# rubendhz/houdini-gsplat-renderer

Hardware: AMD Instinct MI355X
Metric: frames/sec at 1920x1080 + achieved HBM GB/s (blend kernel) (higher is better)
Workload: dtype f32

## Files before the change

### houdini-gsplat-renderer_amd/csrc/gsr_api.hip

```cpp
#include <hip/hip_runtime.h>

#include <cmath>
#include <cstddef>
#include <cstdio>
#include <cstring>
#include <chrono>
#include <algorithm>
#include <new>
#include <vector>

#include "../../include/gsplat_hip.h"
#include "gsr_device.h"
#include "k_binning.h"
#include "k_blend.h"
#include "k_cluster.h"
#include "k_colour.h"
#include "k_preprocess.h"
#ifdef GSR_HOST_TIMING
static double g_t_verdict = 0, g_acc_py = 0, g_acc_pre = 0, g_acc_launch = 0; static long g_acc_n = 0;
static double now_us() { return std::chrono::duration<double, std::micro>(std::chrono::steady_clock::now().time_since_epoch()).count(); }
#endif
#include "k_sort.h"
#include "k_wire.h"
#include "gsr_frame_plan.h"
// ... 21 lines not shown
    bool same(const SortKey& o) const
    {
        return gen == o.gen && shard_index == o.shard_index && shard_count == o.shard_count && shard_layout == o.shard_layout && flags == o.flags &&
               band_first == o.band_first && band_tile_rows == o.band_tile_rows &&
               std::memcmp(&cam, &o.cam, sizeof(gsr_camera)) == 0;
    }
};

struct FrameArgs {
    gsr_camera cam{};
    const float* depth = nullptr;
    bool depth_is_device = false;
    float* out = nullptr;
    bool out_is_device = false;
    int aov = 0;
    float* aov_out = nullptr;
    gsr_background bg{};
};

struct FrameJob {
    FrameArgs args;
    bool open = false;
    GsrFrame f{};
    uint32_t n = 0;
    int local_tiles = 0, band_rows = 0, n_super = 0;
    size_t out_px = 0;
    float* target = nullptr;
    int format = 0;
    const float* d_depth = nullptr;
    bool timing = false, timing_all = false, use_map = false;
    bool speculative = false;
    int bn_items = 4;
    uint32_t bn_grid = 0;
    uint32_t k1_grid = 0;
    bool local_sort = false;
    bool sort_failed = false;
    bool redo = false;
    bool ranges_folded = false;
    bool deferred = false;
    bool lazy = false;
    bool cull = false;
    bool direct = false;
    uint32_t ticket = 0;
    int phase = 0;
    bool dcull = false;
    int dpar = 0;
    bool sort_fresh = false;
    bool dblind = false;
    bool dstat = false;
    bool blend_guess_plain = false;
    float2* aov_target = nullptr;
    GsrBgArgs bg{};
};

struct FrameSlot {
    hipStream_t own = nullptr;
    hipStream_t stream = nullptr;
    hipEvent_t ev_done = nullptr;
    hipEvent_t ev_user = nullptr;
    hipEvent_t ev_band[GSR_HOST_BANDS_MAX] = {nullptr, nullptr, nullptr, nullptr, nullptr, nullptr, nullptr, nullptr};
    int bands = 0;
    int band_row[GSR_HOST_BANDS_MAX + 1] = {0, 0, 0, 0, 0, 0, 0, 0, 0};
    hipEvent_t ev_pairs = nullptr;
    GsrRecord* rec = nullptr;
    uint32_t *keyA = nullptr, *keyB = nullptr;
    uint32_t* blk_cnt = nullptr;
    uint2 *valA = nullptr, *valB = nullptr;
    uint32_t* d_n = nullptr;
    float* zwin = nullptr;
    StageBuf depth_stage;
    float* dpyr = nullptr;
    size_t dpyr_cap = 0;
    uint32_t* dactive = nullptr;
    int dpar = 0;
    bool dpyr_built = false;
    bool sorted_dculled = false;
    uint32_t* hist = nullptr;
    size_t hist_cap = 0;
    uint32_t* totals = nullptr;
    uint2* pvA = nullptr;
    size_t pair_cap = 0;
    int32_t *sstart = nullptr, *send = nullptr;
    uint4* tile_work = nullptr;
    size_t tile_cap = 0;
    uint4* tile_work_a = nullptr;
    float* tbuf = nullptr;
    size_t tbuf_cap = 0;
    float* hpyr2 = nullptr;
    uint32_t* slab = nullptr;
    bool slab_dirty = false;
    int32_t* redo = nullptr;
    int32_t* order = nullptr;
    size_t order_cap = 0;
    bool order_valid = false;
    int order_age = 0;
    int order_sig[6] = {0, 0, 0, 0, 0, 0}, order_per_xcd = 0;
    uint32_t* st_scan = nullptr;
    GsrTilePartial* partial = nullptr;
    uint32_t* sup_work = nullptr;
    int sup_par = 0;
    float* hpyr = nullptr;
    float* hpyr_next = nullptr;
    float* hraw = nullptr;
    float* hstat = nullptr;
    bool hstat_valid = false;
    uint32_t* dbg_viol = nullptr;
    int hpyr_re = 0;
    uint32_t* cseg = nullptr;
    uint32_t* ccnt = nullptr;
    uint32_t* d_counts = nullptr;
    uint32_t* bkt_key = nullptr;
    uint2* bkt_val = nullptr;
    uint32_t* bkt_cnt = nullptr;
    GsrSlotHints hints;
    GsrLocalSortPolicy local_pol;
    unsigned long long* h_end = nullptr;
    unsigned long long* h_rows = nullptr;
    unsigned long long* h_rows_dev = nullptr;
    uint32_t rows_ticket = 0;
    int rows_tiles_y = 0;
    unsigned long long* h_end_dev = nullptr;
    bool horizon_valid = false;
    int horizon_sig[7] = {0, 0, 0, 0, 0, 0, 0};
    gsr_camera horizon_cam{};
    bool sorted_culled = false;
    unsigned long long* lazy_ctr = nullptr;
    uint32_t* colour_evals = nullptr;
    bool last_lazy = false;
    StageBuf fb;
    StageBuf aovb;
    float* fb32 = nullptr;
    size_t fb32_cap = 0;
    StageBuf bgb;
    unsigned long long* counters = nullptr;
    unsigned long long* h_total = nullptr;
    unsigned long long* h_total_dev = nullptr;
    uint32_t ticket = 0;
    unsigned long long* h_counters = nullptr;
    unsigned long long* d_frame = nullptr;
    bool sort_valid = false;
    SortKey sort_key{};
    uint32_t key_min = 0;
    FrameJob job;
    int last_tiles_x = 0, last_local_ty = 0, last_supers = 0;
    uint32_t last_cc_groups = 0, last_cc_per = 0;
    uint32_t last_pairs = 0;
    int super_tile = 0, stiles_x = 0, stiles_y = 0;
    uint64_t frame_id = 0;
    hipEvent_t ev[GSR_STAGE_EVENTS];
    bool ev_pending = false;
    bool ev_all = false;
    bool ev_ok = false;
};

struct gsr_context {
    int device = 0;
    hipStream_t own_stream = nullptr;
    hipStream_t stream = nullptr;

    uint32_t n = 0, cap = 0;
    bool has_sh = false;
    float origin[3] = {0, 0, 0};
    uint64_t geo_gen = 0;
    bool has_geometry = false;
    float4* geoA = nullptr;
    uint4* geoB = nullptr;
    uint4* col = nullptr;
    uint4* colrow = nullptr;
    int col_chunks = 0;
    float4* geoA2 = nullptr;
    uint4 *geoB2 = nullptr, *col2 = nullptr, *colrow2 = nullptr;
    float4 *clusA2 = nullptr, *clusB2 = nullptr;
    uint32_t* perm = nullptr;
    std::vector<int32_t> h_perm;
    float4 *clusA = nullptr, *clusB = nullptr;
    uint32_t nclus = 0;
    uint32_t* prefix = nullptr;
    uint32_t* prefix_all = nullptr;
    uint32_t* prefix_none = nullptr;
    bool prefix_valid = false;
    bool uploading = false;
    uint32_t up_total = 0, up_filled = 0;
    bool bbox_ok = false;
    double bb_lo[3] = {0, 0, 0}, bb_hi[3] = {0, 0, 0};

    FrameSlot slot[GSR_MAX_SLOTS];
    uint32_t* pos_order = nullptr;
    size_t pos_cap = 0;
    bool pos_valid = false;
    uint64_t pos_gen = 0;
    float pos_cam[3] = {0, 0, 0}, last_cam[3] = {0, 0, 0};
    uint32_t pos_kmin = 0, pos_kmax = 0;
    bool last_cam_set = false;
    uint32_t* blk_pre = nullptr;
    size_t blk_pre_cap = 0;
    int opt_order_keep = 32;
    int opt_fuse_order = 1;
    int opt_mid_sort = 1;
    int opt_host_bands = 4;
// ... 68 lines not shown
    hipDeviceSynchronize();
    return hipMemcpyFromSymbol(out128, HIP_SYMBOL(g_kprof), sizeof(g_kprof)) == hipSuccess ? 0 : -1;
}
#endif
#ifdef SW_PROFILE
extern "C" int gsr_debug_sw_profile(unsigned long long* out8) {
    hipDeviceSynchronize();
    hipMemcpyFromSymbol(out8, HIP_SYMBOL(g_sw_prof), 64);
    return 0;
}
#endif
#ifdef GSR_DEBUG_XCC
extern "C" int gsr_debug_xcc(unsigned* out4, int reset) {
    hipDeviceSynchronize();
    if (out4) hipMemcpyFromSymbol(out4, HIP_SYMBOL(g_dbg_xcc), 16);
    if (reset) { void* p = nullptr; hipGetSymbolAddress(&p, HIP_SYMBOL(g_dbg_xcc)); hipMemset(p, 0, 16); }
    return 0;
}
#endif
#ifdef BL_PROFILE
extern "C" int gsr_debug_blend_profile(unsigned long long* out, int reset) {
    hipDeviceSynchronize();
    if (out) hipMemcpyFromSymbol(out, HIP_SYMBOL(g_blend_prof), sizeof(unsigned long long) * BLP_MAX_WG * 4 * 16);
    if (reset) { void* p = nullptr; hipGetSymbolAddress(&p, HIP_SYMBOL(g_blend_prof)); hipMemset(p, 0, sizeof(unsigned long long) * BLP_MAX_WG * 4 * 16); }
    return 0;
}
#endif
__attribute__((visibility("hidden"))) int gsr_internal_set_error(int code, const char* text) { return set_err(code, "%s", text); }
void gsr_internal_comm_release(gsr_context* c);
bool gsr_internal_comm_set_user_stream(gsr_context* c, void* stream, void* own);
int gsr_internal_comm_sync(gsr_context* c);

extern "C" int gsr_device_count(void)
{
    int n = 0;
    if (hipGetDeviceCount(&n) != hipSuccess) return 0;
    return n;
}

extern "C" const char* gsr_last_error(void) { return g_err; }
extern "C" const char* gsr_version(void) { return GSR_VERSION_STR; }

static int finish_open_frames(gsr_context* c);

static int sync_all(gsr_context* c)
{
    int frc = finish_open_frames(c);
    if (frc) return frc;
    for (int k = 0; k < GSR_MAX_SLOTS; ++k)
        if (c->slot[k].own) HIP_TRY(hipStreamSynchronize(c->slot[k].own));
    if (c->stream) HIP_TRY(hipStreamSynchronize(c->stream));
    return GSR_OK;
}

static bool slot_init(FrameSlot& sl)
{
    bool ok = hipStreamCreateWithFlags(&sl.own, hipStreamNonBlocking) == hipSuccess;
    sl.stream = sl.own;
    ok = ok && hipEventCreateWithFlags(&sl.ev_done, hipEventDisableTiming) == hipSuccess;
    ok = ok && hipEventCreateWithFlags(&sl.ev_user, hipEventDisableTiming) == hipSuccess;
    ok = ok && hipEventCreateWithFlags(&sl.ev_pairs, hipEventDisableTiming) == hipSuccess;
    ok = ok && hipMalloc(reinterpret_cast<void**>(&sl.counters), 8 * sizeof(unsigned long long)) == hipSuccess;
    ok = ok && hipMalloc(reinterpret_cast<void**>(&sl.d_n), sizeof(uint32_t)) == hipSuccess;
    ok = ok && hipMemset(sl.d_n, 0, sizeof(uint32_t)) == hipSuccess;
    ok = ok && hipMalloc(reinterpret_cast<void**>(&sl.totals), 512 * sizeof(uint32_t)) == hipSuccess;
    ok = ok && hipMalloc(reinterpret_cast<void**>(&sl.lazy_ctr), 2 * sizeof(unsigned long long)) == hipSuccess;
    ok = ok && hipMemset(sl.lazy_ctr, 0, 2 * sizeof(unsigned long long)) == hipSuccess;
    ok = ok && hipMalloc(reinterpret_cast<void**>(&sl.colour_evals), 256 * sizeof(uint32_t)) == hipSuccess;
    ok = ok && hipMemset(sl.colour_evals, 0, 256 * sizeof(uint32_t)) == hipSuccess;
    ok = ok && hipMalloc(reinterpret_cast<void**>(&sl.hpyr), GSR_PYR_FLOATS * sizeof(float)) == hipSuccess;
    ok = ok && hipMalloc(reinterpret_cast<void**>(&sl.hpyr_next), GSR_PYR_FLOATS * sizeof(float)) == hipSuccess;
    ok = ok && hipMalloc(reinterpret_cast<void**>(&sl.hraw), (size_t)GSR_MAX_TILES_SIDE * GSR_MAX_TILES_SIDE * sizeof(float)) == hipSuccess;
    ok = ok && hipMalloc(reinterpret_cast<void**>(&sl.hstat), (size_t)GSR_MAX_TILES_SIDE * GSR_MAX_TILES_SIDE * sizeof(float)) == hipSuccess;
    ok = ok && hipMalloc(reinterpret_cast<void**>(&sl.hpyr2), GSR_PYR_FLOATS * sizeof(float)) == hipSuccess;
    ok = ok && hipMalloc(reinterpret_cast<void**>(&sl.slab), (GSR_SLAB_BINS + 8) * sizeof(uint32_t)) == hipSuccess;
    ok = ok && hipMemset(sl.slab, 0, (GSR_SLAB_BINS + 8) * sizeof(uint32_t)) == hipSuccess;
    ok = ok && hipMalloc(reinterpret_cast<void**>(&sl.ccnt), CC_MAX_GROUPS * sizeof(uint32_t)) == hipSuccess;
    ok = ok && hipMalloc(reinterpret_cast<void**>(&sl.bkt_key), (size_t)BK_BUCKETS * BK_CAP * sizeof(uint32_t)) == hipSuccess;
    ok = ok && hipMalloc(reinterpret_cast<void**>(&sl.bkt_val), (size_t)BK_BUCKETS * BK_CAP * sizeof(uint2)) == hipSuccess;
    ok = ok && hipMalloc(reinterpret_cast<void**>(&sl.bkt_cnt), (size_t)BK_BUCKETS * BK_STRIDE * sizeof(uint32_t)) == hipSuccess;
    ok = ok && hipMemset(sl.bkt_cnt, 0, (size_t)BK_BUCKETS * BK_STRIDE * sizeof(uint32_t)) == hipSuccess;
    ok = ok && hipMalloc(reinterpret_cast<void**>(&sl.d_counts), 4 * sizeof(uint32_t)) == hipSuccess;
    ok = ok && hipMemset(sl.d_counts, 0, 4 * sizeof(uint32_t)) == hipSuccess;
    ok = ok && hipHostMalloc(reinterpret_cast<void**>(&sl.h_end), sizeof(unsigned long long), hipHostMallocMapped | hipHostMallocCoherent) == hipSuccess;
    if (ok) sl.h_end[0] = 0ull;
    ok = ok && hipHostGetDevicePointer(reinterpret_cast<void**>(&sl.h_end_dev), sl.h_end, 0) == hipSuccess;
    ok = ok && hipMalloc(reinterpret_cast<void**>(&sl.st_scan), 512 * sizeof(uint32_t)) == hipSuccess;
    ok = ok && hipMemset(sl.st_scan, 0, 512 * sizeof(uint32_t)) == hipSuccess;
    ok = ok && hipMalloc(reinterpret_cast<void**>(&sl.partial), (size_t)(GSR_MAX_TILES_SIDE / 8) * (GSR_MAX_TILES_SIDE / 8) * sizeof(GsrTilePartial)) == hipSuccess;
    ok = ok && hipMalloc(reinterpret_cast<void**>(&sl.sup_work), 512 * sizeof(uint32_t)) == hipSuccess;
    ok = ok && hipMemset(sl.sup_work, 0, 512 * sizeof(uint32_t)) == hipSuccess;
    ok = ok && hipHostMalloc(reinterpret_cast<void**>(&sl.h_total), 4 * sizeof(unsigned long long), hipHostMallocMapped | hipHostMallocCoherent) == hipSuccess;
    if (ok) { sl.h_total[0] = 0ull; sl.h_total[1] = 0ull; sl.h_total[2] = 0ull; sl.h_total[3] = 0ull; }
    ok = ok && hipHostGetDevicePointer(reinterpret_cast<void**>(&sl.h_total_dev), sl.h_total, 0) == hipSuccess;
    ok = ok && hipHostMalloc(reinterpret_cast<void**>(&sl.h_counters), 8 * sizeof(unsigned long long), 0) == hipSuccess;
    if (ok) for (int j = 0; j < 8; ++j) sl.h_counters[j] = 0;
    ok = ok && hipMalloc(reinterpret_cast<void**>(&sl.d_frame), 8 * sizeof(unsigned long long)) == hipSuccess;
    ok = ok && hipMemset(sl.d_frame, 0, 8 * sizeof(unsigned long long)) == hipSuccess;
    ok = ok && hipMemset(sl.counters, 0, 8 * sizeof(unsigned long long)) == hipSuccess;
    if (ok) {
        for (int k = 0; k < GSR_STAGE_EVENTS; ++k) sl.ev[k] = nullptr;
        sl.ev_ok = true;
        for (int k = 0; k < GSR_STAGE_EVENTS && ok; ++k) ok = hipEventCreate(&sl.ev[k]) == hipSuccess;
    }
    return ok;
}

static void slot_free_splat_arrays(FrameSlot& sl)
{
    dev_free(sl.rec); dev_free(sl.keyA); dev_free(sl.keyB); dev_free(sl.valA); dev_free(sl.valB); dev_free(sl.blk_cnt);
    dev_free(sl.zwin); dev_free(sl.cseg);
    sl.sort_valid = false;
}

struct SlotSplatArrays {
    GsrRecord* rec = nullptr;
    uint32_t *keyA = nullptr, *keyB = nullptr, *blk_cnt = nullptr, *cseg = nullptr;
    uint2 *valA = nullptr, *valB = nullptr;
    float* zwin = nullptr;
    void release() { dev_free(rec); dev_free(keyA); dev_free(keyB); dev_free(valA); dev_free(valB); dev_free(blk_cnt); dev_free(zwin); dev_free(cseg); }
};
static int alloc_splat_arrays(SlotSplatArrays& a, size_t cap)
{
    int rc = GSR_OK;
    if ((rc = dev_alloc(&a.rec, cap)) || (rc = dev_alloc(&a.keyA, cap + 256)) || (rc = dev_alloc(&a.keyB, cap + 256)) ||
        (rc = dev_alloc(&a.valA, cap + 256)) || (rc = dev_alloc(&a.valB, cap + 256)) ||
        (rc = dev_alloc(&a.zwin, cap)) || (rc = dev_alloc(&a.blk_cnt, cap / 256 + 16)) ||
        (rc = dev_alloc(&a.cseg, cap / GSR_CLUSTER + (size_t)CC_THREADS * 64 + 16)))
        a.release();
    return rc;
}
static void slot_take_splat_arrays(FrameSlot& sl, SlotSplatArrays& a)
{
    slot_free_splat_arrays(sl);
    sl.rec = a.rec; sl.keyA = a.keyA; sl.keyB = a.keyB; sl.valA = a.valA; sl.valB = a.valB; sl.blk_cnt = a.blk_cnt; sl.zwin = a.zwin; sl.cseg = a.cseg;
    a = SlotSplatArrays{};
}

static void slot_destroy(FrameSlot& sl)
{
    slot_free_splat_arrays(sl);
    dev_free(sl.hist); dev_free(sl.totals);
    dev_free(sl.pvA);
    dev_free(sl.sstart); dev_free(sl.send); dev_free(sl.tile_work); dev_free(sl.order); dev_free(sl.sup_work); sl.fb.release(); dev_free(sl.fb32); sl.aovb.release(); sl.bgb.release();
    dev_free(sl.hpyr); dev_free(sl.hpyr_next); dev_free(sl.hraw); dev_free(sl.hstat); dev_free(sl.hpyr2); dev_free(sl.slab); dev_free(sl.tile_work_a); dev_free(sl.tbuf); dev_free(sl.ccnt); dev_free(sl.bkt_key); dev_free(sl.bkt_val); dev_free(sl.bkt_cnt); dev_free(sl.d_counts); dev_free(sl.st_scan); dev_free(sl.partial);
    if (sl.h_end) (void)hipHostFree(sl.h_end); if (sl.h_rows) (void)hipHostFree(sl.h_rows); sl.depth_stage.release(); dev_free(sl.dpyr); dev_free(sl.dactive);
    dev_free(sl.redo); dev_free(sl.lazy_ctr); dev_free(sl.colour_evals);
    dev_free(sl.counters); dev_free(sl.d_n);
    if (sl.h_total) (void)hipHostFree(sl.h_total);
    if (sl.h_counters) (void)hipHostFree(sl.h_counters);
    dev_free(sl.d_frame);
    if (sl.ev_ok)
        for (int k = 0; k < GSR_STAGE_EVENTS; ++k)
            if (sl.ev[k]) (void)hipEventDestroy(sl.ev[k]);
    if (sl.ev_done) (void)hipEventDestroy(sl.ev_done);
    if (sl.ev_user) (void)hipEventDestroy(sl.ev_user);
    for (int k = 0; k < GSR_HOST_BANDS_MAX; ++k) if (sl.ev_band[k]) (void)hipEventDestroy(sl.ev_band[k]);
    if (sl.ev_pairs) (void)hipEventDestroy(sl.ev_pairs);
    if (sl.own) (void)hipStreamDestroy(sl.own);
}

extern "C" int gsr_create(int device, gsr_context** out)
{
    if (!out) return set_err(GSR_E_INVALID, "gsr_create: out is NULL");
    *out = nullptr;
    int ndev = gsr_device_count();
    if (ndev <= 0) return set_err(GSR_E_NO_DEVICE, "gsr_create: no HIP device visible");
    if (device < 0 || device >= ndev) return set_err(GSR_E_NO_DEVICE, "gsr_create: device %d out of range (0..%d)", device, ndev - 1);
    HIP_TRY(hipSetDevice(device));
    gsr_context* c = new (std::nothrow) gsr_context();
    if (!c) return set_err(GSR_E_OOM, "gsr_create: host allocation failed");
    c->device = device;
    if (const char* e = std::getenv("GSR_ORDER_KEEP")) c->opt_order_keep = std::atoi(e);
    if (const char* e = std::getenv("GSR_SCATTER_DIRECT")) c->opt_scatter_direct = std::atoi(e);
    if (const char* e = std::getenv("GSR_K1_SCATTER")) c->opt_k1_scatter = std::atoi(e);
    if (const char* e = std::getenv("GSR_HOST_BANDS")) c->opt_host_bands = std::min(std::max(std::atoi(e), 1), GSR_HOST_BANDS_MAX);
    if (const char* e = std::getenv("GSR_MID_SORT")) c->opt_mid_sort = std::atoi(e);
    if (const char* e = std::getenv("GSR_FUSE_ORDER")) c->opt_fuse_order = std::atoi(e);
    if (const char* e = std::getenv("GSR_SLAB_FRAC")) { const int v = std::atoi(e); if (v >= 1 && v <= 255) c->slab_frac = v; }
    if (const char* e = std::getenv("GSR_SLAB_MIN")) { const int v = std::atoi(e); if (v >= 1) c->slab_min = v; }
    if (const char* e = std::getenv("GSR_SLAB_MAX")) { const int v = std::atoi(e); if (v >= 1) c->slab_max = v; }
    if (const char* e = std::getenv("GSR_BN_ITEMS")) { const int v = std::atoi(e); if (v == 1 || v == 2 || v == 4) c->opt_bn_items = v; }
    hipError_t e = hipStreamCreateWithFlags(&c->own_stream, hipStreamNonBlocking);
    if (e != hipSuccess) { delete c; return set_err(GSR_E_HIP, "hipStreamCreate failed: %s", hipGetErrorString(e)); }
    c->stream = c->own_stream;
    bool ok = true;
    for (int k = 0; k < GSR_MAX_SLOTS && ok; ++k) ok = slot_init(c->slot[k]);
    if (!ok) {
        gsr_destroy(c);
        return set_err(GSR_E_HIP, "gsr_create: allocating frame slots (streams/events/mailboxes) failed");
    }
    if (hipMalloc(reinterpret_cast<void**>(&c->prefix), 256 * 4) != hipSuccess ||
        hipMalloc(reinterpret_cast<void**>(&c->prefix_all), 256 * 4) != hipSuccess ||
        hipMalloc(reinterpret_cast<void**>(&c->prefix_none), 256 * 4) != hipSuccess ||
        hipMemset(c->prefix, 0xff, 256 * 4) != hipSuccess || hipMemset(c->prefix_all, 0xff, 256 * 4) != hipSuccess ||
        hipMemset(c->prefix_none, 0, 256 * 4) != hipSuccess ||
        hipMalloc(reinterpret_cast<void**>(&c->lazy_hint), 4) != hipSuccess || hipMemset(c->lazy_hint, 0, 4) != hipSuccess) {
        gsr_destroy(c);
        return set_err(GSR_E_HIP, "gsr_create: allocating the colour-prefix tables failed");
    }
    c->st.record_bytes = (int32_t)sizeof(GsrRecord);
    c->st.pair_bytes = 8;
    *out = c;
    return GSR_OK;
}

static void vis_drop_mask(gsr_context* c)
{
    dev_free(c->vis_mask);
    if (c->vis.n_volumes == 0) { c->vis_on = false; c->vis_hidden = 0; }
}

static void free_geometry(gsr_context* c)
{
    dev_free(c->geoA); dev_free(c->geoB); dev_free(c->col); dev_free(c->colrow);
    dev_free(c->perm); dev_free(c->clusA); dev_free(c->clusB); c->nclus = 0; c->h_perm.clear();
    dev_free(c->geoA2); dev_free(c->geoB2); dev_free(c->col2); dev_free(c->colrow2); dev_free(c->clusA2); dev_free(c->clusB2);
    dev_free(c->alpha0);
    dev_free(c->alpha0_2);
    vis_drop_mask(c);
    for (int k = 0; k < GSR_MAX_SLOTS; ++k) slot_free_splat_arrays(c->slot[k]);
    c->cap = 0; c->n = 0;
}

extern "C" void gsr_destroy(gsr_context* c)
{
    if (!c) return;
// ... 1256 lines not shown
}

static inline int mark(FrameSlot& sl, int k)
{
    const FrameJob& j = sl.job;
    if (j.timing && (j.timing_all || k >= 5)) HIP_TRY(hipEventRecord(sl.ev[k], sl.stream));
    return GSR_OK;
}

static GsrRangeArgs range_args(gsr_context* c, FrameSlot& sl)
{
    const FrameJob& j = sl.job;
    GsrRangeArgs a;
    a.totals = sl.totals; a.n_super = j.n_super; a.sstart = sl.sstart; a.send = sl.send; a.host_total = sl.h_total_dev;
    a.ticket = j.ticket; a.max_pairs = (unsigned long long)GSR_MAX_PAIRS; a.redo_count = reinterpret_cast<uint32_t*>(sl.lazy_ctr);
    a.lazy_hint = c->lazy_hint; a.n_sorted = sl.d_n; a.k1_counts = sl.d_counts; a.sorted_keys = sl.keyA;
    a.depth_active = j.dcull ? sl.dactive + j.dpar : (const uint32_t*)nullptr;
    return a;
}

static inline void tile_sig(const GsrFrame& f, int* sig )
{
    const int now[6] = {f.width, f.height, f.shard_rpb > 0 ? f.shard_first : f.shard_index, f.shard_count, f.shard_rpb, f.super_shift};
    std::memcpy(sig, now, sizeof now);
}

static inline int32_t list_cap(const FrameSlot& sl) { return (int32_t)std::min<size_t>(sl.pair_cap, (size_t)0x7fffffff); }

static GsrSumArgs sum_args(const FrameJob& j)
{
    GsrSumArgs g;
    g.n_tiles = j.local_tiles; g.tiles_x = j.f.tiles_x; g.tiles_y = j.f.tiles_y; g.shard = gsr_frame_shard(j.f, 0);
    g.super_shift = j.f.super_shift; g.stiles_x = j.f.stiles_x; g.n_super = j.n_super;
    return g;
}

static GsrHorizonArgs horizon_args(const gsr_context* c, const FrameSlot& sl)
{
    const GsrFrame& f = sl.job.f;
    GsrHorizonArgs hz{};
    hz.list_cap = list_cap(sl); hz.lists = sl.pvA; hz.geoA = c->geoA; hz.idx_mask = f.idx_mask;
    for (int l = 0; l < GSR_PYR_LEVELS; ++l) hz.pyr_off[l] = f.pyr_off[l];
    hz.cam[0] = f.cam[0]; hz.cam[1] = f.cam[1]; hz.cam[2] = f.cam[2];
    return hz;
}

static int queue_blend(gsr_context* c, FrameSlot& sl, bool with_depth, bool guarded)
{
    const FrameJob& j = sl.job;
    const GsrFrame& f = j.f;
    hipStream_t s = sl.stream;
    if (j.local_tiles <= 0) return GSR_OK;
    if (!j.direct) HIP_TRY(hipStreamWaitEvent(s, sl.ev_user, 0));
    GsrBlendArgs a;
    a.guard = guarded ? sl.dactive + j.dpar : (const uint32_t*)nullptr; a.guard_want = 0u;
    {
        const bool persp = f.pr[8] == 0.0f && f.pr[9] == 0.0f && f.pr[12] == 0.0f && f.pr[13] == 0.0f && f.pr[14] == -1.0f && f.pr[15] == 0.0f;
        a.near_alpha = persp ? 0.5f * (1.0f - f.pr[10]) : 0.0f;
        a.near_scale = persp ? 1.12f : 0.0f;
    }
    a.tile_cov = (with_depth && j.dcull && !j.dblind) ? sl.dpyr + 4 * sl.dpyr_cap : (const float*)nullptr;
    a.idx_mask = f.idx_mask; a.zq0 = f.zq0; a.zqs = f.zqs;
    a.tile_dmax = (with_depth && j.dcull && !j.dblind && f.idx_mask != 0xffffffffu) ? sl.dpyr + (size_t)(2 * j.dpar) * sl.dpyr_cap + f.pyr_off[0] : (const float*)nullptr;
    a.width = f.width; a.height = f.height; a.tiles_x = f.tiles_x; a.local_tiles = j.local_tiles;
    a.shard = gsr_frame_shard(f, 0); a.band_rows = j.band_rows;
    a.super_shift = f.super_shift; a.rect_shift = f.rect_shift; a.stiles_x = f.stiles_x; a.use_map = j.use_map ? 1 : 0; a.flags = f.flags;
    a.list_cap = list_cap(sl);
    a.sup_work = (a.use_map && c->opt_swizzle >= 2 && sl.sup_work) ? sl.sup_work + 256 * sl.sup_par : nullptr;
    a.slab = j.phase; a.tbuf = sl.tbuf; a.tile_work_a = sl.tile_work_a;
    uint4* const tw = j.phase == 1 ? sl.tile_work_a : sl.tile_work;
    int sig[6];
    tile_sig(f, sig);
    const bool ordered = a.use_map && c->opt_swizzle >= 2 && sl.order_valid && std::memcmp(sig, sl.order_sig, sizeof sig) == 0;
    const int32_t* tmap = ordered ? sl.order : c->tile_map;
    const unsigned grid = ordered ? (unsigned)(8 * sl.order_per_xcd) : a.use_map ? (unsigned)c->map_grid : (unsigned)j.local_tiles;
    GsrLazyArgs lz;
    lz.f = f; lz.colrow = c->colrow;
    lz.redo = j.lazy ? sl.redo : nullptr;
    lz.redo_count = reinterpret_cast<uint32_t*>(sl.lazy_ctr);
    const bool over = j.bg.kind != 0;
    a.out_format = j.format; a.out_packed = (j.format != GSR_TARGET_RGBA32F || over) ? (void*)j.target : nullptr;
    float4* tgt = reinterpret_cast<float4*>((j.format != GSR_TARGET_RGBA32F || over) ? sl.fb32 : j.target);
    auto launch = [&](auto kernel, unsigned g, const int32_t* map, uint4* work, auto... tail) {
        hipLaunchKernelGGL(kernel, dim3(g), dim3(256), 0, s, a, map, sl.pvA, sl.sstart, sl.send, sl.rec, tgt, work, sl.zwin, j.d_depth, lz, tail...);
    };
    auto launch_verb = [&](auto plain, auto aov, auto bg, unsigned g, const int32_t* map, uint4* work) {
        if (j.aov_target) launch(aov, g, map, work, j.aov_target);
        else if (over) launch(bg, g, map, work, j.bg);
        else launch(plain, g, map, work);
    };
    int nb = 1;
    if (!j.args.out_is_device && j.phase != 1 && c->opt_host_bands > 1 && c->shard_count == 1 && c->band_tile_rows < 0 && f.local_tiles_y >= 4 * c->opt_host_bands) nb = c->opt_host_bands;
    if (nb > 1 && !c->copy_stream && hipStreamCreateWithFlags(&c->copy_stream, hipStreamNonBlocking) != hipSuccess) { c->copy_stream = nullptr; nb = 1; (void)hipGetLastError(); }
    for (int b = 0; b < nb && nb > 1; ++b)
        if (!sl.ev_band[b] && hipEventCreateWithFlags(&sl.ev_band[b], hipEventDisableTiming) != hipSuccess) { sl.ev_band[b] = nullptr; nb = 1; (void)hipGetLastError(); }
    sl.bands = nb;
    for (int b = 0; b < nb; ++b) {
        a.row_lo = nb > 1 ? (int)((int64_t)f.local_tiles_y * b / nb) : 0;
        a.row_hi = nb > 1 ? (int)((int64_t)f.local_tiles_y * (b + 1) / nb) : 0x7fffffff;
        sl.band_row[b] = a.row_lo; sl.band_row[b + 1] = nb > 1 ? a.row_hi : f.local_tiles_y;
        if (with_depth) launch_verb(k_blend<true>, k_blend_aov<true>, k_blend_over<true>, grid, tmap, tw);
        else launch_verb(k_blend<false>, k_blend_aov<false>, k_blend_over<false>, grid, tmap, tw);
        if (j.lazy && with_depth) launch_verb(k_blend_lazy<true>, k_blend_aov_lazy<true>, k_blend_over_lazy<true>, (unsigned)j.local_tiles, c->tile_map, sl.tile_work);
        else if (j.lazy) launch_verb(k_blend_lazy<false>, k_blend_aov_lazy<false>, k_blend_over_lazy<false>, (unsigned)j.local_tiles, c->tile_map, sl.tile_work);
        if (nb > 1) HIP_TRY(hipEventRecord(sl.ev_band[b], s));
    }
    HIP_TRY(hipGetLastError());
    return GSR_OK;
}

static int queue_back_end(gsr_context* c, FrameSlot& sl)
{
    const FrameJob& j = sl.job;
    const GsrFrame& f = j.f;
    hipStream_t s = sl.stream;
    int rc;
    if ((rc = mark(sl, 3))) return rc;
    if (j.n > 0) {
        const uint32_t nblk = div_up(j.n, (uint32_t)BN_THREADS * (uint32_t)j.bn_items);
        const size_t lds = (size_t)4 * j.bn_items * j.n_super * (8 + 4);
        const GsrShard shd = gsr_frame_shard(f, f.rect_shift);
        const GsrRangeArgs ra = j.ranges_folded ? range_args(c, sl) : GsrRangeArgs{};
        const uint32_t bn_extra = (uint32_t)BN_SPLIT_TILES * (uint32_t)std::max(f.stiles_y - 1, 0);
        const uint32_t grid = std::min(nblk, j.bn_grid) + bn_extra + (j.ranges_folded ? 1u : 0u);
#define GSR_PLACE(I) hipLaunchKernelGGL((f.idx_mask != 0xffffffffu ? k_bin_place<I, true> : k_bin_place<I, false>), dim3(grid), dim3(BN_THREADS), lds, s, sl.valA, sl.d_n,          \
                                        f.super_shift - f.rect_shift, shd, f.stiles_x, j.n_super, sl.hist, sl.sstart, nblk, (uint32_t)sl.pair_cap, sl.pvA, ra,   \
                                        f.idx_mask != 0xffffffffu ? sl.zwin : (const float*)nullptr, f.zq0, f.zqs)
        if (j.bn_items == 1) GSR_PLACE(1); else if (j.bn_items == 2) GSR_PLACE(2); else GSR_PLACE(4);
#undef GSR_PLACE
        HIP_TRY(hipGetLastError());
    }
    if ((rc = mark(sl, 4))) return rc;
    if (j.lazy && j.n > 0) {
        const bool predict = c->prefix_valid && !(f.flags & GSR_FLAG_LAZY_NO_PREFIX);
        hipLaunchKernelGGL(k_colour_prefix, dim3((unsigned)(j.n_super * CL_BLOCKS_PER_LIST)), dim3(CL_THREADS), 0, s, f, sl.pvA,
                           sl.sstart, sl.send, (f.flags & GSR_FLAG_LAZY_NO_PREFIX) ? c->prefix_none : (predict ? c->prefix : c->prefix_all),
                           (int)list_cap(sl), c->colrow, sl.rec, sl.colour_evals);
        HIP_TRY(hipGetLastError());
    }
    if ((rc = mark(sl, 5))) return rc;
    sl.job.blend_guess_plain = j.d_depth != nullptr && j.dcull && !c->depth_active && !j.deferred && j.f.idx_mask == 0xffffffffu && !j.aov_target && j.bg.kind == 0;
    if ((rc = queue_blend(c, sl, j.d_depth != nullptr && !sl.job.blend_guess_plain, sl.job.blend_guess_plain))) return rc;
    return mark(sl, 6);
}

static int queue_frame_end(gsr_context* c, FrameSlot& sl)
{
    const FrameJob& j = sl.job;
    hipStream_t s = sl.stream;
    const GsrSumArgs g = sum_args(j);
    GsrHorizonArgs hz{};
    hz.list_cap = list_cap(sl);
    if (c->opt_cull && c->opt_cull != 3 && j.n > 0 && !j.deferred && (c->opt_cull >= 2 || j.cull || j.phase == 2 || (c->cull_pol.vis_unculled >= 300000u && c->cull_pol.holdoff <= 2))) {
        hz = horizon_args(c, sl);
        hz.raw = sl.hraw; hz.pyr_in = sl.hpyr; hz.pyr_out = sl.hpyr_next; hz.dilate = j.f.cull_dilate; hz.culled = j.cull ? 1 : 0;
        hz.host_end = j.cull ? sl.h_end_dev : nullptr; hz.ticket = j.ticket;
        hz.stat = sl.hstat;
        hz.stat_in_use = (j.cull && j.dcull && j.dstat) ? 1 : 0;
        hz.depth_culled = (j.dcull && !j.dblind) ? 1 : 0;
        static const bool dbgv = std::getenv("GSR_DEBUG_VIOL") != nullptr;
        if (dbgv) {
            if (!sl.dbg_viol && hipMalloc(reinterpret_cast<void**>(&sl.dbg_viol), 80 * 4) != hipSuccess) sl.dbg_viol = nullptr;
            if (sl.dbg_viol) (void)hipMemsetAsync(sl.dbg_viol, 0, 80 * 4, s);
            hz.dbg = sl.dbg_viol;
        }
    }
    if (j.phase == 2) { hz.slab = 2; hz.tile_work_a = sl.tile_work_a; }
    const int nblocks8 = ((j.f.tiles_x + 7) >> 3) * ((j.f.tiles_y + 7) >> 3);
    hipLaunchKernelGGL(k_tile_pass, dim3((unsigned)nblocks8), dim3(64), 0, s, sl.tile_work, g, sl.sstart, sl.send, hz, sl.partial, sl.st_scan);
    uint32_t* const prefix_arg = (j.f.sh_order > 0 && c->opt_lazy) ? c->prefix : (uint32_t*)nullptr;
    const uint32_t* const redo_arg = j.lazy ? reinterpret_cast<const uint32_t*>(sl.lazy_ctr) : (const uint32_t*)nullptr;
    uint32_t* const work_next = sl.sup_work ? sl.sup_work + 256 * (sl.sup_par ^ 1) : (uint32_t*)nullptr;
    sl.horizon_valid = hz.raw != nullptr;
    sl.hstat_valid = hz.raw != nullptr;
    int osig[6];
    tile_sig(j.f, osig);
    const bool order_due = c->opt_swizzle >= 3 || (c->opt_swizzle == 2 && c->order_pays);
    const bool order_kept = !order_due && c->opt_swizzle == 2 && c->opt_order_keep > 0 && sl.order_valid && sl.order_age < c->opt_order_keep &&
                            std::memcmp(osig, sl.order_sig, sizeof osig) == 0;
    const bool order_refresh = !order_due && !order_kept && c->opt_swizzle == 2 && c->opt_order_keep > 0 && c->n >= 1000000u;
    if (order_kept) sl.order_age += 1; else sl.order_valid = false;
    const bool order_now = j.use_map && (order_due || order_refresh) && j.local_tiles > 0 && j.n_super <= 256 && sl.sup_work;
    const int per_xcd = 2 * ((j.n_super + 15) / 16) << (2 * j.f.super_shift);
    if (order_now && (size_t)8 * per_xcd > sl.order_cap) {
        const int rc = regrow(s, sl.order, sl.order_cap, (size_t)8 * per_xcd, (size_t)8 * per_xcd);
        if (rc) return rc;
    }
    const bool fused_order = order_now && c->opt_fuse_order != 0;
    if (sl.horizon_valid) sl.hpyr_re = std::min(c->cull_pol.dilate, GSR_DILATE_EXACT_MAX);
    if (fused_order) {
        const GsrOrderArgs oa{sl.tile_work, j.f.tiles_y, sl.sup_work + 256 * sl.sup_par, per_xcd, sl.order};
        const int ndil = sl.horizon_valid ? nblocks8 : 0;
        hipLaunchKernelGGL(k_frame_end_order, dim3(9u + (unsigned)((ndil + TO_THREADS / 64 - 1) / (TO_THREADS / 64))), dim3(TO_THREADS), 0, s, sl.partial, nblocks8, ndil, g, sl.counters, sl.d_n, sl.d_frame,
                           prefix_arg, redo_arg, sl.colour_evals, sl.lazy_ctr + 1, sl.sstart, sl.send, c->lazy_hint, work_next, hz, sl.st_scan, sl.hpyr_re, oa);
        HIP_TRY(hipGetLastError());
    } else if (sl.horizon_valid) {
        hipLaunchKernelGGL(k_frame_end, dim3((unsigned)nblocks8 + 1u), dim3(SW_THREADS), 0, s, sl.partial, nblocks8, g, sl.counters, sl.d_n, sl.d_frame,
                           prefix_arg, redo_arg, sl.colour_evals, sl.lazy_ctr + 1, sl.sstart, sl.send, c->lazy_hint, work_next, hz, sl.st_scan, sl.hpyr_re);
        HIP_TRY(hipGetLastError());
    } else {
        hipLaunchKernelGGL(k_sum_work, dim3(1), dim3(SW_THREADS), 0, s, sl.partial, nblocks8, g, sl.counters, sl.d_n, sl.d_frame,
                           prefix_arg, redo_arg, sl.colour_evals, sl.lazy_ctr + 1, sl.sstart, sl.send, c->lazy_hint, work_next, hz, sl.st_scan);
        HIP_TRY(hipGetLastError());
    }
    if (sl.horizon_valid) {
        std::swap(sl.hpyr, sl.hpyr_next);
        tile_sig(j.f, sl.horizon_sig);
        sl.horizon_sig[6] = (int)c->geo_gen;
        sl.horizon_cam = j.args.cam;
    }
    if (order_now) {
        if (!fused_order) {
            hipLaunchKernelGGL(k_tile_order, dim3(8), dim3(TO_THREADS), 0, s, sl.tile_work, g, j.f.tiles_y, sl.sup_work + 256 * sl.sup_par,
                               per_xcd, sl.order);
            HIP_TRY(hipGetLastError());
        }
        std::memcpy(sl.order_sig, osig, sizeof osig);
        sl.order_per_xcd = per_xcd;
        sl.order_valid = true;
        sl.order_age = 0;
    }
    if (c->opt_row_work && sl.h_rows_dev) {
        hipLaunchKernelGGL(k_row_work, dim3((unsigned)((j.f.tiles_y + RW_THREADS / 64 - 1) / (RW_THREADS / 64))), dim3(RW_THREADS), 0, s, sl.tile_work,
                           j.phase == 2 ? sl.tile_work_a : (const uint4*)nullptr, g, sl.h_rows_dev, j.ticket);
        HIP_TRY(hipGetLastError());
        sl.rows_ticket = j.ticket; sl.rows_tiles_y = j.f.tiles_y;
    }
    sl.sup_par ^= 1;
    if (j.f.sh_order > 0 && c->opt_lazy) c->prefix_valid = j.phase == 0;
    sl.last_lazy = j.lazy;
    if (j.timing) { sl.ev_pending = true; sl.ev_all = j.timing_all; }
    if (!j.args.out_is_device) {
        const size_t bpp = (size_t)gsr_format_pixel_bytes(j.format);
        if (sl.bands > 1 && c->copy_stream) {
            for (int b = 0; b < sl.bands; ++b) {
                const size_t r0 = std::min<size_t>((size_t)sl.band_row[b] * GSR_TILE, (size_t)j.band_rows), r1 = std::min<size_t>((size_t)sl.band_row[b + 1] * GSR_TILE, (size_t)j.band_rows);
                if (r1 <= r0) continue;
                const size_t off = r0 * (size_t)j.f.width * bpp;
                HIP_TRY(hipStreamWaitEvent(c->copy_stream, sl.ev_band[b], 0));
                HIP_TRY(hipMemcpyAsync(reinterpret_cast<char*>(j.args.out) + off, static_cast<const char*>(sl.fb.p) + off, (r1 - r0) * (size_t)j.f.width * bpp, hipMemcpyDeviceToHost, c->copy_stream));
            }
            HIP_TRY(hipStreamSynchronize(c->copy_stream));
        } else {
            HIP_TRY(hipMemcpyAsync(j.args.out, sl.fb.p, j.out_px * bpp, hipMemcpyDeviceToHost, s));
        }
        if (j.aov_target) HIP_TRY(hipMemcpyAsync(j.args.aov_out, sl.aovb.p, j.out_px * 8, hipMemcpyDeviceToHost, s));
        HIP_TRY(hipStreamSynchronize(s));
    }
    if (!j.direct) {
        HIP_TRY(hipEventRecord(sl.ev_done, s));
        HIP_TRY(hipStreamWaitEvent(c->stream, sl.ev_done, 0));
    }
// ... 107 lines not shown
    }
    GsrOutcomeIn in;
    in.has_splats = j.n > 0; in.phase = j.phase; in.cull = j.cull; in.local_sort = j.local_sort; in.dcull = j.dcull; in.dblind = j.dblind;
    in.speculative = j.speculative; in.deferred = j.deferred; in.blend_guess_plain = j.blend_guess_plain; in.key_min = j.f.key_min;
    in.pair_cap = sl.pair_cap; in.has_list_buffer = sl.pvA != nullptr; in.max_pairs = (uint64_t)GSR_MAX_PAIRS;
    in.mb_pairs = mb.pairs; in.mb_hints = mb.hints; in.mb_kept = mb.kept; in.mb_clusters = mb.clusters; in.mb_key_lo = mb.key_lo; in.mb_key_hi = mb.key_hi;
    const GsrFrameOutcome o = gsr_frame_outcome(in, sl.hints);
    const uint32_t D = mb.pairs;
    if (o.local_result >= 0) sl.local_pol.on_sort_result(o.local_result != 0);
    if (o.end == GSR_FE_SORT_GAVE_UP) {
        j.sort_failed = true;
        sl.last_pairs = 0;
        return abandon_attempt(sl, false);
    }
    if (o.end == GSR_FE_DEPTH_APPEARED) {
        c->depth_active = true;
        c->st.frames_requeued += 1;
        return abandon_attempt(sl, true);
    }
    if (o.depth_active >= 0) {
        c->depth_active = o.depth_active != 0;
        if (j.sort_fresh) sl.sorted_dculled = c->depth_active;
    }
    if (o.verdicts) {
        c->lazy_pays = mb.has(GSR_HINT_LAZY_PAYS);
        c->cull_pol.on_kernel_verdict(mb.has(GSR_HINT_CULL_PAYS));
        c->prefix_cheaper = mb.has(GSR_HINT_PREFIX_CHEAPER);
        c->order_pays = mb.has(GSR_HINT_ORDER_PAYS);
    }
    if (o.kept_counts) c->cull_pol.on_kept(j.cull, mb.kept, c->opt_cull);
    if (o.slab_done) c->slab_pol.on_frame_done(sl.hints.kept_hint, c->cull_pol.vis_unculled);
    if (j.n > 0 && j.phase != 0) {
        static const bool dbg = std::getenv("GSR_SLAB_DEBUG") != nullptr;
        if (dbg) fprintf(stderr, "[slab] phase %d: clusters through K1 %u, splats kept %u, pairs %u\n", j.phase, mb.clusters, mb.kept, D);
    }
    if (o.end == GSR_FE_TOO_MANY_PAIRS)
        return frame_abort(sl, set_err(GSR_E_TOO_MANY_PAIRS, "gsr_render: the frame's super-tile pairs exceed the limit of %lld", GSR_MAX_PAIRS));
    if (o.grow) {
        const size_t floor_ = sl.pvA ? 0 : std::min<size_t>((size_t)2 * j.n + 4096, (size_t)1 << 22);
        const size_t want = std::max<size_t>((size_t)D + D / 4 + 4096, std::max(floor_, c->pair_want));
        const int rc = regrow(sl.stream, sl.pvA, sl.pair_cap, want + 4, want);
        if (rc) return frame_abort(sl, rc);
        c->pair_want = std::max(c->pair_want, want);
    }
    if (o.end == GSR_FE_SLAB_OVERRUN) {
        c->st.frames_requeued += 1;
        return abandon_attempt(sl, true);
    }
    if (o.back_end == GSR_BE_TRUNCATED) c->st.frames_truncated += 1;
    if (o.back_end == GSR_BE_REQUEUED) {
        c->st.frames_requeued += 1;
        if (sl.sup_work) (void)hipMemsetAsync(sl.sup_work + 256 * sl.sup_par, 0, 256 * sizeof(uint32_t), sl.stream);
    }
    if (o.back_end == GSR_BE_QUEUED || o.back_end == GSR_BE_REQUEUED) {
        const int rc = queue_back_end(c, sl);
        if (rc) return frame_abort(sl, rc);
    }
    sl.last_pairs = D;
    if (o.guard_miss) {
        j.blend_guess_plain = false;
        const int rc = queue_blend(c, sl, true, false);
        if (rc) return frame_abort(sl, rc);
    }
    if (o.end == GSR_FE_PHASE_2) {
        const int rc = queue_slab_mid(c, sl);
        if (rc) return frame_abort(sl, rc);
        if (j.timing) { sl.ev_pending = true; sl.ev_all = false; }
        j.open = false;
        const FrameArgs a = j.args;
        return render_again(c, a, 2, nullptr);
    }
    if (!j.deferred) {
        const int rc = queue_frame_end(c, sl);
        if (rc) return frame_abort(sl, rc);
    }
    j.open = false;
    return GSR_OK;
}

static int frame_verdict(gsr_context* c, FrameSlot& sl, bool* broke)
{
    (void)c;
    const FrameJob& j = sl.job;
    volatile unsigned long long* box = sl.h_end;
    unsigned long long v = 0;
    const int wrc = wait_mailbox(sl, box, j.ticket, "culling verdict", &v);
    if (wrc) return wrc;
    *broke = (v & GSR_END_HORIZON_BROKE) != 0ull;
    return GSR_OK;
}

static int finish_open_frames(gsr_context* c)
{
    int rc = GSR_OK;
    for (int k = 0; k < GSR_MAX_SLOTS; ++k) {
        const int r = frame_finish(c, c->slot[k]);
        if (r && !rc) rc = r;
    }
    return rc;
}

static int build_pos_order(gsr_context* c, FrameSlot& sl, const GsrFrame& f, int key_bits)
{
    const uint32_t n = c->n;
    int rc;
    uint32_t *kA = nullptr, *kB = nullptr, *vA = nullptr, *vB = nullptr;
    auto drop = [&]() { dev_free(kA); dev_free(kB); dev_free(vA); dev_free(vB); };
    if ((rc = dev_alloc(&kA, (size_t)n + 256)) || (rc = dev_alloc(&kB, (size_t)n + 256)) || (rc = dev_alloc(&vA, (size_t)n + 256)) ||
        (rc = dev_alloc(&vB, (size_t)n + 256))) { drop(); return rc; }
    hipStream_t s = sl.stream;
    hipLaunchKernelGGL(k_pos_keys, dim3(div_up(n, 256)), dim3(256), 0, s, c->geoA, n, f.cam[0], f.cam[1], f.cam[2], f.key_min, f.key_max, kA, vA);
    rc = radix_sort(sl, kA, vA, kB, vB, n, key_bits, true, (uint32_t*)nullptr, RS_XCD_DEPTH != 0);
    if (!rc && hipStreamSynchronize(s) != hipSuccess) rc = set_err(GSR_E_HIP, "position-keyed order: sort failed");
    if (rc) { drop(); return rc; }
    dev_free(c->pos_order);
    c->pos_order = vA; vA = nullptr;
    drop();
    c->pos_valid = true;
    c->pos_gen = c->geo_gen;
    std::memcpy(c->pos_cam, f.cam, sizeof c->pos_cam);
    c->pos_kmin = f.key_min; c->pos_kmax = f.key_max;
    return GSR_OK;
}

struct FrontEnd {
    GsrFramePlan p;
    bool pos_match = false;
    SortKey key_now;
    int rounds = 0; uint32_t ngroups = 0;
    int hist_shift = 0;
    GsrDepthPyrArgs dp{};
    uint32_t n_dp = 0;
    GsrDepthCull dc_clus{nullptr, nullptr, nullptr}, dc_k1{nullptr, nullptr, nullptr};
    GsrK1Scatter scat{};
};

static int frame_open(gsr_context* c, const FrameArgs& a, FrameSlot*& slot)
{
    const gsr_camera* cam = &a.cam;
    if (c->uploading) return set_err(GSR_E_INVALID, "gsr_render: upload in progress");
    if (cam->width <= 0 || cam->height <= 0 || cam->width > GSR_MAX_DIM || cam->height > GSR_MAX_DIM)
        return set_err(GSR_E_INVALID, "gsr_render: bad framebuffer size %dx%d (max %d)", cam->width, cam->height, GSR_MAX_DIM);
    if (!c->has_geometry) return set_err(GSR_E_NO_GEOMETRY, "gsr_render: nothing uploaded");
    HIP_TRY(hipSetDevice(c->device));

    FrameSlot& sl = c->slot[c->frame_no % (uint64_t)c->nslots];
    slot = &sl;
    int rc = frame_finish(c, sl);
    if (rc) return rc;
    hipStream_t want = (c->nslots == 1) ? c->stream : sl.own;
    if (want != sl.stream) {
        HIP_TRY(hipStreamSynchronize(sl.stream));
        sl.stream = want;
    }
    if (sl.pair_cap > 0 && sl.pair_cap < c->pair_want && (rc = regrow(sl.stream, sl.pvA, sl.pair_cap, c->pair_want + 4, c->pair_want))) return rc;

    FrameJob& j = sl.job;
    j = FrameJob();
    j.args = a;
    build_frame(c, cam, &j.f);
    j.n = c->n;
    j.local_tiles = j.f.tiles_x * j.f.local_tiles_y;
    j.band_rows = ctx_band_rows(c, cam->height);
    j.out_px = (size_t)j.band_rows * cam->width;
    j.n_super = j.f.stiles_x * j.f.stiles_y;
    j.use_map = c->opt_swizzle != 0;
    return GSR_OK;
}

static void plan_frame(gsr_context* c, FrameSlot& sl, FrontEnd& fe, bool allow_cull, int phase_in)
{
    FrameJob& j = sl.job;
    const FrameArgs& a = j.args;
    const gsr_camera* cam = &a.cam;
    const GsrFrame& f = j.f;
    fe.key_now = SortKey{c->geo_gen, c->shard_index, c->shard_count, c->shard_layout, c->opt_flags, c->band_first, c->band_tile_rows, *cam};
    int sig[7] = {0, 0, 0, 0, 0, 0, (int)c->geo_gen};
    tile_sig(f, sig);
    GsrPlanIn in;
    in.phase_in = phase_in; in.allow_cull = allow_cull; in.out_is_device = a.out_is_device; in.has_depth = a.depth != nullptr;
    in.n = j.n; in.nclus = c->nclus; in.sh_order = f.sh_order; in.key_min = f.key_min; in.key_max = f.key_max;
    in.opt_deferred = c->opt_deferred; in.opt_lazy = c->opt_lazy; in.opt_cull = c->opt_cull; in.opt_slab = c->opt_slab; in.opt_cluster = c->opt_cluster;
    in.opt_sort_cache = c->opt_sort_cache; in.opt_local_sort = c->opt_local_sort; in.opt_k1_scatter = c->opt_k1_scatter;
    in.opt_scatter_direct = c->opt_scatter_direct; in.opt_mid_sort = c->opt_mid_sort; in.opt_bn_items = c->opt_bn_items;
    in.full_keys = (c->opt_flags & GSR_FLAG_FULL_KEYS) != 0; in.shard_count = c->shard_count;
    in.timing = c->opt_timing != 0 && (c->opt_timing >= 2 || c->frame_no % (uint64_t)c->opt_timing_every == 0);
    in.timing_all = c->opt_timing >= 2;
    in.opt_timing = c->opt_timing;
    in.lazy_pays = c->lazy_pays; in.prefix_cheaper = c->prefix_cheaper; in.prefix_valid = c->prefix_valid; in.bbox_ok = c->bbox_ok;
    in.horizon_match = sl.horizon_valid && std::memcmp(sig, sl.horizon_sig, sizeof sig) == 0;
    in.hpyr_re = sl.hpyr_re;
    in.sort_match = sl.sort_valid && sl.sort_key.same(fe.key_now);
    in.sorted_culled = sl.sorted_culled; in.sorted_dculled = sl.sorted_dculled;
    in.pos_match = c->pos_valid && c->pos_gen == c->geo_gen && std::memcmp(c->pos_cam, cam->cam_pos, sizeof c->pos_cam) == 0 &&
                   c->pos_kmin == f.key_min && c->pos_kmax == f.key_max;
    in.same_pos = c->last_cam_set && std::memcmp(c->last_cam, cam->cam_pos, sizeof c->last_cam) == 0;
    in.hints = sl.hints;
    fe.pos_match = in.pos_match;
    fe.p = gsr_plan_frame(in, c->cull_pol, c->slab_pol, sl.local_pol, c->classic_once, [&] { return camera_jumped(c, sl.horizon_cam, *cam); });
    const GsrFramePlan& p = fe.p;
    j.deferred = p.deferred; j.lazy = p.lazy; j.cull = p.cull; j.phase = p.phase; j.timing = p.timing; j.timing_all = p.timing_all;
    j.dcull = p.dcull; j.local_sort = p.local || p.local_phase; j.bn_items = p.bn_items; j.bn_grid = p.bn_grid; j.k1_grid = p.k1_grid;
    j.f.cull_dilate = p.cull_dilate;
    j.f.phase = p.phase;
    c->st.frames_jumped += p.jumped;
    c->st.frames_culled += p.cull;
    c->st.frames_slab += p.phase == 1;
    c->st.frames_lazy += p.lazy && j.n > 0 && phase_in == 0;
    j.ticket = ++sl.ticket ? sl.ticket : ++sl.ticket;
    if (j.timing) harvest_slot(c, sl);
}

static int stage_frame_buffers(gsr_context* c, FrameSlot& sl)
{
    FrameJob& j = sl.job;
    const FrameArgs& a = j.args;
    const gsr_camera* cam = &a.cam;
    const GsrFrame& f = j.f;
    hipStream_t s = sl.stream;
    int rc;
    j.direct = sl.stream == c->stream;
    if (!j.direct) HIP_TRY(hipEventRecord(sl.ev_user, c->stream));

    if ((size_t)j.local_tiles + 1 > sl.tile_cap || !sl.sstart) {
        HIP_TRY(hipStreamSynchronize(s));
        dev_free(sl.tile_work); dev_free(sl.tile_work_a); dev_free(sl.sstart); dev_free(sl.send); dev_free(sl.redo);
        sl.tile_cap = 0;
        if ((rc = dev_alloc(&sl.tile_work, (size_t)j.local_tiles + 1)) || (rc = dev_alloc(&sl.tile_work_a, (size_t)j.local_tiles + 1)) || (rc = dev_alloc(&sl.sstart, (size_t)65536 + 1)) ||
            (rc = dev_alloc(&sl.send, (size_t)65536 + 1)) || (rc = dev_alloc(&sl.redo, (size_t)j.local_tiles + 1))) return rc;
        sl.tile_cap = (size_t)j.local_tiles + 1;
    }
    if (j.phase == 1 && j.out_px > sl.tbuf_cap && (rc = regrow(s, sl.tbuf, sl.tbuf_cap, j.out_px, j.out_px))) return rc;
    if (j.use_map && (rc = build_tile_map(c, f))) return rc;
    j.d_depth = a.depth;
    if (a.depth && !a.depth_is_device) {
        if ((rc = sl.depth_stage.upload(s, a.depth, (size_t)cam->width * cam->height * sizeof(float)))) return rc;
        j.d_depth = static_cast<const float*>(sl.depth_stage.p);
    }
    if (a.bg.kind != 0) {
        j.bg.kind = a.bg.kind; j.bg.format = a.bg.format;
        std::memcpy(j.bg.rgba, a.bg.rgba, sizeof j.bg.rgba);
        j.bg.image = a.bg.kind == GSR_BG_IMAGE ? a.bg.image : nullptr;
        if (a.bg.kind == GSR_BG_IMAGE && !a.bg.image_is_device) {
            if ((rc = sl.bgb.upload(s, a.bg.image, (size_t)cam->width * cam->height * (size_t)gsr_format_pixel_bytes(a.bg.format)))) return rc;
            j.bg.image = sl.bgb.p;
        }
    }
    if (j.dcull) {
        frame_depth_codes(c, cam, &j.f);
        const size_t need = (size_t)f.pyr_off[GSR_PYR_LEVELS - 1] + (size_t)gsr_pyr_dim(f.tiles_x, GSR_PYR_LEVELS - 1) * gsr_pyr_dim(f.tiles_y, GSR_PYR_LEVELS - 1) + 16;
        if (need > sl.dpyr_cap || !sl.dactive) {
            if ((rc = regrow(s, sl.dpyr, sl.dpyr_cap, 5 * need, need))) return rc;
            HIP_TRY(hipMemsetAsync(sl.dpyr, 0, 5 * need * sizeof(float), s));
            if (!sl.dactive) {
                if ((rc = dev_alloc(&sl.dactive, 2))) return rc;
                HIP_TRY(hipMemsetAsync(sl.dactive, 0, 2 * sizeof(uint32_t), s));
            }
        }
        if (j.phase != 2) sl.dpar ^= 1;
        j.dpar = sl.dpar;
    }
    j.target = a.out;
    j.format = c->target_format;
    const size_t bpp = (size_t)gsr_format_pixel_bytes(j.format);
    if ((j.format != GSR_TARGET_RGBA32F || a.bg.kind != 0) && j.phase == 1 && j.out_px * 4 > sl.fb32_cap && (rc = regrow(s, sl.fb32, sl.fb32_cap, j.out_px * 4, j.out_px * 4))) return rc;
    int band[6];
    tile_sig(f, band);
    if (!a.out_is_device) {
        band[5] = j.format;
        if ((rc = sl.fb.ensure(s, j.out_px * bpp)) || (rc = sl.fb.clear_if_reshaped(s, band, j.out_px * bpp))) return rc;
        j.target = static_cast<float*>(sl.fb.p);
    }
    if (a.aov != 0 && a.aov_out != nullptr) {
        j.aov_target = reinterpret_cast<float2*>(a.aov_out);
        if (!a.out_is_device) {
            band[5] = 0;
            if ((rc = sl.aovb.ensure(s, j.out_px * sizeof(float2))) || (rc = sl.aovb.clear_if_reshaped(s, band, j.out_px * sizeof(float2)))) return rc;
            j.aov_target = static_cast<float2*>(sl.aovb.p);
        }
    }
    return GSR_OK;
}

static int queue_pos_order(gsr_context* c, FrameSlot& sl, FrontEnd& fe)
{
    if (fe.p.want_pos && !fe.pos_match) {
        c->pos_valid = false;
        if (const int rc = fe.p.ordered ? build_pos_order(c, sl, sl.job.f, fe.p.key_bits) : GSR_OK) return rc;
    }
    std::memcpy(c->last_cam, sl.job.args.cam.cam_pos, sizeof c->last_cam);
    c->last_cam_set = true;
    return GSR_OK;
}

static int queue_cull(gsr_context* c, FrameSlot& sl, FrontEnd& fe)
{
    FrameJob& j = sl.job;
    const GsrFrame& f = j.f;
    const GsrFramePlan& p = fe.p;
    hipStream_t s = sl.stream;
    if (j.n == 0) return GSR_OK;
    cluster_grid(c->nclus, &fe.rounds, &fe.ngroups);
    if ((c->opt_flags & GSR_FLAG_CULL_ROUNDS) && c->nclus > 0) {
        fe.rounds = std::max(fe.rounds, 3);
        fe.ngroups = div_up(c->nclus, (uint32_t)CC_THREADS * (uint32_t)fe.rounds);
    }
    fe.hist_shift = p.key_bits > 10 ? p.key_bits - 10 : 0;
    const float* pyr = j.phase == 2 ? sl.hpyr2 : ((j.cull && !p.ordered) ? sl.hpyr : (const float*)nullptr);
    const GsrSlabPick pk{(uint32_t)c->slab_min, (uint32_t)c->slab_max, (uint32_t)c->slab_frac, f.key_max - f.key_min};
    GsrDepthPyrArgs& dp = fe.dp;
    if (j.dcull) {
        float* const dp0 = sl.dpyr + (size_t)(2 * j.dpar) * sl.dpyr_cap;
// ... 432 lines not shown
    if (rc) return rc;
    hipStream_t s = c->slot[0].own;
    GsrFrame f;
    build_frame(c, cam, &f);
    const size_t npix = (size_t)cam->width * cam->height;
    if (npix > c->wire_cap) {
        dev_free(c->wire_zbuf); dev_free(c->wire_out);
        c->wire_cap = 0;
        if ((rc = dev_alloc(&c->wire_zbuf, npix)) || (rc = dev_alloc(&c->wire_out, npix * 4))) {
            dev_free(c->wire_zbuf); dev_free(c->wire_out);
            return rc;
        }
        c->wire_cap = npix;
    }
    if ((rc = ensure_inverse_perm(c))) return rc;
    const uint32_t* const inv = (c->perm && c->n > 0) ? c->wire_inv : (const uint32_t*)nullptr;
    unsigned long long* zbuf = c->wire_zbuf;
    float* target = out_is_device ? rgba_out : c->wire_out;
    hipError_t e = hipMemsetAsync(zbuf, 0xff, npix * 8, s);
    if (e == hipSuccess && over && !out_is_device) e = hipMemcpyAsync(c->wire_out, rgba_out, npix * bpp, hipMemcpyHostToDevice, s);
    if (e == hipSuccess && c->n > 0)
        hipLaunchKernelGGL(k_wire_splats, dim3(div_up(c->n, 256)), dim3(256), 0, s, c->n, f, c->geoA, c->geoB, zbuf, inv ? c->perm : (const uint32_t*)nullptr);
    if (e == hipSuccess)
        hipLaunchKernelGGL(k_wire_resolve, dim3((unsigned)((npix + 255) / 256)), dim3(256), 0, s, zbuf, npix, c->col,
                           target, c->target_format, inv, over);
    if (e == hipSuccess) e = hipGetLastError();
    if (e == hipSuccess && !out_is_device) e = hipMemcpyAsync(rgba_out, c->wire_out, npix * bpp, hipMemcpyDeviceToHost, s);
    if (e == hipSuccess) e = hipStreamSynchronize(s);
    if (e != hipSuccess) return set_err(GSR_E_HIP, "gsr_render_wire: %s", hipGetErrorString(e));
    return GSR_OK;
}

extern "C" int gsr_debug_policy(int32_t* state16, int event, long long a, long long b)
{
    if (!state16) return set_err(GSR_E_INVALID, "gsr_debug_policy: NULL state");
    gsr_policy_apply(state16, event, a, b);
    return state16[11] < 0 ? set_err(GSR_E_INVALID, "gsr_debug_policy: unknown event %d", event) : GSR_OK;
}
extern "C" int gsr_debug_frame_plan(int which, const int32_t* in, int32_t* policy16, int32_t* out)
{
    if (!in || !out || (which == 0 && !policy16)) return set_err(GSR_E_INVALID, "gsr_debug_frame_plan: NULL argument");
    return gsr_frame_plan_apply(which, in, policy16, out) ? set_err(GSR_E_INVALID, "gsr_debug_frame_plan: unknown selector %d", which) : GSR_OK;
}
extern "C" int gsr_debug_policy_state(gsr_context* c, int32_t* state16)
{
    if (!c || !state16) return set_err(GSR_E_INVALID, "gsr_debug_policy_state: NULL argument");
    const GsrCullPolicy& p = c->cull_pol;
    const int32_t v[GSR_POLICY_STATE_INTS] = {p.pays, p.weak, (int32_t)p.vis_unculled, p.holdoff, p.backoff, p.streak, p.dilate, p.opt_dilate,
                                              c->slab_pol.holdoff, c->slot[0].local_pol.fails, c->slot[0].local_pol.holdoff, 0, 0, 0, 0, 0};
    std::memcpy(state16, v, sizeof v);
    return GSR_OK;
}

extern "C" int gsr_synchronize(gsr_context* c)
{
    if (!c) return set_err(GSR_E_INVALID, "gsr_synchronize: ctx is NULL");
    HIP_TRY(hipSetDevice(c->device));
    int rc = sync_all(c);
    return rc ? rc : gsr_internal_comm_sync(c);
}

static void fetch_counters(gsr_context* c)
{
    for (int k = 0; k < GSR_MAX_SLOTS; ++k)
        if (c->slot[k].d_frame && c->slot[k].h_counters)
            (void)hipMemcpy(c->slot[k].h_counters, c->slot[k].d_frame, 8 * sizeof(unsigned long long), hipMemcpyDeviceToHost);
}

static FrameSlot* latest_slot(gsr_context* c)
{
    FrameSlot* best = nullptr;
    for (int k = 0; k < GSR_MAX_SLOTS; ++k)
        if (c->slot[k].frame_id && (!best || c->slot[k].frame_id > best->frame_id)) best = &c->slot[k];
    return best;
}

extern "C" int gsr_get_stats(gsr_context* c, gsr_stats* out)
{
    if (!c || !out) return set_err(GSR_E_INVALID, "gsr_get_stats: NULL argument");
    HIP_TRY(hipSetDevice(c->device));
    int rc = sync_all(c);
    if (rc) return rc;
    fetch_counters(c);
    FrameSlot* last = latest_slot(c);
    for (int k = 0; k < GSR_MAX_SLOTS; ++k)
        if (&c->slot[k] != last) harvest_slot(c, c->slot[k]);
    if (last) {
        harvest_slot(c, *last);
        FrameSlot& sl = *last;
        c->st.n_visible = (int64_t)(sl.h_counters[6] & 0xffffffffull);
        c->st.lazy_redo_tiles = sl.last_lazy ? (int64_t)(sl.h_counters[7] & 0xffffffffull) : 0;
        c->st.pairs_consumed = (int64_t)sl.h_counters[1];
        c->st.entries_scanned = (int64_t)sl.h_counters[3];
        c->st.pairs_total = sl.last_pairs;
        c->st.clusters_total = c->nclus;
        c->st.clusters_kept = sl.hints.surv_hint;
        c->st.policy_bits = (c->lazy_pays ? 1 : 0) | (c->order_pays ? 2 : 0) | (c->cull_pol.pays ? 4 : 0) | (c->cull_pol.weak ? 8 : 0) | (c->prefix_cheaper ? 16 : 0) | (c->depth_active ? 32 : 0);
        c->st.cull_dilate = c->cull_pol.dilate;
        c->st.cull_holdoff = c->cull_pol.holdoff;
        c->st.tiles_x = sl.last_tiles_x;
        c->st.tiles_y = sl.last_local_ty;
        c->st.super_tile = sl.super_tile;
        c->st.stiles_x = sl.stiles_x;
        c->st.stiles_y = sl.stiles_y;
        int64_t rec_tot = 0, ent_tot = 0, ev_tot = 0;
        for (int k = 0; k < GSR_MAX_SLOTS; ++k) {
            if (!c->slot[k].frame_id) continue;
            rec_tot += (int64_t)c->slot[k].h_counters[2];
            ent_tot += (int64_t)c->slot[k].h_counters[4];
            ev_tot += (int64_t)c->slot[k].h_counters[5];
        }
        c->st.blend_pairs_consumed_total = rec_tot;
        c->st.blend_entries_scanned_total = ent_tot;
        c->st.blend_wave_evals_total = ev_tot;
        {
            unsigned long long tot = 0, v = 0;
            for (int k = 0; k < GSR_MAX_SLOTS; ++k)
                if (c->slot[k].lazy_ctr && hipMemcpy(&v, c->slot[k].lazy_ctr + 1, 8, hipMemcpyDeviceToHost) == hipSuccess) tot += v;
            c->st.lazy_colours_total = (int64_t)tot - c->lazy_base;
        }
    }
    *out = c->st;
    return GSR_OK;
}

static int peek_row_work(gsr_context* c, uint32_t* out, int n_rows, int64_t* frame_out)
{
    int order[GSR_MAX_SLOTS];
    for (int k = 0; k < GSR_MAX_SLOTS; ++k) order[k] = k;
    std::sort(order, order + GSR_MAX_SLOTS, [&](int a, int b) { return c->slot[a].frame_id > c->slot[b].frame_id; });
    for (int k = 0; k < GSR_MAX_SLOTS; ++k) {
        const FrameSlot& sl = c->slot[order[k]];
        if (!sl.h_rows || !sl.frame_id || !sl.rows_ticket || sl.rows_ticket != sl.ticket || sl.rows_tiles_y != n_rows) continue;
        const volatile unsigned long long* box = sl.h_rows;
        bool whole = true;
        for (int r = 0; r < n_rows && whole; ++r) {
            const unsigned long long v = box[r];
            whole = (uint32_t)(v >> 32) == sl.rows_ticket;
            out[r] = (uint32_t)v;
        }
        if (!whole) continue;
        if (frame_out) *frame_out = (int64_t)sl.frame_id;
        return 0;
    }
    return 1;
}
__attribute__((visibility("hidden"))) int gsr_internal_peek_row_work(gsr_context* c, uint32_t* out, int n_rows, int64_t* frame_out)
{
    if (!c || !out || !c->opt_row_work || n_rows < 1 || n_rows > GSR_MAX_TILES_SIDE) return 1;
    return peek_row_work(c, out, n_rows, frame_out);
}

extern "C" int gsr_read_row_work(gsr_context* c, uint32_t* out, int n_rows, int64_t* frame_out)
{
    if (!c || !out) return set_err(GSR_E_INVALID, "gsr_read_row_work: NULL argument");
    if (!c->opt_row_work) return set_err(GSR_E_INVALID, "gsr_read_row_work: GSR_OPT_ROW_WORK is off");
    HIP_TRY(hipSetDevice(c->device));
    int rc = sync_all(c);
    if (rc) return rc;
    FrameSlot* sl = latest_slot(c);
    if (!sl || !sl->rows_ticket) return set_err(GSR_E_INVALID, "gsr_read_row_work: no frame has run with GSR_OPT_ROW_WORK on");
    if (n_rows != sl->rows_tiles_y) return set_err(GSR_E_INVALID, "gsr_read_row_work: expected %d tile rows", sl->rows_tiles_y);
    if (peek_row_work(c, out, n_rows, frame_out)) return set_err(GSR_E_HIP, "gsr_read_row_work: the frame finished without delivering its row sums");
    return GSR_OK;
}

// ... 97 lines not shown
            gsr_debug_record& o = out[i];
            const GsrRecord& q = hr[slot];
            o.visible = 1;
            o.cx = q.cx; o.cy = q.cy; o.a1x = q.a1x; o.a1y = q.a1y; o.b1x = q.b1x; o.b1y = q.b1y;
            o.hx = q.hx; o.hy = q.hy; o.r = q.r; o.g = q.g; o.b = q.b; o.la = q.la;
            const uint32_t kb = hk[r] + sl->key_min;
            std::memcpy(&o.key, &kb, 4);
        }
    }
    delete[] hr; delete[] hk; delete[] hv;
    return rc;
}

extern "C" int gsr_debug_read_cull(gsr_context* c, uint32_t* rect, int64_t n, uint32_t* clusters, int64_t cap, int64_t* n_clusters)
{
    if (!c || !rect || n < 0 || (uint64_t)n > c->n || cap < 0 || (cap > 0 && !clusters) || !n_clusters) return set_err(GSR_E_INVALID, "gsr_debug_read_cull: bad argument");
    HIP_TRY(hipSetDevice(c->device));
    int rc = sync_all(c);
    if (rc) return rc;
    FrameSlot* sl = latest_slot(c);
    if (!sl) return set_err(GSR_E_INVALID, "gsr_debug_read_cull: no frame rendered yet");
    if (!sl->last_cc_groups) return set_err(GSR_E_INVALID, "gsr_debug_read_cull: the last frame ran no cluster pass over clusters");
    if ((rc = host_perm(c))) return rc;
    const uint32_t ns = sorted_count(sl);
    std::vector<uint2> hv(ns ? ns : 1);
    if (ns) HIP_TRY(hipMemcpy(hv.data(), sl->valA, (size_t)ns * 8, hipMemcpyDeviceToHost));
    for (int64_t i = 0; i < n; ++i) rect[i] = 0xffffffffu;
    for (uint32_t r = 0; r < ns; ++r) {
        const uint32_t slot = hv[r].x;
        if ((uint64_t)slot >= c->n) continue;
        const uint32_t i = to_upload_index(c, slot);
        if ((int64_t)i < n) rect[i] = hv[r].y;
    }
    const uint32_t ng = sl->last_cc_groups, per = sl->last_cc_per;
    std::vector<uint32_t> cnt(ng), seg((size_t)ng * per);
    HIP_TRY(hipMemcpy(cnt.data(), sl->ccnt, (size_t)ng * 4, hipMemcpyDeviceToHost));
    HIP_TRY(hipMemcpy(seg.data(), sl->cseg, (size_t)ng * per * 4, hipMemcpyDeviceToHost));
    int64_t m = 0;
    for (uint32_t g = 0; g < ng; ++g)
        for (uint32_t k = 0; k < cnt[g] && k < per; ++k, ++m)
            if (m < cap) clusters[m] = seg[(size_t)g * per + k];
    *n_clusters = m;
    return GSR_OK;
}

extern "C" int gsr_debug_read_depth_order(gsr_context* c, int32_t* perm, int64_t cap, int64_t* n_sorted)
{
    if (!c || !perm || !n_sorted || cap < 0) return set_err(GSR_E_INVALID, "gsr_debug_read_depth_order: bad argument");
    HIP_TRY(hipSetDevice(c->device));
    int rc = sync_all(c);
    if (rc) return rc;
    FrameSlot* sl = latest_slot(c);
    if (!sl) return set_err(GSR_E_INVALID, "gsr_debug_read_depth_order: no frame rendered yet");
    const uint32_t ns = sorted_count(sl);
    *n_sorted = ns;
    const int64_t m = (int64_t)ns < cap ? (int64_t)ns : cap;
    if (m) HIP_TRY(hipMemcpy2D(perm, 4, sl->valA, 8, 4, (size_t)m, hipMemcpyDeviceToHost));
    if ((rc = host_perm(c))) return rc;
    for (int64_t r = 0; r < m; ++r) perm[r] = (int32_t)to_upload_index(c, (uint32_t)perm[r]);
    return GSR_OK;
}

extern "C" int gsr_debug_read_tile_lists(gsr_context* c, int32_t* list_start, int32_t* list_end, int64_t n_lists,
                                         int32_t* pair_splat, int64_t n_pairs)
{
    if (!c || !list_start || !list_end) return set_err(GSR_E_INVALID, "gsr_debug_read_tile_lists: bad argument");
    HIP_TRY(hipSetDevice(c->device));
    int rc = sync_all(c);
    if (rc) return rc;
    FrameSlot* sl = latest_slot(c);
    if (!sl) return set_err(GSR_E_INVALID, "gsr_debug_read_tile_lists: no frame rendered yet");
    if (n_lists != (int64_t)sl->last_supers || n_pairs != (int64_t)sl->last_pairs || (n_pairs > 0 && !pair_splat))
        return set_err(GSR_E_INVALID, "gsr_debug_read_tile_lists: expected %d lists / %u pairs", sl->last_supers, sl->last_pairs);
    if (n_lists) {
        HIP_TRY(hipMemcpy(list_start, sl->sstart, (size_t)n_lists * 4, hipMemcpyDeviceToHost));
        HIP_TRY(hipMemcpy(list_end, sl->send, (size_t)n_lists * 4, hipMemcpyDeviceToHost));
    }
    if (n_pairs) HIP_TRY(hipMemcpy2D(pair_splat, 4, sl->pvA, 8, 4, (size_t)n_pairs, hipMemcpyDeviceToHost));
    if ((rc = host_perm(c))) return rc;
    for (int64_t r = 0; r < n_pairs; ++r) pair_splat[r] = (int32_t)to_upload_index(c, (uint32_t)pair_splat[r] & sl->job.f.idx_mask);
    return GSR_OK;
}

extern "C" int gsr_debug_read_tile_work(gsr_context* c, uint32_t* work4, int64_t n_tiles)
{
    if (!c || !work4) return set_err(GSR_E_INVALID, "gsr_debug_read_tile_work: bad argument");
    HIP_TRY(hipSetDevice(c->device));
    int rc = sync_all(c);
    if (rc) return rc;
    FrameSlot* sl = latest_slot(c);
    if (!sl || n_tiles != (int64_t)sl->last_tiles_x * sl->last_local_ty)
        return set_err(GSR_E_INVALID, "gsr_debug_read_tile_work: expected %d tiles", sl ? sl->last_tiles_x * sl->last_local_ty : 0);
    if (n_tiles) HIP_TRY(hipMemcpy(work4, sl->tile_work, (size_t)n_tiles * 16, hipMemcpyDeviceToHost));
    return GSR_OK;
}

extern "C" int gsr_debug_read_horizons(gsr_context* c, float* out4, int64_t n_tiles)
{
    if (!c || !out4) return set_err(GSR_E_INVALID, "gsr_debug_read_horizons: bad argument");
    HIP_TRY(hipSetDevice(c->device));
    int rc = sync_all(c);
    if (rc) return rc;
    FrameSlot* sl = latest_slot(c);
    if (!sl || n_tiles <= 0) return set_err(GSR_E_INVALID, "gsr_debug_read_horizons: no frame");
    std::vector<float> zero((size_t)n_tiles, 0.0f);
    HIP_TRY(hipMemcpy(out4, sl->hpyr, (size_t)n_tiles * 4, hipMemcpyDeviceToHost));
    HIP_TRY(hipMemcpy(out4 + n_tiles, sl->hraw, (size_t)n_tiles * 4, hipMemcpyDeviceToHost));
    HIP_TRY(hipMemcpy(out4 + 2 * n_tiles, sl->hstat, (size_t)n_tiles * 4, hipMemcpyDeviceToHost));
    if (sl->dpyr && sl->dpyr_cap >= (size_t)n_tiles) HIP_TRY(hipMemcpy(out4 + 3 * n_tiles, sl->dpyr + (size_t)(2 * sl->dpar + 1) * sl->dpyr_cap, (size_t)n_tiles * 4, hipMemcpyDeviceToHost));
    else std::memcpy(out4 + 3 * n_tiles, zero.data(), (size_t)n_tiles * 4);
    return GSR_OK;
}

static int debug_sort_pairs(gsr_context* c, uint32_t* keys, uint32_t* vals, int64_t n64, int key_bits, bool local);
extern "C" int gsr_debug_sort_pairs(gsr_context* c, uint32_t* keys, uint32_t* vals, int64_t n64, int key_bits)
{
    return debug_sort_pairs(c, keys, vals, n64, key_bits, false);
}
static thread_local uint32_t dbg_lo = 0;
static thread_local int dbg_shift = 0;
extern "C" int gsr_debug_sort_pairs_local(gsr_context* c, uint32_t* keys, uint32_t* vals, int64_t n64, int key_bits, uint32_t bucket_lo, int bucket_shift)
{
    if (bucket_shift < 0 || bucket_shift > 31) return set_err(GSR_E_INVALID, "gsr_debug_sort_pairs_local: bad bucket shift");
    dbg_lo = bucket_lo; dbg_shift = bucket_shift;
    return debug_sort_pairs(c, keys, vals, n64, key_bits, true);
}
static int debug_sort_pairs(gsr_context* c, uint32_t* keys, uint32_t* vals, int64_t n64, int key_bits, bool local)
{
    if (!c || n64 < 0 || n64 > 0x7fffffffll || key_bits < 1 || key_bits > 32 || (n64 > 0 && (!keys || !vals)))
        return set_err(GSR_E_INVALID, "gsr_debug_sort_pairs: bad argument");
    if (n64 == 0) return GSR_OK;
    HIP_TRY(hipSetDevice(c->device));
    int rc = sync_all(c);
    if (rc) return rc;
    FrameSlot& sl = c->slot[0];
    const uint32_t n = (uint32_t)n64;
    uint32_t *kA = nullptr, *kB = nullptr, *vA = nullptr, *vB = nullptr;
    if ((rc = dev_alloc(&kA, n)) || (rc = dev_alloc(&kB, n)) || (rc = dev_alloc(&vA, n)) || (rc = dev_alloc(&vB, n))) {
        dev_free(kA); dev_free(kB); dev_free(vA); dev_free(vB);
        return rc;
    }
    hipError_t e = hipMemcpyAsync(kA, keys, (size_t)n * 4, hipMemcpyHostToDevice, sl.stream);
    if (e == hipSuccess) e = hipMemcpyAsync(vA, vals, (size_t)n * 4, hipMemcpyHostToDevice, sl.stream);
    if (e == hipSuccess) {
        if (local) {
            const uint32_t nblk = div_up(n, RS_TILE);
            hipError_t e2 = hipMemsetAsync(sl.bkt_cnt, 0, (size_t)BK_BUCKETS * BK_STRIDE * sizeof(uint32_t), sl.stream);
            if (e2 == hipSuccess) e2 = hipMemsetAsync(sl.d_counts + 2, 0, 4, sl.stream);
            hipLaunchKernelGGL(HIP_KERNEL_NAME(k_bucket_scatter<uint32_t, false>), dim3(nblk), dim3(RS_THREADS), 0, sl.stream, kA, vA, n, (const uint32_t*)nullptr,
                               dbg_shift, dbg_lo, (const uint32_t*)nullptr, sl.bkt_cnt, sl.bkt_key, reinterpret_cast<uint32_t*>(sl.bkt_val), (uint32_t*)nullptr, sl.d_counts + 2);
            hipLaunchKernelGGL(HIP_KERNEL_NAME(k_radix_local<uint32_t>), dim3(BK_BUCKETS), dim3(RL_THREADS), 0, sl.stream, sl.bkt_cnt, dbg_shift, key_bits, dbg_lo,
                               sl.bkt_key, reinterpret_cast<uint32_t*>(sl.bkt_val), kA, vA, (uint32_t*)nullptr, (uint32_t*)nullptr);
            uint32_t over = 0;
            if (e2 == hipSuccess) e2 = hipMemcpyAsync(&over, sl.d_counts + 2, 4, hipMemcpyDeviceToHost, sl.stream);
            if (e2 == hipSuccess) e2 = hipStreamSynchronize(sl.stream);
            if (e2 != hipSuccess) rc = set_err(GSR_E_HIP, "gsr_debug_sort_pairs_local: %s", hipGetErrorString(e2));
            else if (over) rc = set_err(GSR_E_INVALID, "gsr_debug_sort_pairs_local: a bucket overflowed its region of %d keys (the pipeline would fall back to the global sort)", BK_CAP);
        } else {
            rc = radix_sort(sl, kA, vA, kB, vB, n, key_bits, true, (uint32_t*)nullptr, RS_XCD_DEPTH != 0);
        }
        if (!rc) {
            e = hipMemcpyAsync(keys, kA, (size_t)n * 4, hipMemcpyDeviceToHost, sl.stream);
            if (e == hipSuccess) e = hipMemcpyAsync(vals, vA, (size_t)n * 4, hipMemcpyDeviceToHost, sl.stream);
            if (e == hipSuccess) e = hipStreamSynchronize(sl.stream);
        }
    }
// ... 563 lines not shown
```

### houdini-gsplat-renderer_amd/csrc/gsr_mailbox.h

```cpp
#pragma once
#include <stdint.h>

static constexpr uint32_t GSR_HINT_LAZY_PAYS = 1u;
static constexpr uint32_t GSR_HINT_ORDER_PAYS = 2u;
static constexpr uint32_t GSR_HINT_CULL_PAYS = 4u;
static constexpr uint32_t GSR_HINT_PREFIX_CHEAPER = 8u;
static constexpr uint32_t GSR_HINT_VERDICTS = 31u;
static constexpr uint32_t GSR_HINT_SORT_GAVE_UP = 32u;
static constexpr uint32_t GSR_HINT_DEPTH_COVERED = 64u;
static constexpr uint32_t GSR_MB_TOO_MANY_PAIRS = 0xffffffffu;
static constexpr uint32_t GSR_END_HORIZON_BROKE = 1u;

struct GsrMailbox {
    uint32_t pairs = 0, hints = 0, kept = 0, clusters = 0, key_lo = 0, key_hi = 0;
    static GsrMailbox read(const volatile unsigned long long* box)
    {
        GsrMailbox m;
        const unsigned long long w1 = box[1], w3 = box[3];
        m.pairs = (uint32_t)box[0];
        m.hints = (uint32_t)w1; m.kept = (uint32_t)(w1 >> 32);
        m.clusters = (uint32_t)box[2];
        m.key_lo = (uint32_t)w3; m.key_hi = (uint32_t)(w3 >> 32);
        return m;
    }
    bool has(uint32_t hint) const { return (hints & hint) != 0u; }
};
```

### houdini-gsplat-renderer_amd/csrc/k_blend.h

```cpp
#pragma once
#include <type_traits>
#include "gsr_device.h"
#include "k_preprocess.h"
#include "k_cluster.h"

#ifndef BL_ROUND
#define BL_ROUND 64
#endif
#ifndef BL_WAVES_PER_EU
#define BL_WAVES_PER_EU 6
#endif
#ifndef BL_CHECK
#define BL_CHECK 4
#endif
#ifndef BL_BATCH
#define BL_BATCH 256
#endif
#ifndef BL_CHECK_AOVD
#define BL_CHECK_AOVD 2
#endif
#define BL_QCAP 2048
#define BL_PAIR_F4_MAX 6
#define GSR_T_MIN 6.103515625e-05f

#ifdef BL_PROFILE
#define BLP_MAX_WG 65536
__device__ unsigned long long g_blend_prof[BLP_MAX_WG][4][16];
#define BLP(i) { const long long now_ = clock64(); prof[i] += (unsigned long long)(now_ - tlast); tlast = now_; }
#else
#define BLP(i)
#endif

__device__ __forceinline__ uint32_t gsr_tile_weight(const uint4& w) { return w.z * 32u + w.y * 8u + (w.x >> 1); }

#ifdef GSR_DEBUG_XCC
__device__ uint32_t g_dbg_xcc[4];
#endif
struct GsrBlendArgs {
    int32_t width, height;
    int32_t tiles_x;
    int32_t local_tiles;
    GsrShard shard;
    int32_t band_rows;
    int32_t super_shift;
    int32_t rect_shift;
    int32_t stiles_x;
    int32_t use_map;
    int32_t flags;
    int32_t list_cap;
    uint32_t* sup_work;
    int32_t slab;
    float* tbuf;
    const uint4* tile_work_a;
    const uint32_t* guard;
    uint32_t guard_want;
    float near_alpha, near_scale;
    const float* tile_cov;
    uint32_t idx_mask;
    float zq0, zqs;
    const float* tile_dmax;
    int32_t row_lo, row_hi;
    int32_t out_format;
    void* out_packed;
};

#if BL_WAVES_PER_EU > 0
#define BL_OCC __attribute__((amdgpu_waves_per_eu(BL_WAVES_PER_EU)))
#else
#define BL_OCC
#endif
struct GsrLazyArgs {
    GsrFrame f;
    const uint4* colrow;
    int32_t* redo;
    uint32_t* redo_count;
};
struct GsrBgArgs {
    int32_t kind;
    int32_t format;
    float rgba[4];
    const void* image;
};
template <bool HAS_DEPTH, bool LAZY, bool AOV = false, bool OVER = false>
__device__ __forceinline__ void
gsr_blend_tile(const GsrBlendArgs& a, const int32_t* __restrict__ tile_map, const uint2* __restrict__ svals,
               const int32_t* __restrict__ sstart, const int32_t* __restrict__ send,
               const GsrRecord* __restrict__ recs, float4* __restrict__ out, uint4* __restrict__ tile_work,
               const float* __restrict__ zwin, const float* __restrict__ depth, const GsrLazyArgs& lz, float2* __restrict__ aov = nullptr,
               const GsrBgArgs* __restrict__ bg = nullptr)
{
    constexpr bool ZSTAGE = HAS_DEPTH || AOV;
    constexpr int PF4 = 5;
    __shared__ float4 slist[4][(BL_ROUND / 2) * PF4];
    __shared__ float2 szl[ZSTAGE ? 4 : 1][ZSTAGE ? BL_ROUND / 2 : 1];
    __shared__ uint32_t q[BL_QCAP];
    __shared__ __attribute__((aligned(16))) uint32_t scnt[2][4];
    __shared__ uint32_t sdone[2][4];
    __shared__ float swmax[2][4];
    __shared__ uint32_t sevals, sredo, sdmet;
    __shared__ uint32_t slastu[4];
    __shared__ uint32_t stail[32];
    __shared__ uint32_t slast[4];

    int tile;
    if (LAZY) {
        if (blockIdx.x >= *lz.redo_count) return;
        tile = lz.redo[blockIdx.x];
    } else {
        tile = a.use_map ? tile_map[blockIdx.x] : (int)blockIdx.x;
    }
#ifdef GSR_DEBUG_XCC
    if (threadIdx.x == 0) {
        uint32_t xcc;
        asm volatile("s_getreg_b32 %0, hwreg(HW_REG_XCC_ID)" : "=s"(xcc));
        xcc &= 0xfu;
        atomicAdd(&g_dbg_xcc[(xcc == (blockIdx.x & 7u)) ? 0 : 1], 1u);
        if (blockIdx.x == 0) g_dbg_xcc[2] = xcc;
    }
#endif
    if (tile < 0 || tile >= a.local_tiles) return;
    if (a.row_hi != 0x7fffffff) { const int row = tile / a.tiles_x; if (row < a.row_lo || row >= a.row_hi) return; }
    const uint32_t guard_now = (!HAS_DEPTH && a.guard) ? *a.guard : 0u;
    const int tid = threadIdx.x, lane = tid & 63, wave = tid >> 6;
#ifdef BL_PROFILE
    unsigned long long prof[10] = {0, 0, 0, 0, 0, 0, 0, 0, 0, 0};
    unsigned long long occ_lanes = 0, occ_evals = 0, occ_half = 0, occ_none = 0;
    long long tlast = clock64();
    const unsigned long long wall0 = wall_clock64();
#endif
    const int tx = tile % a.tiles_x, lty = tile / a.tiles_x;
    const int gty = gsr_shard_global_row(a.shard, lty);
    const int px = tx * GSR_TILE_PX + (wave & 1) * 8 + (lane & 7);
    const int py = gty * GSR_TILE_PX + (wave >> 1) * 8 + (lane >> 3);
    const bool pix_ok = (px < a.width) && (py < a.height);
    const gsr_v2f lx = (gsr_v2f)((float)((wave & 1) * 8 + (lane & 7))), ly = (gsr_v2f)((float)((wave >> 1) * 8 + (lane >> 3)));
    const float tcx0 = (float)(tx * GSR_TILE_PX) + 0.5f, tcy0 = (float)(gty * GSR_TILE_PX) + 0.5f;
    const float qcx = tcx0 + 3.5f + 8.0f * (float)(wave & 1), qcy = tcy0 + 3.5f + 8.0f * (float)(wave >> 1);
    if (tid == 0) { sevals = 0; sredo = 0; sdmet = 0; }
    if (tid < 4) slast[tid] = 0u;
    uint32_t my_evals = 0;
    uint32_t my_last = 0;
    const bool tile_plain = HAS_DEPTH && a.tile_cov != nullptr && !(a.flags & GSR_FLAG_NO_DEPTH_CLASS) && a.tile_cov[gty * a.tiles_x + tx] < 0.0f;
    const float dpx = (HAS_DEPTH && pix_ok && !tile_plain) ? depth[(size_t)py * a.width + px] : __builtin_inff();
    bool d_met = false;
    bool d_triv = true, d_init = !HAS_DEPTH;
    float d_wmin = __builtin_inff();

    const int st = (gty >> a.super_shift) * a.stiles_x + (tx >> a.super_shift);
    const int s = sstart[st];
    const int e_ = send[st] < a.list_cap ? send[st] : a.list_cap;
    const int n = e_ > s ? e_ - s : 0;
    if (!HAS_DEPTH && a.guard && (guard_now != 0u) != (a.guard_want != 0u)) return;

    gsr_v2f C01 = {0.0f, 0.0f};
    float C2 = 0.0f, T = 1.0f;
    float Z = 0.0f;
    bool wave_done = false;
    if (a.slab == 2) {
        const uint4 wa = a.tile_work_a[tile];
        if (wa.w & 1u) {
            if (tid == 0) tile_work[tile] = make_uint4(0u, 0u, 0u, 1u | 0x8000u | (0xffffu << 16));
            return;
        }
        if (pix_ok) {
            const size_t at = (size_t)(lty * GSR_TILE_PX + (wave >> 1) * 8 + (lane >> 3)) * a.width + (size_t)(tx * GSR_TILE_PX + (wave & 1) * 8 + (lane & 7));
            const float4 c = out[at];
            C01 = (gsr_v2f){c.x, c.y}; C2 = c.z; T = a.tbuf[at];
            if constexpr (AOV) Z = aov[at].x;
        }
        wave_done = __all(!pix_ok || T < GSR_T_MIN);
    }
    bool u_done = false;
    uint32_t my_last_u = 0;
    uint32_t es_u = 0xffu;
    bool u_all = false;
    uint32_t fetched = 0;


    int scan_pos = 0;
    uint32_t q_head = 0, q_tail = 0;
    int spar = 0;
    uint32_t zlim = 0xffffffffu;
    const bool zfilter = HAS_DEPTH && a.tile_dmax != nullptr && a.idx_mask != 0xffffffffu && !tile_plain && !(a.flags & GSR_FLAG_NO_DEPTH_CLASS);
    if (zfilter) zlim = (gsr_zq(a.tile_dmax[gty * a.tiles_x + tx], a.zq0, a.zqs) << GSR_ZQ_SHIFT) | a.idx_mask;
    uint32_t imask = HAS_DEPTH ? a.idx_mask : 0xffffffffu;
    if (HAS_DEPTH) asm volatile("" : "+s"(imask));
    const uint32_t sub_mask = (1u << a.super_shift) - 1u;
    const uint32_t tile_bits = (1u << ((tx & sub_mask) >> a.rect_shift)) | (0x10000u << ((gty & sub_mask) >> a.rect_shift));
    typedef uint32_t gsr_u4 __attribute__((ext_vector_type(4), aligned(8)));
    gsr_u4 preA = {0u, 0u, 0u, 0u}, preB = {0u, 0u, 0u, 0u};
    auto prefetch = [&]() __attribute__((always_inline)) {
        const int i = scan_pos + 4 * tid;
        if (i < n) {
            const gsr_u4* src = reinterpret_cast<const gsr_u4*>(svals + s + i);
            preA = src[0]; preB = src[1];
        }
    };
    prefetch();
    int round = 0;
    int first_hit_step = -1;
    bool saturated = false;

    auto ext_steps_of = [&](uint32_t c) __attribute__((always_inline)) -> uint32_t {
        const int cur = (scan_pos >> 10) - 1;
        if (c == 0u) return 0u;
        if (cur < 0) return 0xffu;
        const int ln = (int)__builtin_amdgcn_mbcnt_hi(~0u, __builtin_amdgcn_mbcnt_lo(~0u, 0u));
        const bool reached = ln < 32 && cur - ln >= 0 && stail[(cur - ln) & 31] >= c;
        const unsigned long long m = __ballot(reached);
        const int k = __builtin_ctzll(~m | (1ull << 63));
        const int e = cur - (k - 1) + 1;
        return (m & 1ull) == 0ull || e <= 0 || e > 0xfe ? 0xffu : (uint32_t)e;
    };
    auto init_depth = [&]() __attribute__((always_inline)) {
        d_init = true;
        u_done = __all(!pix_ok || T < GSR_T_MIN || dpx < 1.0f);
        d_triv = __all(dpx >= 1.0f) && !(a.flags & GSR_FLAG_NO_DEPTH_CLASS);
        if (a.flags & GSR_FLAG_NO_DEPTH_CLASS) {
            d_wmin = -__builtin_inff();
        } else if (!d_triv) {
            const float ninf = -__builtin_inff();
            float vmin = pix_ok ? (dpx == dpx ? dpx : ninf) : __builtin_inff();
#pragma unroll
            for (int d = 32; d > 0; d >>= 1) vmin = __builtin_fminf(vmin, __shfl_xor(vmin, d, 64));
            d_wmin = __builtin_bit_cast(float, __builtin_amdgcn_readfirstlane(__builtin_bit_cast(int, vmin)));
        }
    };
    BLP(0)
    for (;;) {
        bool scanned_any = false;
        constexpr int batch = BL_BATCH;
        while ((int)(q_tail - q_head) < batch && scan_pos < n) {
            const int rem = n - (scan_pos + 4 * tid);
            bool h0 = rem > 0 && (preA.y & tile_bits) == tile_bits, h1 = rem > 1 && (preA.w & tile_bits) == tile_bits;
            bool h2 = rem > 2 && (preB.y & tile_bits) == tile_bits, h3 = rem > 3 && (preB.w & tile_bits) == tile_bits;
            if (HAS_DEPTH) { h0 = h0 && preA.x <= zlim; h1 = h1 && preA.z <= zlim; h2 = h2 && preB.x <= zlim; h3 = h3 && preB.z <= zlim; }
            const unsigned long long b0 = __ballot(h0), b1 = __ballot(h1), b2 = __ballot(h2), b3 = __ballot(h3);
            uint32_t pos = 0;
            pos = __builtin_amdgcn_mbcnt_hi((uint32_t)(b0 >> 32), __builtin_amdgcn_mbcnt_lo((uint32_t)b0, pos));
            pos = __builtin_amdgcn_mbcnt_hi((uint32_t)(b1 >> 32), __builtin_amdgcn_mbcnt_lo((uint32_t)b1, pos));
            pos = __builtin_amdgcn_mbcnt_hi((uint32_t)(b2 >> 32), __builtin_amdgcn_mbcnt_lo((uint32_t)b2, pos));
            pos = __builtin_amdgcn_mbcnt_hi((uint32_t)(b3 >> 32), __builtin_amdgcn_mbcnt_lo((uint32_t)b3, pos));
            const uint32_t wtot = (uint32_t)(__builtin_popcountll(b0) + __builtin_popcountll(b1) + __builtin_popcountll(b2) +
                                             __builtin_popcountll(b3));
            if (lane == 0) scnt[spar][wave] = wtot;
            __syncthreads();
            const uint4 wt = *reinterpret_cast<const uint4*>(scnt[spar]);
            pos += q_tail + (wave > 0 ? wt.x : 0u) + (wave > 1 ? wt.y : 0u) + (wave > 2 ? wt.z : 0u);
            if (h0) { q[pos & (BL_QCAP - 1)] = preA.x; ++pos; }
            if (h1) { q[pos & (BL_QCAP - 1)] = preA.z; ++pos; }
            if (h2) { q[pos & (BL_QCAP - 1)] = preB.x; ++pos; }
            if (h3) { q[pos & (BL_QCAP - 1)] = preB.z; }
            q_tail += wt.x + wt.y + wt.z + wt.w;
            if (tid == 0) stail[(scan_pos >> 10) & 31] = q_tail;
            if (first_hit_step < 0 && q_tail != 0u) first_hit_step = scan_pos >> 10;
            scan_pos += 1024;
            spar ^= 1;
            scanned_any = true;
            prefetch();
        }
        if (scanned_any) __syncthreads();
        BLP(1)

        const int avail = (int)(q_tail - q_head);
        const int take = avail < batch ? avail : batch;
        if (take == 0) break;
        fetched += (uint32_t)take;
        BLP(2)
        if (HAS_DEPTH && !d_init) init_depth();
        if (!wave_done) {
            for (int sub = 0; sub < take; sub += 64) {
                my_last = q_head + (uint32_t)(sub + 64 < take ? sub + 64 : take);
                const bool have = sub + lane < take;
                float w_max = __builtin_inff(), w_min = -__builtin_inff();
                if (HAS_DEPTH && !d_triv && !(a.flags & GSR_FLAG_NO_DEPTH_CLASS)) {
                    const bool live = pix_ok && T >= GSR_T_MIN;
                    const float dl = dpx == dpx ? dpx : -__builtin_inff();
                    float vmax = live ? dl : -__builtin_inff();
#pragma unroll
                    for (int d = 32; d > 0; d >>= 1) vmax = __builtin_fmaxf(vmax, __shfl_xor(vmax, d, 64));
                    w_max = __builtin_bit_cast(float, __builtin_amdgcn_readfirstlane(__builtin_bit_cast(int, vmax)));
                    w_min = d_wmin;
                }
                float4 r1, r2;
                float rz = 0.0f, c0 = 0.0f, c1 = 0.0f;
                bool hit = false, pending = false, dtest = false, dmet_l = false;
                if (have) {
                    const uint32_t ridx = q[(q_head + (uint32_t)(sub + lane)) & (BL_QCAP - 1)] & imask;
                    const float4* p = reinterpret_cast<const float4*>(recs + ridx);
                    const float4 r0 = p[0];
                    r1 = p[1]; r2 = p[2];
                    rz = (AOV || (HAS_DEPTH && !d_triv)) ? zwin[ridx] : 0.0f;
                    const float rqk = (((a.flags & GSR_FLAG_NO_ALPHA_RADIUS) ? 2.0f : gsr_support_radius_from_la(r2.w)) + 1.0e-3f) * GSR_KAPPA;
                    const float ddx = qcx - r0.x, ddy = qcy - r0.y;
                    const bool box = __builtin_fmaxf(__builtin_fabsf(ddx) - r0.z, __builtin_fabsf(ddy) - r0.w) <= 3.5f;
                    const float lim1 = rqk + 3.5f * (__builtin_fabsf(r1.x) + __builtin_fabsf(r1.y));
                    const float lim2 = rqk + 3.5f * (__builtin_fabsf(r1.z) + __builtin_fabsf(r1.w));
                    const float pu = __builtin_fabsf(ddx * r1.x + ddy * r1.y);
                    const float pv = __builtin_fabsf(ddx * r1.z + ddy * r1.w);
                    hit = box && (((a.flags & GSR_FLAG_NO_SAT) != 0) || (pu <= lim1 && pv <= lim2));
                    if (HAS_DEPTH && !d_triv) {
                        dmet_l = hit && !(rz <= d_wmin && (a.near_alpha - rz) >= a.near_scale * (a.near_alpha - d_wmin));
                        hit = hit && (rz <= w_max);
                        dtest = hit && !(rz <= w_min);
                    }
                    pending = __builtin_bit_cast(uint32_t, r2.x) == GSR_COLOUR_PENDING;
                    if (LAZY) {
                        if (hit && pending) gsr_splat_colour_from_row(lz.f, lz.colrow, ridx, r2.x, r2.y, r2.z);
                    }
                    const float d0x = tcx0 - r0.x, d0y = tcy0 - r0.y;
                    c0 = gsr_fma(d0x, r1.x, d0y * r1.y);
                    c1 = gsr_fma(d0x, r1.z, d0y * r1.w);
                }
                if (!LAZY && __any(pending)) {
                    if (lane == 0) sredo = 1u;
                    wave_done = true;
                    break;
                }
                const unsigned long long bal = __ballot(hit);
                const int cnt = (int)__builtin_popcountll(bal);
                const bool dslow = HAS_DEPTH && __any(dtest);
                if (HAS_DEPTH && __any(dmet_l)) d_met = true;
                if (hit) {
                    const uint32_t pos = __builtin_amdgcn_mbcnt_hi((uint32_t)(bal >> 32), __builtin_amdgcn_mbcnt_lo((uint32_t)bal, 0u));
                    float* blk = reinterpret_cast<float*>(&slist[wave][(pos >> 1) * PF4]);
                    const uint32_t h = pos & 1u;
                    blk[0 + h] = r1.x; blk[2 + h] = r1.y; blk[4 + h] = r1.z; blk[6 + h] = r1.w;
                    blk[8 + h] = c0; blk[10 + h] = c1;
                    reinterpret_cast<float4*>(blk)[3 + h] = r2;
                    if (ZSTAGE) reinterpret_cast<float*>(&szl[wave][pos >> 1])[h] = rz;
                }
                if ((cnt & 1) && lane == 0) {
                    float* blk = reinterpret_cast<float*>(&slist[wave][(cnt >> 1) * PF4]);
                    blk[1] = 0.0f; blk[3] = 0.0f; blk[5] = 0.0f; blk[7] = 0.0f;
                    blk[9] = 0.0f; blk[11] = 0.0f;
                    {
                        typedef volatile __attribute__((address_space(3))) float lds_vfloat;
// ... 98 lines not shown
        q_head += (uint32_t)take;
        const int rpar = round & 1;
        const int wv = __builtin_amdgcn_readfirstlane(wave);
        if (HAS_DEPTH && wave_done && !u_done) { u_done = true; my_last_u = my_last; }
        if (HAS_DEPTH && zfilter) {
            const bool live = pix_ok && T >= GSR_T_MIN && !wave_done;
            float vmax = live ? (dpx == dpx ? dpx : -__builtin_inff()) : -__builtin_inff();
#pragma unroll
            for (int d = 32; d > 0; d >>= 1) vmax = __builtin_fmaxf(vmax, __shfl_xor(vmax, d, 64));
            if (lane == 0) swmax[rpar][wv] = vmax;
        }
        if (lane == 0) { sdone[rpar][wv] = (wave_done ? 1u : 0u) | ((HAS_DEPTH ? u_done : wave_done) ? 2u : 0u); slast[wv] = my_last; if (HAS_DEPTH) slastu[wv] = my_last_u; }
        ++round;
        BLP(5)
        __syncthreads();
        BLP(6)
        if (!LAZY && sredo) {
            int t3 = tile;
            asm volatile("" : "+s"(t3));
            if (tid == 0 && lz.redo) lz.redo[atomicAdd(lz.redo_count, 1u)] = t3;
            return;
        }
        if (HAS_DEPTH && zfilter) {
            const float tm = __builtin_fmaxf(__builtin_fmaxf(swmax[rpar][0], swmax[rpar][1]), __builtin_fmaxf(swmax[rpar][2], swmax[rpar][3]));
            zlim = (gsr_zq(tm, a.zq0, a.zqs) << GSR_ZQ_SHIFT) | a.idx_mask;
        }
        const uint32_t dall = sdone[rpar][0] & sdone[rpar][1] & sdone[rpar][2] & sdone[rpar][3];
        if (HAS_DEPTH && !u_all && (dall & 2u)) {
            u_all = true;
            es_u = ext_steps_of(max(max(slastu[0], slastu[1]), max(slastu[2], slastu[3])));
        }
        if ((dall & 1u) != 0u) { saturated = true; break; }
    }
    if (pix_ok) {
        int t2 = tid;
        asm volatile("" : "+v"(t2));
        const int w2 = t2 >> 6, l2 = t2 & 63;
        const int brow = lty * GSR_TILE_PX + (w2 >> 1) * 8 + (l2 >> 3);
        const int bcol = tx * GSR_TILE_PX + (w2 & 1) * 8 + (l2 & 7);
        const size_t at = (size_t)brow * a.width + bcol;
        if constexpr (OVER) {
            float4 B = make_float4(bg->rgba[0], bg->rgba[1], bg->rgba[2], bg->rgba[3]);
            if (bg->kind == GSR_BGK_IMAGE) {
                const int grow = gsr_shard_global_row(a.shard, lty) * GSR_TILE_PX + (w2 >> 1) * 8 + (l2 >> 3);
                B = gsr_background_pixel(bg->image, bg->format, (size_t)grow * a.width + bcol);
            }
            const float4 S = make_float4(C01.x, C01.y, C2, 1.0f - T);
            if (a.slab == 1) { out[at] = S; a.tbuf[at] = T; }
            const float4 o = gsr_composite_over_pixel(S, B);
            if (a.out_format == GSR_FMT_RGBA32F) reinterpret_cast<float4*>(a.out_packed)[at] = o;
            else gsr_store_packed(a.out_packed, a.out_format, at, o.x, o.y, o.z, o.w);
        } else {
            if (a.out_format == GSR_FMT_RGBA32F || a.slab == 1) out[at] = make_float4(C01.x, C01.y, C2, 1.0f - T);
            if (a.out_format != GSR_FMT_RGBA32F) gsr_store_packed(a.out_packed, a.out_format, at, C01.x, C01.y, C2, 1.0f - T);
            if (a.slab == 1) a.tbuf[at] = T;
        }
        if constexpr (AOV) aov[at] = make_float2(Z, 1.0f - T);
    }
    BLP(8)
#ifdef BL_PROFILE
    if (lane == 0 && blockIdx.x < BLP_MAX_WG) {
        unsigned long long* o = g_blend_prof[blockIdx.x][wave];
#pragma unroll
        for (int i = 0; i < 9; ++i) o[i] = prof[i];
        o[9] = 1ull; o[10] = (unsigned long long)round; o[11] = wall0; o[12] = wall_clock64();
        o[13] = occ_lanes; o[14] = occ_evals; o[15] = occ_half | (occ_none << 32);
    }
#endif
    __syncthreads();
    if (lane == 0) { atomicAdd(&sevals, my_evals); if (HAS_DEPTH && d_met) sdmet = 1u; }
    __syncthreads();
    if (HAS_DEPTH && !d_init) init_depth();
    const uint32_t es_c = ext_steps_of(max(max(slast[0], slast[1]), max(slast[2], slast[3])));
    if (!HAS_DEPTH) { u_all = saturated; es_u = es_c; }
    else if (!u_all) {
        const uint32_t dl = sdone[(round - 1) & 1][0] & sdone[(round - 1) & 1][1] & sdone[(round - 1) & 1][2] & sdone[(round - 1) & 1][3];
        if (round > 0 ? (dl & 2u) != 0u : __syncthreads_and(u_done ? 1 : 0) != 0) { u_all = true; es_u = round > 0 ? ext_steps_of(max(max(slastu[0], slastu[1]), max(slastu[2], slastu[3]))) : 0u; }
    }
    if (tid == 0) {
        const int rd = scan_pos + 1024;
        const uint32_t fs = (uint32_t)(first_hit_step < 0 ? 0 : (first_hit_step > 0x1fff ? 0x1fff : first_hit_step)) | (sdmet ? 0x2000u : 0u);
        const uint4 tw = make_uint4((uint32_t)(rd < n ? rd : n), fetched, sevals, (saturated ? 1u : 0u) | (fs << 1) | (u_all ? 0x8000u : 0u) | (es_c << 16) | (es_u << 24));
        tile_work[tile] = tw;
        if (a.sup_work && gsr_tile_weight(tw)) atomicAdd(&a.sup_work[st], gsr_tile_weight(tw));
    }
}

template <bool HAS_DEPTH>
__global__ void __launch_bounds__(256) BL_OCC
k_blend(GsrBlendArgs a, const int32_t* __restrict__ tile_map, const uint2* __restrict__ svals,
        const int32_t* __restrict__ sstart, const int32_t* __restrict__ send,
        const GsrRecord* __restrict__ recs, float4* __restrict__ out, uint4* __restrict__ tile_work,
        const float* __restrict__ zwin, const float* __restrict__ depth, GsrLazyArgs lz)
{
    gsr_blend_tile<HAS_DEPTH, false>(a, tile_map, svals, sstart, send, recs, out, tile_work, zwin, depth, lz);
}
template <bool HAS_DEPTH>
__global__ void __launch_bounds__(256)
k_blend_lazy(GsrBlendArgs a, const int32_t* __restrict__ tile_map, const uint2* __restrict__ svals,
             const int32_t* __restrict__ sstart, const int32_t* __restrict__ send,
             const GsrRecord* __restrict__ recs, float4* __restrict__ out, uint4* __restrict__ tile_work,
             const float* __restrict__ zwin, const float* __restrict__ depth, GsrLazyArgs lz)
{
    gsr_blend_tile<HAS_DEPTH, true>(a, tile_map, svals, sstart, send, recs, out, tile_work, zwin, depth, lz);
}

template <bool HAS_DEPTH>
__global__ void __launch_bounds__(256) BL_OCC
k_blend_aov(GsrBlendArgs a, const int32_t* __restrict__ tile_map, const uint2* __restrict__ svals,
            const int32_t* __restrict__ sstart, const int32_t* __restrict__ send,
            const GsrRecord* __restrict__ recs, float4* __restrict__ out, uint4* __restrict__ tile_work,
            const float* __restrict__ zwin, const float* __restrict__ depth, GsrLazyArgs lz, float2* __restrict__ aov)
{
    gsr_blend_tile<HAS_DEPTH, false, true>(a, tile_map, svals, sstart, send, recs, out, tile_work, zwin, depth, lz, aov);
}
template <bool HAS_DEPTH>
__global__ void __launch_bounds__(256)
k_blend_aov_lazy(GsrBlendArgs a, const int32_t* __restrict__ tile_map, const uint2* __restrict__ svals,
                 const int32_t* __restrict__ sstart, const int32_t* __restrict__ send,
                 const GsrRecord* __restrict__ recs, float4* __restrict__ out, uint4* __restrict__ tile_work,
                 const float* __restrict__ zwin, const float* __restrict__ depth, GsrLazyArgs lz, float2* __restrict__ aov)
{
    gsr_blend_tile<HAS_DEPTH, true, true>(a, tile_map, svals, sstart, send, recs, out, tile_work, zwin, depth, lz, aov);
}

template <bool HAS_DEPTH>
__global__ void __launch_bounds__(256) BL_OCC
k_blend_over(GsrBlendArgs a, const int32_t* __restrict__ tile_map, const uint2* __restrict__ svals,
             const int32_t* __restrict__ sstart, const int32_t* __restrict__ send,
             const GsrRecord* __restrict__ recs, float4* __restrict__ out, uint4* __restrict__ tile_work,
             const float* __restrict__ zwin, const float* __restrict__ depth, GsrLazyArgs lz, GsrBgArgs bg)
{
    gsr_blend_tile<HAS_DEPTH, false, false, true>(a, tile_map, svals, sstart, send, recs, out, tile_work, zwin, depth, lz, nullptr, &bg);
}
template <bool HAS_DEPTH>
__global__ void __launch_bounds__(256)
k_blend_over_lazy(GsrBlendArgs a, const int32_t* __restrict__ tile_map, const uint2* __restrict__ svals,
                  const int32_t* __restrict__ sstart, const int32_t* __restrict__ send,
                  const GsrRecord* __restrict__ recs, float4* __restrict__ out, uint4* __restrict__ tile_work,
                  const float* __restrict__ zwin, const float* __restrict__ depth, GsrLazyArgs lz, GsrBgArgs bg)
{
    gsr_blend_tile<HAS_DEPTH, true, false, true>(a, tile_map, svals, sstart, send, recs, out, tile_work, zwin, depth, lz, nullptr, &bg);
}

#ifdef SW_PROFILE
__device__ unsigned long long g_sw_prof[8];
#define SWP(i) { if (threadIdx.x == 0) g_sw_prof[i] = clock64(); }
#else
#define SWP(i)
#endif
#define SW_THREADS 256
#ifndef SW_HEADROOM_SHIFT
#define SW_HEADROOM_SHIFT 2
#endif
#ifndef SW_HEADROOM_ADD
#define SW_HEADROOM_ADD 1024u
#endif
struct GsrSumArgs {
    int32_t n_tiles, tiles_x, tiles_y , super_shift, stiles_x, n_super;
    GsrShard shard;
};
struct GsrHorizonArgs {
    float* raw;
    const float* pyr_in;
    float* pyr_out;
    int32_t pyr_off[GSR_PYR_LEVELS];
    int32_t culled;
    int32_t dilate;
    const uint2* lists;
    int32_t list_cap;
    const float4* geoA;
    float cam[3];
    unsigned long long* host_end;
    uint32_t ticket;
    int32_t slab;
    const uint4* tile_work_a;
    float* stat;
    int32_t stat_in_use;
    uint32_t idx_mask;
    int32_t depth_culled;
    uint32_t* dbg;
};
struct __attribute__((aligned(16))) GsrTilePartial {
    unsigned long long scanned, fetched, evals;
    uint32_t wmax, unsat, nused, nfin, viol, pad_;
};
__global__ void __launch_bounds__(64)
k_tile_pass(const uint4* __restrict__ tile_work, GsrSumArgs g, const int32_t* __restrict__ sstart, const int32_t* __restrict__ send,
            GsrHorizonArgs hz, GsrTilePartial* __restrict__ partial ,
            uint32_t* __restrict__ st_scan )
{
    const int lane = threadIdx.x;
    const int lx = (lane & 1) | ((lane >> 1) & 2) | ((lane >> 2) & 4), ly = ((lane >> 1) & 1) | ((lane >> 2) & 2) | ((lane >> 3) & 4);
    const int nbx = (g.tiles_x + 7) >> 3;
    const int b = (int)blockIdx.x, by = b / nbx, bx = b - by * nbx;
    const int tx = bx * 8 + lx, gty = by * 8 + ly;
    const bool inside = tx < g.tiles_x && gty < g.tiles_y;
    if (hz.raw && b == 0) {
        const int n45 = gsr_pyr_dim(g.tiles_x, 4) * gsr_pyr_dim(g.tiles_y, 4) + gsr_pyr_dim(g.tiles_x, 5) * gsr_pyr_dim(g.tiles_y, 5);
        for (int i = lane; i < n45; i += 64) hz.pyr_out[hz.pyr_off[4] + i] = 0.0f;
    }
    bool own = false;
    int ti = 0, st = 0;
    if (inside && gsr_shard_owns(g.shard, gty)) {
        const int lty = gsr_shard_local_row(g.shard, gty);
        const int i = lty * g.tiles_x + tx;
        if (i < g.n_tiles) { own = true; ti = i; st = (gty >> g.super_shift) * g.stiles_x + (tx >> g.super_shift); }
    }
    uint4 w = tile_work[ti];
    uint4 wa = make_uint4(0u, 0u, 0u, 0u);
    if (hz.slab == 2 && own) wa = hz.tile_work_a[ti];
    const bool a_done = (wa.w & 1u) != 0u;
    if (a_done) w = make_uint4(0u, 0u, 0u, 0u);
    const int s0 = sstart[st];
    int e0 = send[st];
    float hold = __builtin_inff();
    if (hz.raw && hz.culled && inside)
        hold = gsr_pyr_max(hz.pyr_in, hz.pyr_off, g.tiles_x, max(tx - hz.dilate, 0), max(gty - hz.dilate, 0),
                           min(tx + hz.dilate, g.tiles_x - 1), min(gty + hz.dilate, g.tiles_y - 1));
    if (!own) { w = make_uint4(0u, 0u, 0u, 0u); hold = __builtin_inff(); }
    e0 = e0 < hz.list_cap ? e0 : hz.list_cap;
    const uint32_t len = (own && e0 > s0) ? (uint32_t)(e0 - s0) : 0u;
    const uint32_t es_all = (w.w >> 16) & 0xffu;
    const uint32_t rd_all = (es_all == 0xffu || (es_all << 10) > w.x) ? w.x : (es_all << 10);
    const bool opaque_all = own && (w.w & 1u) != 0u;
    const bool classic_now = opaque_all && (w.w & 0x4000u) == 0u;
    const bool pred_classic = !(hz.stat && hz.stat_in_use) || !inside || hz.stat[gty * g.tiles_x + tx] != 0.0f;
    const uint32_t es_u = w.w >> 24;
    const uint32_t rd_u = (es_u == 0xffu || (es_u << 10) > w.x) ? w.x : (es_u << 10);
    const uint32_t rdc = pred_classic ? rd_all : rd_u;
    const bool opaque_c = own && (pred_classic ? opaque_all : (classic_now || (w.w & 0x8000u) != 0u));
    const uint32_t rd = classic_now ? rd_all : rd_u;
    const bool opaque = own && (classic_now || (w.w & 0x8000u) != 0u);
    const uint32_t first = ((w.w >> 1) & 0x1fffu) << 10;
    const uint32_t want = rd + ((rd > first ? rd - first : 0u) >> 2) + 1024u;
    {
        const int gs = g.super_shift < 3 ? g.super_shift : 3;
        uint32_t m = opaque_all ? rd_all : 0u, open = (own && !opaque_all && !a_done) ? 1u : 0u, any = own ? 1u : 0u;
        for (int d = 1; d < (1 << (2 * gs)); d <<= 1) {
            const uint32_t om = __shfl_xor(m, d, 64), oo = __shfl_xor(open, d, 64), oa = __shfl_xor(any, d, 64);
            m = om > m ? om : m; open |= oo; any |= oa;
        }
        const int gst = (gty >> g.super_shift) * g.stiles_x + (tx >> g.super_shift);
        if ((lane & ((1 << (2 * gs)) - 1)) == 0 && any && gst < 256 && (tx >> g.super_shift) < g.stiles_x) {
            if (m) atomicMax(&st_scan[gst], m);
            if (open) st_scan[256 + gst] = 1u;
        }
    }
    uint32_t viol = 0u, nused = 0u, nfin = 0u;
    if (hz.raw) {
        const bool ok = opaque && rd > 0u && rd <= len;
        const bool c1 = opaque_c && rdc > 0u && rdc <= len && hold < 3.0e38f, c2 = ok && want < len;
        const uint32_t i1 = hz.lists[c1 ? (uint32_t)s0 + rdc - 1u : 0u].x & hz.idx_mask;
        const bool c3 = ok && !c2 && !(hold < 3.0e38f) && hz.depth_culled != 0;
        const uint32_t i2 = hz.lists[c2 ? (uint32_t)s0 + want : (c3 ? (uint32_t)s0 + len - 1u : 0u)].x & hz.idx_mask;
        const float4 P1 = hz.geoA[c1 ? i1 : 0u], P2 = hz.geoA[c2 ? i2 : 0u];
        float klast, hnew;
        { const float dx = P1.x - hz.cam[0], dy = P1.y - hz.cam[1], dz = P1.z - hz.cam[2]; klast = gsr_fma(dz, dz, gsr_fma(dy, dy, dx * dx)); }
        { const float dx = P2.x - hz.cam[0], dy = P2.y - hz.cam[1], dz = P2.z - hz.cam[2]; hnew = gsr_fma(dz, dz, gsr_fma(dy, dy, dx * dx)); }
        float h = 0.0f;
        if (own) {
            const bool none_c = opaque_c && !pred_classic && rdc == 0u;
            const bool none = opaque && !classic_now && rd == 0u;
            if (hold < 3.0e38f && !none_c && (!opaque_c || !c1 || !(klast <= hold))) viol = 1u;
            if (viol && hz.dbg) {
                const uint32_t k = atomicAdd(hz.dbg, 1u);
                if (k < 8u) {
                    uint32_t* o = hz.dbg + 1 + 8 * k;
                    o[0] = (uint32_t)tx; o[1] = (uint32_t)gty; o[2] = w.w; o[3] = w.x; o[4] = __float_as_uint(hold); o[5] = __float_as_uint(klast);
                    o[6] = (pred_classic ? 1u : 0u) | (opaque_c ? 2u : 0u) | (c1 ? 4u : 0u) | (classic_now ? 8u : 0u); o[7] = (rdc << 8) | (len > 0xffffffu ? 0xffu : 0u); 
                    o[7] = rdc; 
                }
            }
            h = __builtin_inff();
            if (none) h = 0.0f;
            else if (opaque) {
                if (c2) h = hnew;
                else if (hold < 3.0e38f) h = hold * 1.05f;
                else if (c3) h = hnew * 1.05f;
            }
        }
        if (inside && !a_done) hz.raw[gty * g.tiles_x + tx] = (own && !classic_now) ? -h : h;
    }
    if (own && len > 0u) { nused = 1u; if (opaque && rd > 0u && rd <= len && (unsigned long long)want * 10ull <= (unsigned long long)len * 7ull) nfin = 1u; }
    if (a_done) { nused = 1u; nfin = 1u; }
    unsigned long long sc = (unsigned long long)w.x + wa.x, fe = (unsigned long long)w.y + wa.y, ev = (unsigned long long)w.z + wa.z;
    uint32_t wmax = gsr_tile_weight(w) + gsr_tile_weight(wa), unsat = (own && !a_done && !(w.w & 1u) && (w.y || wa.y)) ? 1u : 0u;
#pragma unroll
    for (int d = 32; d > 0; d >>= 1) {
        sc += __shfl_down(sc, d, 64); fe += __shfl_down(fe, d, 64); ev += __shfl_down(ev, d, 64); unsat += __shfl_down(unsat, d, 64);
        nused += __shfl_down(nused, d, 64); nfin += __shfl_down(nfin, d, 64);
        { const uint32_t o = __shfl_down(wmax, d, 64); wmax = o > wmax ? o : wmax; }
    }
    const bool any_viol = __ballot(viol != 0u) != 0ull;
    if (lane == 0) {
        GsrTilePartial p;
        p.scanned = sc; p.fetched = fe; p.evals = ev; p.wmax = wmax; p.unsat = unsat; p.nused = nused; p.nfin = nfin;
        p.viol = any_viol ? 1u : 0u; p.pad_ = 0u;
        partial[b] = p;
    }
}

__global__ void __launch_bounds__(64)
k_slab_mid(const uint4* __restrict__ tile_work_a, GsrSumArgs g, const int32_t* __restrict__ sstart, const int32_t* __restrict__ send,
           GsrHorizonArgs hz ,
           float* __restrict__ pyr2 , const uint32_t* __restrict__ slab, uint32_t key_min)
{
    const int lane = threadIdx.x;
    const int lx = (lane & 1) | ((lane >> 1) & 2) | ((lane >> 2) & 4), ly = ((lane >> 1) & 1) | ((lane >> 2) & 2) | ((lane >> 3) & 4);
    const int nbx = (g.tiles_x + 7) >> 3;
    const int b = (int)blockIdx.x, by = b / nbx, bx = b - by * nbx;
    const int tx = bx * 8 + lx, gty = by * 8 + ly;
    const bool inside = tx < g.tiles_x && gty < g.tiles_y;
    bool own = false;
    int ti = 0, st = 0;
    if (inside && gsr_shard_owns(g.shard, gty)) {
        const int lty = gsr_shard_local_row(g.shard, gty);
        const int i = lty * g.tiles_x + tx;
        if (i < g.n_tiles) { own = true; ti = i; st = (gty >> g.super_shift) * g.stiles_x + (tx >> g.super_shift); }
    }
    const uint4 w = tile_work_a[ti];
    const int s0 = sstart[st];
    int e0 = send[st];
    e0 = e0 < hz.list_cap ? e0 : hz.list_cap;
    const bool opaque = own && (w.w & 1u) != 0u;
    {
        float v = inside ? ((own && !opaque) ? __builtin_inff() : 0.0f) : 0.0f;
        if (inside) pyr2[hz.pyr_off[0] + gty * g.tiles_x + tx] = v;
        v = __builtin_fmaxf(v, __shfl_xor(v, 1, 64)); v = __builtin_fmaxf(v, __shfl_xor(v, 2, 64));
        if ((lane & 3) == 0 && inside) pyr2[hz.pyr_off[1] + (gty >> 1) * gsr_pyr_dim(g.tiles_x, 1) + (tx >> 1)] = v;
        v = __builtin_fmaxf(v, __shfl_xor(v, 4, 64)); v = __builtin_fmaxf(v, __shfl_xor(v, 8, 64));
        if ((lane & 15) == 0 && inside) pyr2[hz.pyr_off[2] + (gty >> 2) * gsr_pyr_dim(g.tiles_x, 2) + (tx >> 2)] = v;
        v = __builtin_fmaxf(v, __shfl_xor(v, 16, 64)); v = __builtin_fmaxf(v, __shfl_xor(v, 32, 64));
        if (lane == 0) {
            pyr2[hz.pyr_off[3] + by * nbx + bx] = v;
            atomicMax(reinterpret_cast<uint32_t*>(pyr2) + hz.pyr_off[4] + (by >> 1) * gsr_pyr_dim(g.tiles_x, 4) + (bx >> 1), __float_as_uint(v));
            atomicMax(reinterpret_cast<uint32_t*>(pyr2) + hz.pyr_off[5] + (by >> 2) * gsr_pyr_dim(g.tiles_x, 5) + (bx >> 2), __float_as_uint(v));
        }
    }
    if (hz.raw) {
        const uint32_t len = (own && e0 > s0) ? (uint32_t)(e0 - s0) : 0u;
        const uint32_t es = (w.w >> 16) & 0xffu;
        const uint32_t rd = (es == 0xffu || (es << 10) > w.x) ? w.x : (es << 10);
        const uint32_t first = ((w.w >> 1) & 0x1fffu) << 10;
        const uint32_t want = rd + ((rd > first ? rd - first : 0u) >> 2) + 1024u;
        const bool c2 = opaque && rd > 0u && rd <= len && want < len;
        const uint32_t i2 = hz.lists[c2 ? (uint32_t)s0 + want : 0u].x & hz.idx_mask;
        const float4 P2 = hz.geoA[c2 ? i2 : 0u];
        const float dx = P2.x - hz.cam[0], dy = P2.y - hz.cam[1], dz = P2.z - hz.cam[2];
        const float hnew = gsr_fma(dz, dz, gsr_fma(dy, dy, dx * dx));
        const uint32_t ka = slab[0];
        const float slab_d2 = ka == 0xffffffffu ? __builtin_inff() : __builtin_bit_cast(float, ka + key_min);
        float h = 0.0f;
        if (own) h = !opaque ? __builtin_inff() : (c2 ? hnew : slab_d2 * 1.05f);
        if (inside) hz.raw[gty * g.tiles_x + tx] = (own && !(opaque && (w.w & 0x4000u) == 0u)) ? -h : h;
    }
}

__device__ __forceinline__ void
gsr_sum_work(const GsrTilePartial* __restrict__ partial, int nblocks, GsrSumArgs g, unsigned long long* __restrict__ counters,
           const uint32_t* __restrict__ n_visible, unsigned long long* __restrict__ summary ,
           uint32_t* __restrict__ prefix ,
           const uint32_t* __restrict__ redo_count ,
           uint32_t* __restrict__ colour_evals ,
           unsigned long long* __restrict__ colour_total ,
           const int32_t* __restrict__ sstart, const int32_t* __restrict__ send,
           uint32_t* __restrict__ lazy_hint ,
           uint32_t* __restrict__ sup_work_next ,
           GsrHorizonArgs hz, uint32_t* __restrict__ st_scan )
{
    SWP(0)
    __shared__ unsigned long long s_sum[3];
    __shared__ uint32_t s_unsat, s_est, s_cev, s_wmax, s_nfin, s_nused, s_viol;
    unsigned long long old2 = 0, old4 = 0, old5 = 0, old_ct = 0;
    uint32_t nvis = 0, nredo = 0, my_cev = 0, my_m = 0;
    int my_s0 = 0, my_e0 = 0;
    if (threadIdx.x == 0) {
        old2 = counters[2]; old4 = counters[4]; old5 = counters[5];
        nvis = *n_visible;
        nredo = redo_count ? *redo_count : 0u;
        if (colour_evals) old_ct = *colour_total;
        s_unsat = 0; s_est = 0; s_cev = 0; s_wmax = 0; s_nfin = 0; s_nused = 0; s_viol = 0;
    }
    if (threadIdx.x < 3) s_sum[threadIdx.x] = 0;
    if (colour_evals) my_cev = colour_evals[threadIdx.x];
    if ((int)threadIdx.x < g.n_super) { my_m = st_scan[threadIdx.x]; my_s0 = sstart[threadIdx.x]; my_e0 = send[threadIdx.x]; }
    unsigned long long sc = 0, fe = 0, ev = 0;
    uint32_t wmax = 0, unsat = 0, nused = 0, nfin = 0, viol = 0;
    for (int i = (int)threadIdx.x; i < nblocks; i += SW_THREADS) {
        const GsrTilePartial p = partial[i];
        sc += p.scanned; fe += p.fetched; ev += p.evals; unsat += p.unsat; nused += p.nused; nfin += p.nfin; viol |= p.viol;
        wmax = p.wmax > wmax ? p.wmax : wmax;
    }
    __syncthreads();
#pragma unroll
    for (int d = 32; d > 0; d >>= 1) {
        sc += __shfl_down(sc, d, 64); fe += __shfl_down(fe, d, 64); ev += __shfl_down(ev, d, 64); unsat += __shfl_down(unsat, d, 64);
        nused += __shfl_down(nused, d, 64); nfin += __shfl_down(nfin, d, 64);
        { const uint32_t o = __shfl_down(wmax, d, 64); wmax = o > wmax ? o : wmax; }
    }
    const bool any_viol = __ballot(viol != 0u) != 0ull;
    if ((threadIdx.x & 63) == 0) {
        atomicAdd(&s_sum[0], sc); atomicAdd(&s_sum[1], fe); atomicAdd(&s_sum[2], ev); atomicAdd(&s_unsat, unsat); atomicMax(&s_wmax, wmax);
        atomicAdd(&s_nused, nused); atomicAdd(&s_nfin, nfin);
        if (any_viol) s_viol = 1u;
    }
    __syncthreads();
    SWP(2)
    if (hz.host_end && threadIdx.x == 0) {
        uint32_t v = s_viol;
        *hz.host_end = ((unsigned long long)hz.ticket << 32) | (unsigned long long)(v ? GSR_END_HORIZON_BROKE : 0u);
        __threadfence_system();
    }
    if (sup_work_next) sup_work_next[threadIdx.x] = 0u;
    {
        const int st = (int)threadIdx.x;
        if (st < g.n_super) {
            st_scan[st] = 0u; st_scan[256 + st] = 0u;
            if (prefix) {
                const uint32_t len = my_e0 > my_s0 ? (uint32_t)(my_e0 - my_s0) : 0u;
                const uint32_t want = my_m + (my_m >> SW_HEADROOM_SHIFT) + SW_HEADROOM_ADD;
                atomicAdd(&s_est, want < len ? want : len);
                prefix[st] = want;
            }
        }
        if (colour_evals) {
            colour_evals[threadIdx.x] = 0u;
            if (my_cev) atomicAdd(&s_cev, my_cev);
        }
    }
    __syncthreads();
    SWP(4)
    if (threadIdx.x == 0) {
        const unsigned long long wsum = s_sum[2] * 32ull + s_sum[1] * 8ull + (s_sum[0] >> 1);
        const uint32_t order_pays = ((unsigned long long)s_wmax * 3072ull > wsum && wsum > 60000000ull) ? GSR_HINT_ORDER_PAYS : 0u;
        if (lazy_hint) *lazy_hint = ((prefix && (unsigned long long)s_est * 10ull < (unsigned long long)nvis * 4ull &&
                                      s_unsat * 64u <= (uint32_t)g.n_tiles) ? GSR_HINT_LAZY_PAYS : 0u) | order_pays |
                                    ((prefix && (unsigned long long)s_est * 3ull < (unsigned long long)nvis * 2ull) ? GSR_HINT_PREFIX_CHEAPER : 0u) |
                                    ((hz.culled || ((unsigned long long)s_nfin * 10ull >= (unsigned long long)s_nused * 3ull && s_nused > 0u)) ? GSR_HINT_CULL_PAYS : 0u);
        const unsigned long long t2 = old2 + s_sum[1], t4 = old4 + s_sum[0], t5 = old5 + s_sum[2];
        counters[1] = s_sum[1]; counters[2] = t2; counters[3] = s_sum[0]; counters[4] = t4; counters[5] = t5;
        if (colour_evals) *colour_total = old_ct + s_cev;
        summary[0] = 0ull; summary[1] = s_sum[1]; summary[2] = t2; summary[3] = s_sum[0]; summary[4] = t4; summary[5] = t5;
        summary[6] = (unsigned long long)nvis;
        summary[7] = (unsigned long long)nredo;
    }
    SWP(5)
}
__global__ void __launch_bounds__(SW_THREADS)
k_sum_work(const GsrTilePartial* __restrict__ partial, int nblocks, GsrSumArgs g, unsigned long long* __restrict__ counters,
           const uint32_t* __restrict__ n_visible, unsigned long long* __restrict__ summary, uint32_t* __restrict__ prefix,
           const uint32_t* __restrict__ redo_count, uint32_t* __restrict__ colour_evals, unsigned long long* __restrict__ colour_total,
           const int32_t* __restrict__ sstart, const int32_t* __restrict__ send, uint32_t* __restrict__ lazy_hint,
           uint32_t* __restrict__ sup_work_next, GsrHorizonArgs hz, uint32_t* __restrict__ st_scan)
{
    gsr_sum_work(partial, nblocks, g, counters, n_visible, summary, prefix, redo_count, colour_evals, colour_total, sstart, send, lazy_hint,
                 sup_work_next, hz, st_scan);
}

__device__ __forceinline__ void
gsr_horizon_dilate(const float* __restrict__ raw, int tiles_x, int tiles_y, int r, const GsrHorizonArgs& hz, float* __restrict__ pyr, const int b,
                   const int lane )
{
    const int lx = (lane & 1) | ((lane >> 1) & 2) | ((lane >> 2) & 4), ly = ((lane >> 1) & 1) | ((lane >> 2) & 2) | ((lane >> 3) & 4);
    const int nbx = (tiles_x + 7) >> 3;
    const int by = b / nbx, bx = b - by * nbx;
    const int tx = bx * 8 + lx, ty = by * 8 + ly;
    const bool inside = tx < tiles_x && ty < tiles_y;
    float v = 0.0f;
    if (inside) {
        const int x0 = max(tx - r, 0), x1 = min(tx + r, tiles_x - 1), y0 = max(ty - r, 0), y1 = min(ty + r, tiles_y - 1);
        bool allc = true;
        for (int y = y0; y <= y1; ++y)
            for (int x = x0; x <= x1; ++x) {
                const float rv = raw[y * tiles_x + x];
                v = __builtin_fmaxf(v, __builtin_fabsf(rv));
                allc = allc && (__float_as_uint(rv) >> 31) == 0u;
            }
        pyr[hz.pyr_off[0] + ty * tiles_x + tx] = v;
        if (hz.stat) hz.stat[ty * tiles_x + tx] = allc ? 1.0f : 0.0f;
    }
    v = __builtin_fmaxf(v, __shfl_xor(v, 1, 64)); v = __builtin_fmaxf(v, __shfl_xor(v, 2, 64));
    if ((lane & 3) == 0 && inside) pyr[hz.pyr_off[1] + (ty >> 1) * gsr_pyr_dim(tiles_x, 1) + (tx >> 1)] = v;
    v = __builtin_fmaxf(v, __shfl_xor(v, 4, 64)); v = __builtin_fmaxf(v, __shfl_xor(v, 8, 64));
    if ((lane & 15) == 0 && inside) pyr[hz.pyr_off[2] + (ty >> 2) * gsr_pyr_dim(tiles_x, 2) + (tx >> 2)] = v;
    v = __builtin_fmaxf(v, __shfl_xor(v, 16, 64)); v = __builtin_fmaxf(v, __shfl_xor(v, 32, 64));
    if (lane == 0) {
        pyr[hz.pyr_off[3] + by * nbx + bx] = v;
        atomicMax(reinterpret_cast<uint32_t*>(pyr) + hz.pyr_off[4] + (by >> 1) * gsr_pyr_dim(tiles_x, 4) + (bx >> 1), __float_as_uint(v));
        atomicMax(reinterpret_cast<uint32_t*>(pyr) + hz.pyr_off[5] + (by >> 2) * gsr_pyr_dim(tiles_x, 5) + (bx >> 2), __float_as_uint(v));
    }
}
__global__ void __launch_bounds__(64)
k_horizon_dilate(const float* __restrict__ raw, int tiles_x, int tiles_y, int r, GsrHorizonArgs hz, float* __restrict__ pyr)
{
    gsr_horizon_dilate(raw, tiles_x, tiles_y, r, hz, pyr, (int)blockIdx.x, (int)threadIdx.x);
}

__global__ void __launch_bounds__(SW_THREADS)
k_frame_end(const GsrTilePartial* __restrict__ partial, int nblocks, GsrSumArgs g, unsigned long long* __restrict__ counters,
            const uint32_t* __restrict__ n_visible, unsigned long long* __restrict__ summary, uint32_t* __restrict__ prefix,
            const uint32_t* __restrict__ redo_count, uint32_t* __restrict__ colour_evals, unsigned long long* __restrict__ colour_total,
            const int32_t* __restrict__ sstart, const int32_t* __restrict__ send, uint32_t* __restrict__ lazy_hint,
            uint32_t* __restrict__ sup_work_next, GsrHorizonArgs hz, uint32_t* __restrict__ st_scan, int dilate_r)
{
    if ((int)blockIdx.x == nblocks) {
        gsr_sum_work(partial, nblocks, g, counters, n_visible, summary, prefix, redo_count, colour_evals, colour_total, sstart, send, lazy_hint,
                     sup_work_next, hz, st_scan);
        return;
    }
    if (threadIdx.x >= 64) return;
    gsr_horizon_dilate(hz.raw, g.tiles_x, g.tiles_y, dilate_r, hz, hz.pyr_out, (int)blockIdx.x, (int)threadIdx.x);
}

#define TO_THREADS 1024
#define TO_LEVELS 128
__device__ __forceinline__ void
gsr_tile_order(const uint4* __restrict__ tile_work, const GsrSumArgs& g, int tiles_y, const uint32_t* __restrict__ sup_work, int cap,
               int32_t* __restrict__ order, const int xcd)
{
    __shared__ uint32_t s_sup[256];
    __shared__ uint32_t s_own[64];
    __shared__ uint32_t s_hist[TO_LEVELS];
    __shared__ uint32_t s_nown, s_wmax;
    const int tid = threadIdx.x, lane = tid & 63, wave = tid >> 6;
    if (tid < 256) s_sup[tid] = tid < g.n_super ? sup_work[tid] : 0u;
// ... 141 lines not shown
```

### houdini-gsplat-renderer_amd/engine.py

```python
from __future__ import annotations

import ctypes as C
import os

import numpy as np

from . import build as _build

_LIB = None


class GsrError(RuntimeError):
    def __init__(self, code: int, msg: str):
        super().__init__(f"gsplat_hip error {code}: {msg}")
        self.code = code


class gsr_camera(C.Structure):
    _fields_ = [("obj_view", C.c_float * 16), ("object", C.c_float * 16), ("inv_object", C.c_float * 16),
                ("view", C.c_float * 16), ("proj", C.c_float * 16), ("cam_pos", C.c_float * 3),
                ("width", C.c_int32), ("height", C.c_int32), ("sh_order", C.c_int32)]


class gsr_stats(C.Structure):
    _fields_ = [("n_splats", C.c_int64), ("n_visible", C.c_int64), ("pairs_total", C.c_int64),
                ("pairs_consumed", C.c_int64), ("tiles_x", C.c_int32), ("tiles_y", C.c_int32),
                ("record_bytes", C.c_int32), ("pair_bytes", C.c_int32),
                ("ms_preprocess", C.c_float), ("ms_depth_sort", C.c_float), ("ms_emit", C.c_float),
                ("ms_tile_sort", C.c_float), ("ms_blend", C.c_float), ("ms_total", C.c_float),
                ("blend_ms_total", C.c_double), ("blend_launches", C.c_int64),
                ("blend_pairs_consumed_total", C.c_int64), ("frame_ms_total", C.c_double), ("frames", C.c_int64),
                ("entries_scanned", C.c_int64), ("blend_entries_scanned_total", C.c_int64),
                ("super_tile", C.c_int32), ("stiles_x", C.c_int32), ("stiles_y", C.c_int32), ("reserved_", C.c_int32),
                ("blend_wave_evals_total", C.c_int64), ("stage_ms_total", C.c_double * 5),
                ("stage_frames", C.c_int64), ("sorts_skipped", C.c_int64), ("frames_requeued", C.c_int64),
                ("lazy_redo_tiles", C.c_int64), ("lazy_colours_total", C.c_int64), ("frames_truncated", C.c_int64),
                ("frames_culled", C.c_int64), ("frames_repaired", C.c_int64),
                ("clusters_total", C.c_int64), ("clusters_kept", C.c_int64),
                ("policy_bits", C.c_int32), ("cull_dilate", C.c_int32), ("cull_holdoff", C.c_int32), ("reserved2_", C.c_int32),
                ("frames_resorted", C.c_int64), ("frames_slab", C.c_int64), ("frames_jumped", C.c_int64), ("frames_lazy", C.c_int64),
                ("uploads", C.c_int64), ("upload_ms", C.c_double * 6),
                ("moves", C.c_int64), ("move_ms", C.c_double * 4)]

    def as_dict(self) -> dict:
        d = {n: getattr(self, n) for n, _ in self._fields_}
        d["stage_ms_total"] = list(self.stage_ms_total)
        d["upload_ms"] = list(self.upload_ms)
        d["move_ms"] = list(self.move_ms)
        return d


class gsr_debug_record(C.Structure):
    _fields_ = [(n, C.c_float) for n in
                ("cx", "cy", "a1x", "a1y", "b1x", "b1y", "hx", "hy", "r", "g", "b", "la", "key")] + \
               [("visible", C.c_int32)]


DEBUG_RECORD_DTYPE = np.dtype([(n, np.float32) for n in
                               ("cx", "cy", "a1x", "a1y", "b1x", "b1y", "hx", "hy", "r", "g", "b", "la", "key")]
                              + [("visible", np.int32)])


class GSplatRenderContext(C.Structure):
    _fields_ = [("obj_view", C.c_float * 16), ("object", C.c_float * 16), ("inv_object", C.c_float * 16),
                ("view", C.c_float * 16), ("proj", C.c_float * 16), ("width", C.c_int32), ("height", C.c_int32),
                ("target", C.c_void_p), ("target_is_device", C.c_int32),
                ("depth", C.c_void_p), ("depth_is_device", C.c_int32)]


class gsr_raw_attrs(C.Structure):
    _fields_ = [("P", C.c_void_p), ("Cd", C.c_void_p), ("alpha", C.c_void_p), ("scale", C.c_void_p), ("orient", C.c_void_p),
                ("sh_scheme", C.c_int32), ("sh_vec3_per_point", C.c_int32), ("sh_array", C.c_void_p), ("sh_ptr", C.POINTER(C.c_void_p))]


class gsr_background(C.Structure):
    _fields_ = [("kind", C.c_int32), ("format", C.c_int32), ("rgba", C.c_float * 4), ("image", C.c_void_p),
                ("image_is_device", C.c_int32), ("reserved_", C.c_int32)]


class gsr_attr_update(C.Structure):
    _fields_ = [("Cd", C.c_void_p), ("alpha", C.c_void_p), ("scale", C.c_void_p), ("orient", C.c_void_p),
                ("shx", C.c_void_p), ("shy", C.c_void_p), ("shz", C.c_void_p)]


class gsr_device_attrs(C.Structure):
    _fields_ = [("P", C.c_void_p), ("Cd", C.c_void_p), ("alpha", C.c_void_p), ("scale", C.c_void_p), ("orient", C.c_void_p),
                ("sh", C.c_void_p), ("sh_vec3_per_point", C.c_int32), ("reserved_", C.c_int32)]


class gsr_crop_volume(C.Structure):
    _fields_ = [("kind", C.c_int32), ("invert", C.c_int32), ("to_unit", C.c_float * 12)]


class gsr_visibility(C.Structure):
    _fields_ = [("n_volumes", C.c_int32), ("reserved_", C.c_int32), ("volume", gsr_crop_volume * 4),
                ("mask", C.c_void_p), ("mask_splats", C.c_int64)]


class gsplat_attrs(C.Structure):
    _fields_ = [("count", C.c_int64), ("P", C.c_void_p), ("Cd", C.c_void_p), ("opacity", C.c_void_p), ("Alpha", C.c_void_p),
                ("scale", C.c_void_p), ("orient", C.c_void_p), ("sh_coefficients", C.c_void_p),
                ("sh_coefficients_len", C.c_int32), ("sh", C.POINTER(C.c_void_p)), ("f_rest", C.POINTER(C.c_void_p)),
                ("sh_order", C.POINTER(C.c_int32)), ("explicit_camera_pos", C.POINTER(C.c_float))]


TRANSPORT_AUTO, TRANSPORT_RCCL, TRANSPORT_COPY = 0, 1, 2
MAX_DIM = 16384
MISSING_CD, MISSING_OPACITY, MISSING_SCALE, MISSING_ORIENT, MISSING_SH, BAD_SH_ORDER = 1, 2, 4, 8, 16, 32
OPT_XCD_SWIZZLE, OPT_STAGE_TIMING, OPT_SORT_CACHE, OPT_SUPER_TILE, OPT_DEBUG_FLAGS, OPT_FRAMES_IN_FLIGHT, OPT_DEFERRED_CHECK, OPT_LAZY_COLOUR, OPT_SHARD_LAYOUT = 1, 2, 3, 4, 5, 6, 7, 8, 9
OPT_OCCLUSION_CULL = 10
OPT_TIMING_EVERY = 11
OPT_CLUSTER_CULL = 12
OPT_STORAGE_ORDER = 13
OPT_CULL_DILATE = 14
OPT_LOCAL_SORT = 15
OPT_FRONT_SLAB = 16
OPT_ROW_WORK = 17
TILE = 16

TARGET_RGBA32F = 0
TARGET_RGBA16F = 1
TARGET_RGBA8 = 2
AOV_DEPTH = 1
BG_COLOUR = 1
BG_IMAGE = 2
VIS_MAX_VOLUMES = 4
VOL_BOX = 1
VOL_ELLIPSOID = 2
REMOVE_HIDDEN = 1
REMOVE_BLOCK = 4096
TARGET_DTYPES = {TARGET_RGBA32F: np.dtype(np.float32), TARGET_RGBA16F: np.dtype(np.float16), TARGET_RGBA8: np.dtype(np.uint8)}

C_ABI_SYMBOLS = [
    "gsr_device_count", "gsr_create", "gsr_destroy", "gsr_last_error", "gsr_version", "gsr_set_stream",
    "gsr_upload_begin", "gsr_upload_append", "gsr_upload_append_raw", "gsr_upload_end", "gsr_upload_abort", "gsr_upload", "gsr_set_row_shard", "gsr_band_rows",
    "gsr_stitch_bands", "gsr_render", "gsr_render_depth", "gsr_render_wire", "gsr_render_wire_over", "gsr_synchronize", "gsr_get_stats", "gsr_stats_reset", "gsr_set_option",
    "gsr_debug_read_records", "gsr_debug_read_depth_order", "gsr_debug_read_storage_order", "gsr_debug_read_tile_lists", "gsr_debug_sort_pairs", "gsr_debug_sort_pairs_local", "gsr_debug_policy", "gsr_debug_policy_state", "gsr_debug_frame_plan",
    "gsr_debug_read_tile_work", "gsr_debug_read_horizons", "gsr_debug_read_cull",
    "gsr_multi_create", "gsr_multi_destroy", "gsr_multi_count", "gsr_multi_transport", "gsr_multi_context",
    "gsr_multi_set_stream", "gsr_multi_set_option", "gsr_multi_upload_begin", "gsr_multi_upload_append",
    "gsr_multi_upload_end", "gsr_multi_upload_abort", "gsr_multi_upload", "gsr_multi_render", "gsr_multi_render_depth",
    "gsr_multi_synchronize", "gsr_multi_get_stats", "gsr_multi_comm_info", "gsr_multi_gather_stats",
    "gsr_comm_available", "gsr_comm_get_unique_id", "gsr_comm_init", "gsr_comm_info", "gsr_comm_destroy", "gsr_comm_render",
    "gsplat_renderer_create_multi", "gsplat_renderer_multi",
    "gsplat_prim_create", "gsplat_prim_destroy", "gsplat_prim_update", "gsplat_prim_render", "gsplat_prim_missing",
    "gsplat_prim_sh_order", "gsplat_prim_has_sh", "gsplat_prim_array",
    "gsplat_renderer_create", "gsplat_renderer_get_instance", "gsplat_renderer_destroy",
    "gsplat_renderer_register_update", "gsplat_renderer_include_in_render_pass",
    "gsplat_renderer_flush_entries_for_matching_detail", "gsplat_renderer_generate_render_geometry",
    "gsplat_renderer_render", "gsplat_renderer_post_render", "gsplat_renderer_redraw", "gsplat_renderer_set_rendering_enabled",
    "gsplat_renderer_set_explicit_camera_pos", "gsplat_renderer_set_spherical_harmonics_order",
    "gsplat_renderer_query", "gsplat_renderer_get_origin", "gsplat_renderer_get_last_camera_pos",
    "gsplat_renderer_engine", "gsplat_closest_sqrt_power_of_2", "gsplat_quantize_half",
    "gsplat_pack_sh_from_vec3", "gsplat_pack_sh_from_frest", "gsplat_pack_sh_from_array",
    "gsr_target_pixel_bytes", "gsr_set_target_format", "gsr_get_target_format", "gsr_multi_set_target_format", "gsr_convert_pixels",
    "gsplat_renderer_set_target_format", "gsplat_renderer_get_target_format",
    "gsr_render_aov", "gsr_resolve_depth", "gsr_resolve_depth_device", "gsplat_renderer_set_aov_target",
    "gsr_render_over", "gsr_composite_over", "gsplat_renderer_set_background",
    "gsr_update", "gsr_multi_update", "gsr_debug_read_resident", "gsplat_renderer_update_attributes", "gsplat_renderer_row_array",
    "gsr_move", "gsr_multi_move", "gsplat_renderer_move_splats",
    "gsr_upload_append_device", "gsr_update_device", "gsr_move_device", "gsr_debug_check_device_source",
    "gsr_set_row_band", "gsr_read_row_work", "gsr_debug_balance_rows", "gsr_multi_get_bands",
    "gsr_set_visibility", "gsr_get_visibility", "gsr_visibility_eval", "gsr_multi_set_visibility", "gsplat_renderer_set_visibility",
    "gsr_remove", "gsr_remove_map", "gsr_get_removal", "gsr_multi_remove",
    "gsr_add", "gsr_add_device", "gsr_add_capacity", "gsr_get_add", "gsr_multi_add",
]


def balance_rows(row_work, count: int, cur_first=None, min_gain_permille: int = 0):
    L = load_library()
    w = np.ascontiguousarray(row_work, dtype=np.uint32).reshape(-1)
    cur = None if cur_first is None else np.ascontiguousarray(cur_first, dtype=np.int32).reshape(-1)
    if cur is not None and cur.size != count + 1:
        raise ValueError("cur_first holds count + 1 boundaries")
    out = np.zeros(max(int(count), 0) + 1, np.int32)
    rc = L.gsr_debug_balance_rows(_ptr(w) if w.size else None, int(w.size), int(count), _ptr(cur), int(min_gain_permille), out.ctypes.data)
    _check(rc if rc < 0 else 0)
    return bool(rc), out


POLICY_FIELDS = ("cull_pays", "cull_weak", "vis_unculled", "cull_holdoff", "cull_backoff", "cull_streak", "cull_dilate", "opt_dilate",
                 "slab_holdoff", "local_fails", "local_holdoff")


def lib_path() -> str:
    return os.environ.get("GSR_LIBRARY") or _build.LIB


def load_library() -> C.CDLL:
    global _LIB
    if _LIB is not None:
        return _LIB
    path = lib_path()
    if not os.path.exists(path):
        raise GsrError(-100, f"{path} is missing: run __graft_entry__.build() (hipcc --offload-arch=gfx950) first")
    L = C.CDLL(path)
    vp, i32, i64, f32p = C.c_void_p, C.c_int, C.c_int64, C.POINTER(C.c_float)
    L.gsr_device_count.restype = i32
    L.gsr_last_error.restype = C.c_char_p
    L.gsr_version.restype = C.c_char_p
    L.gsr_create.argtypes = [i32, C.POINTER(vp)]
    L.gsr_destroy.argtypes = [vp]
    L.gsr_destroy.restype = None
    L.gsr_set_stream.argtypes = [vp, vp]
    L.gsr_upload_begin.argtypes = [vp, i64, i32, f32p]
    L.gsr_upload_append.argtypes = [vp, i64] + [vp] * 8
    L.gsr_upload_append_raw.argtypes = [vp, i64, C.POINTER(gsr_raw_attrs)]
    L.gsr_upload_end.argtypes = [vp]
    L.gsr_update.argtypes = [vp, i64, i64, C.POINTER(gsr_attr_update)]
    L.gsr_multi_update.argtypes = [vp, i64, i64, C.POINTER(gsr_attr_update)]
    L.gsr_move.argtypes = [vp, i64, i64, vp, f32p, C.POINTER(gsr_attr_update)]
    L.gsr_multi_move.argtypes = [vp, i64, i64, vp, f32p, C.POINTER(gsr_attr_update)]
    L.gsplat_renderer_move_splats.argtypes = [vp, C.c_char_p, vp, f32p] + [vp] * 7 + [C.POINTER(C.c_int64), C.POINTER(C.c_int64)]
    L.gsr_upload_append_device.argtypes = [vp, i64, C.POINTER(gsr_device_attrs)]
    L.gsr_update_device.argtypes = [vp, i64, i64, C.POINTER(gsr_device_attrs)]
    L.gsr_move_device.argtypes = [vp, i64, i64, f32p, C.POINTER(gsr_device_attrs)]
    L.gsr_debug_check_device_source.argtypes = [vp, vp, i64]
    L.gsr_debug_read_resident.argtypes = [vp, i32, vp, i64]
    L.gsr_set_visibility.argtypes = [vp, C.POINTER(gsr_visibility)]
    L.gsr_get_visibility.argtypes = [vp, C.POINTER(gsr_visibility), C.POINTER(C.c_int64)]
    L.gsr_visibility_eval.argtypes = [C.POINTER(gsr_visibility), vp, i64, i64, vp]
    L.gsr_multi_set_visibility.argtypes = [vp, C.POINTER(gsr_visibility)]
    L.gsplat_renderer_set_visibility.argtypes = [vp, C.POINTER(gsr_visibility)]
    L.gsr_remove.argtypes = [vp, vp, i32, i32, C.POINTER(C.c_int64)]
    L.gsr_remove_map.argtypes = [vp, i64, vp, C.POINTER(C.c_int64)]
    L.gsr_get_removal.argtypes = [vp, C.POINTER(C.c_int64), C.POINTER(C.c_int64), C.POINTER(C.c_double)]
    L.gsr_multi_remove.argtypes = [vp, vp, i32, C.POINTER(C.c_int64)]
    L.gsr_add.argtypes = [vp, i64] + [vp] * 8 + [C.POINTER(C.c_int64)]
    L.gsr_add_device.argtypes = [vp, i64, C.POINTER(gsr_device_attrs), C.POINTER(C.c_int64)]
    L.gsr_add_capacity.argtypes = [i64, i64]
    L.gsr_add_capacity.restype = i64
    L.gsr_get_add.argtypes = [vp] + [C.POINTER(C.c_int64)] * 4 + [C.POINTER(C.c_double)]
    L.gsr_multi_add.argtypes = [vp, i64] + [vp] * 8 + [C.POINTER(C.c_int64)]
    L.gsplat_renderer_update_attributes.argtypes = [vp, C.c_char_p] + [vp] * 7 + [C.POINTER(C.c_int64), C.POINTER(C.c_int64)]
    L.gsplat_renderer_row_array.argtypes = [vp, C.c_char_p, i32]
    L.gsplat_renderer_row_array.restype = vp
    L.gsr_upload_abort.argtypes = [vp]
    L.gsr_upload.argtypes = [vp, i64] + [vp] * 8 + [f32p]
    L.gsr_set_row_shard.argtypes = [vp, i32, i32]
    L.gsr_band_rows.argtypes = [i32, i32, i32]
    L.gsr_stitch_bands.argtypes = [vp, vp, i32, i32, i32, vp]
    L.gsr_render.argtypes = [vp, C.POINTER(gsr_camera), vp, i32]
    L.gsr_render_depth.argtypes = [vp, C.POINTER(gsr_camera), vp, i32, vp, i32]
    L.gsr_render_aov.argtypes = [vp, C.POINTER(gsr_camera), vp, i32, vp, i32, i32, vp]
    L.gsr_resolve_depth.argtypes = [vp, i64, C.c_float, vp]
    L.gsr_resolve_depth_device.argtypes = [vp, vp, i64, C.c_float, vp]
    L.gsplat_renderer_set_aov_target.argtypes = [vp, i32, vp]
    L.gsr_render_over.argtypes = [vp, C.POINTER(gsr_camera), vp, i32, C.POINTER(gsr_background), vp, i32]
    L.gsr_composite_over.argtypes = [vp, i64, C.POINTER(gsr_background), i32, vp]
    L.gsplat_renderer_set_background.argtypes = [vp, C.POINTER(gsr_background)]
    L.gsr_render_wire.argtypes = [vp, C.POINTER(gsr_camera), vp, i32]
    L.gsr_render_wire_over.argtypes = [vp, C.POINTER(gsr_camera), vp, i32]
    L.gsr_synchronize.argtypes = [vp]
    L.gsr_get_stats.argtypes = [vp, C.POINTER(gsr_stats)]
    L.gsr_stats_reset.argtypes = [vp]
    L.gsr_set_option.argtypes = [vp, i32, i32]
    L.gsr_debug_read_records.argtypes = [vp, vp, i64]
    L.gsr_debug_read_depth_order.argtypes = [vp, vp, i64, C.POINTER(C.c_int64)]
    L.gsr_debug_read_cull.argtypes = [vp, vp, i64, vp, i64, C.POINTER(C.c_int64)]
    L.gsr_debug_read_tile_lists.argtypes = [vp, vp, vp, i64, vp, i64]
    L.gsr_debug_read_storage_order.argtypes = [vp, vp, i64]
    L.gsr_debug_sort_pairs.argtypes = [vp, vp, vp, i64, i32]
    L.gsr_debug_sort_pairs_local.argtypes = [vp, vp, vp, i64, i32, C.c_uint32, i32]
    L.gsr_debug_policy.argtypes = [vp, i32, C.c_longlong, C.c_longlong]
    L.gsr_debug_policy_state.argtypes = [vp, vp]
    L.gsr_debug_frame_plan.argtypes = [i32, vp, vp, vp]
    L.gsr_debug_read_tile_work.argtypes = [vp, vp, i64]
    L.gsr_debug_read_horizons.argtypes = [vp, vp, i64]
    L.gsr_target_pixel_bytes.argtypes = [i32]
    L.gsr_set_target_format.argtypes = [vp, i32]
    L.gsr_get_target_format.argtypes = [vp]
    L.gsr_multi_set_target_format.argtypes = [vp, i32]
    L.gsr_convert_pixels.argtypes = [vp, i64, i32, vp]
    L.gsplat_renderer_set_target_format.argtypes = [vp, i32]
    L.gsplat_renderer_get_target_format.argtypes = [vp]
    L.gsplat_renderer_create.restype = vp
    L.gsplat_renderer_create.argtypes = [i32]
    L.gsplat_renderer_get_instance.restype = vp
    L.gsplat_renderer_destroy.argtypes = [vp]
    L.gsplat_renderer_destroy.restype = None
    L.gsplat_renderer_register_update.argtypes = [vp, C.c_uint64, C.POINTER(C.c_int64), i64, i64, f32p] + [vp] * 8 + \
                                                 [i64, C.c_char_p, i32]
    L.gsplat_renderer_include_in_render_pass.argtypes = [vp, C.c_char_p]
    L.gsplat_renderer_include_in_render_pass.restype = None
    L.gsplat_renderer_flush_entries_for_matching_detail.argtypes = [vp, C.c_char_p]
    L.gsplat_renderer_flush_entries_for_matching_detail.restype = None
    L.gsplat_renderer_generate_render_geometry.argtypes = [vp, C.POINTER(GSplatRenderContext)]
    L.gsplat_renderer_generate_render_geometry.restype = None
    L.gsplat_renderer_render.argtypes = [vp, C.POINTER(GSplatRenderContext), i32]
    L.gsplat_renderer_render.restype = None
    L.gsplat_renderer_post_render.argtypes = [vp]
    L.gsplat_renderer_post_render.restype = None
    L.gsplat_renderer_redraw.argtypes = [vp, C.POINTER(C.c_char_p), i32, C.POINTER(GSplatRenderContext), i32]
    L.gsplat_renderer_redraw.restype = None
    L.gsplat_renderer_set_rendering_enabled.argtypes = [vp, i32]
    L.gsplat_renderer_set_rendering_enabled.restype = None
    L.gsplat_renderer_set_explicit_camera_pos.argtypes = [vp, f32p]
    L.gsplat_renderer_set_explicit_camera_pos.restype = None
    L.gsplat_renderer_set_spherical_harmonics_order.argtypes = [vp, i32]
    L.gsplat_renderer_set_spherical_harmonics_order.restype = None
    L.gsplat_renderer_query.argtypes = [vp, i32, C.c_char_p]
    L.gsplat_renderer_query.restype = i64
    L.gsplat_renderer_get_origin.argtypes = [vp, f32p]
    L.gsplat_renderer_get_origin.restype = None
    L.gsplat_renderer_get_last_camera_pos.argtypes = [vp, f32p]
    L.gsplat_renderer_get_last_camera_pos.restype = None
    L.gsplat_renderer_engine.argtypes = [vp]
    L.gsplat_renderer_engine.restype = vp
    L.gsplat_closest_sqrt_power_of_2.argtypes = [i32]
    L.gsplat_closest_sqrt_power_of_2.restype = C.c_uint
    L.gsplat_quantize_half.argtypes = [vp, vp, i64]
    L.gsplat_quantize_half.restype = None
    L.gsplat_pack_sh_from_vec3.argtypes = [C.POINTER(vp), i64, vp, vp, vp]
    L.gsplat_pack_sh_from_vec3.restype = None
    L.gsplat_pack_sh_from_frest.argtypes = [C.POINTER(vp), i64, vp, vp, vp]
    L.gsplat_pack_sh_from_frest.restype = None
    L.gsplat_pack_sh_from_array.argtypes = [vp, i64, i32, vp, vp, vp]
    L.gsplat_pack_sh_from_array.restype = None
    L.gsr_multi_create.argtypes = [C.POINTER(C.c_int), i32, i32, C.POINTER(vp)]
    L.gsr_multi_destroy.argtypes = [vp]
    L.gsr_multi_destroy.restype = None
    L.gsr_multi_count.argtypes = [vp]
    L.gsr_multi_transport.argtypes = [vp]
    L.gsr_multi_context.argtypes = [vp, i32]
    L.gsr_multi_context.restype = vp
    L.gsr_multi_set_stream.argtypes = [vp, vp]
    L.gsr_multi_set_option.argtypes = [vp, i32, i32]
    L.gsr_multi_upload_begin.argtypes = [vp, i64, i32, f32p]
    L.gsr_multi_upload_append.argtypes = [vp, i64] + [vp] * 8
    L.gsr_multi_upload_end.argtypes = [vp]
    L.gsr_multi_upload_abort.argtypes = [vp]
    L.gsr_multi_upload.argtypes = [vp, i64] + [vp] * 8 + [f32p]
    L.gsr_multi_render.argtypes = [vp, C.POINTER(gsr_camera), vp, i32]
    L.gsr_multi_render_depth.argtypes = [vp, C.POINTER(gsr_camera), vp, i32, vp, i32]
    L.gsr_multi_synchronize.argtypes = [vp]
    L.gsr_multi_get_stats.argtypes = [vp, i32, C.POINTER(gsr_stats)]
    L.gsr_multi_comm_info.argtypes = [vp, C.POINTER(C.c_int), C.POINTER(C.c_int)]
    L.gsr_set_row_band.argtypes = [vp, i32, i32]
    L.gsr_read_row_work.argtypes = [vp, vp, i32, C.POINTER(C.c_int64)]
    L.gsr_debug_balance_rows.argtypes = [vp, i32, i32, vp, i32, vp]
    L.gsr_multi_get_bands.argtypes = [vp, vp, C.POINTER(C.c_int64)]
    L.gsr_multi_gather_stats.argtypes = [vp, i32, C.POINTER(C.c_double), C.POINTER(C.c_int64)]
    L.gsr_comm_info.argtypes = [vp, C.POINTER(C.c_int), C.POINTER(C.c_int)]
    L.gsr_comm_get_unique_id.argtypes = [vp]
    L.gsr_comm_init.argtypes = [vp, vp, i32, i32]
    L.gsr_comm_destroy.argtypes = [vp]
    L.gsr_comm_render.argtypes = [vp, C.POINTER(gsr_camera), vp, i32, vp]
    L.gsplat_renderer_create_multi.argtypes = [C.POINTER(C.c_int), i32, i32]
    L.gsplat_renderer_create_multi.restype = vp
    L.gsplat_renderer_multi.argtypes = [vp]
# ... 587 lines not shown
    def render_struct_to_host(self, cam_struct: gsr_camera, host_ptr: int):
        _check(self.L.gsr_render(self.h, C.byref(cam_struct), C.c_void_p(host_ptr), 0))

    def render_struct_depth_to_device(self, cam_struct: gsr_camera, depth_device_ptr: int, device_ptr: int):
        _check(self.L.gsr_render_depth(self.h, C.byref(cam_struct), C.c_void_p(depth_device_ptr), 1, C.c_void_p(device_ptr), 1))

    def stitch_bands(self, gathered_ptr: int, count: int, width: int, height: int, out_ptr: int):
        _check(self.L.gsr_stitch_bands(self.h, C.c_void_p(gathered_ptr), count, width, height, C.c_void_p(out_ptr)))

    def comm_unique_id(self) -> bytes:
        buf = C.create_string_buffer(128)
        _check(self.L.gsr_comm_get_unique_id(buf))
        return buf.raw

    def comm_init(self, unique_id: bytes, rank: int, world: int):
        _check(self.L.gsr_comm_init(self.h, C.c_char_p(unique_id), int(rank), int(world)))
        self.shard = (rank, world)

    def comm_render(self, cam_struct: gsr_camera, out_ptr: int, depth_ptr: int = 0):
        _check(self.L.gsr_comm_render(self.h, C.byref(cam_struct), C.c_void_p(depth_ptr or None), 1, C.c_void_p(out_ptr or None)))

    def comm_info(self):
        r, n = C.c_int(-1), C.c_int(0)
        _check(self.L.gsr_comm_info(self.h, C.byref(r), C.byref(n)))
        return r.value, n.value

    def comm_destroy(self):
        _check(self.L.gsr_comm_destroy(self.h))
        self.shard = (0, 1)

    def synchronize(self):
        _check(self.L.gsr_synchronize(self.h))

    def stats(self) -> dict:
        st = gsr_stats()
        _check(self.L.gsr_get_stats(self.h, C.byref(st)))
        return st.as_dict()

    def stats_reset(self):
        _check(self.L.gsr_stats_reset(self.h))

    def debug_records(self, n: int) -> np.ndarray:
        out = np.zeros(n, dtype=DEBUG_RECORD_DTYPE)
        _check(self.L.gsr_debug_read_records(self.h, out.ctypes.data, n))
        return out

    def debug_cull(self, n: int):
        rect = np.zeros(n, dtype=np.uint32)
        nclus = (n + 63) // 64
        clus = np.zeros(max(nclus, 1), dtype=np.uint32)
        cnt = C.c_int64()
        _check(self.L.gsr_debug_read_cull(self.h, rect.ctypes.data, n, clus.ctypes.data, nclus, C.byref(cnt)))
        assert cnt.value <= nclus
        return rect, clus[:cnt.value]

    def debug_depth_order(self, n: int) -> np.ndarray:
        out = np.zeros(n, dtype=np.int32)
        cnt = C.c_int64()
        _check(self.L.gsr_debug_read_depth_order(self.h, out.ctypes.data, n, C.byref(cnt)))
        return out[:cnt.value]

    def debug_storage_order(self, n: int) -> np.ndarray:
        out = np.zeros(n, dtype=np.int32)
        _check(self.L.gsr_debug_read_storage_order(self.h, out.ctypes.data, n))
        return out

    def debug_tile_lists(self):
        st = self.stats()
        nt = st["stiles_x"] * st["stiles_y"]
        npairs = st["pairs_total"]
        ts = np.zeros(nt, np.int32)
        te = np.zeros(nt, np.int32)
        pv = np.zeros(max(npairs, 1), np.int32)
        _check(self.L.gsr_debug_read_tile_lists(self.h, ts.ctypes.data, te.ctypes.data, nt, pv.ctypes.data, npairs))
        return ts, te, pv[:npairs]

    def debug_tile_work(self) -> np.ndarray:
        st = self.stats()
        nt = st["tiles_x"] * st["tiles_y"]
        out = np.zeros((nt, 4), np.uint32)
        _check(self.L.gsr_debug_read_tile_work(self.h, out.ctypes.data, nt))
        return out.reshape(st["tiles_y"], st["tiles_x"], 4)

    def debug_horizons(self, tiles_x: int, tiles_y: int) -> np.ndarray:
        out = np.zeros((4, tiles_y, tiles_x), np.float32)
        _check(self.L.gsr_debug_read_horizons(self.h, out.ctypes.data, tiles_x * tiles_y))
        return out

    def debug_sort_pairs(self, keys: np.ndarray, vals: np.ndarray, key_bits: int = 32, local=None):
        k = np.ascontiguousarray(keys, dtype=np.uint32).copy()
        v = np.ascontiguousarray(vals, dtype=np.uint32).copy()
        if local is None:
            _check(self.L.gsr_debug_sort_pairs(self.h, k.ctypes.data, v.ctypes.data, k.shape[0], key_bits))
        else:
            _check(self.L.gsr_debug_sort_pairs_local(self.h, k.ctypes.data, v.ctypes.data, k.shape[0], key_bits, int(local[0]), int(local[1])))
        return k, v


class GSplatRenderer:

    Q_REGISTRY_SIZE, Q_ACTIVE_STAGED, Q_SPLAT_COUNT, Q_CAN_RENDER, Q_STAGING_COUNT, Q_RENDER_COUNT, Q_SH_PRESENT, \
        Q_LAST_STATUS, Q_ENTRY_AGE, Q_ENTRY_AGE_SINCE_ACTIVE = range(10)

    def __init__(self, device=0, transport: int = TRANSPORT_AUTO):
        self.L = load_library()
        if isinstance(device, (list, tuple)):
            arr = (C.c_int * len(device))(*[int(d) for d in device])
            self.h = self.L.gsplat_renderer_create_multi(arr, len(device), int(transport))
        else:
            self.h = self.L.gsplat_renderer_create(int(device))
        if not self.h:
            raise GsrError(-3, self.L.gsr_last_error().decode("utf-8", "replace") or "gsplat_renderer_create failed")
        self._keep = {}
        self._updates = {}

    def close(self):
        if getattr(self, "h", None):
            self.L.gsplat_renderer_destroy(self.h)
            self.h = None

    def __del__(self):
        try:
            self.close()
        except Exception:
            pass

    def registerUpdate(self, gdp: int, gversion, gVtxOffset: int, splats, splatOrigin=None) -> str:
        a = _Arrays(splats)
        origin = splats.barycenter() if splatOrigin is None else splatOrigin
        ver = (C.c_int64 * 4)(*[int(x) for x in gversion])
        buf = C.create_string_buffer(256)
        p = a.ptrs()
        n = self.L.gsplat_renderer_register_update(self.h, int(gdp), ver, int(gVtxOffset), a.n, _f3(origin), *p,
                                                   a.n if a.shx is not None else 0, buf, 256)
        if n < 0:
            raise GsrError(n, "registerUpdate failed")
        rid = buf.value.decode()
        self._keep[rid] = a
        detail = rid.split("__", 1)[0] + "__"
        for k in [k for k in self._updates if k == rid or (k.startswith(detail) and k.rsplit("__", 1)[-1] != rid.rsplit("__", 1)[-1])]:
            del self._updates[k]
        return rid

    def updateAttributes(self, rid: str, Cd=None, alpha=None, scale=None, orient=None, shx=None, shy=None, shz=None):
        given = dict(Cd=Cd, alpha=alpha, scale=scale, orient=orient, shx=shx, shy=shy, shz=shz)
        u, n, keep = attr_update_struct(**given)
        first, cnt = C.c_int64(0), C.c_int64(0)
        rc = int(self.L.gsplat_renderer_update_attributes(self.h, rid.encode(), u.Cd, u.alpha, u.scale, u.orient, u.shx, u.shy, u.shz,
                                                          C.byref(first), C.byref(cnt)))
        what = {"Cd": 1, "alpha": 2, "scale": 3, "orient": 4, "shx": 5, "shy": 6, "shz": 7}
        names = [k for k, _, _ in UPDATE_ATTRS if given[k] is not None]
        for k, a in zip(names, keep):
            if self.rowArray(rid, what[k]) == a.ctypes.data:
                self._updates.setdefault(rid, {})[k] = a
        return rc, first.value, cnt.value

    def moveSplats(self, rid: str, P, origin=None, Cd=None, alpha=None, scale=None, orient=None, shx=None, shy=None, shz=None):
        given = dict(Cd=Cd, alpha=alpha, scale=scale, orient=orient, shx=shx, shy=shy, shz=shz)
        P, n, u, keep = move_arrays(P, **given)
        first, cnt = C.c_int64(0), C.c_int64(0)
        rc = int(self.L.gsplat_renderer_move_splats(self.h, rid.encode(), P.ctypes.data, None if origin is None else _f3(origin),
                                                    u.Cd, u.alpha, u.scale, u.orient, u.shx, u.shy, u.shz, C.byref(first), C.byref(cnt)))
        what = {"P": 0, "Cd": 1, "alpha": 2, "scale": 3, "orient": 4, "shx": 5, "shy": 6, "shz": 7}
        names = ["P"] + [k for k, _, _ in UPDATE_ATTRS if given[k] is not None]
        for k, a in zip(names, [P] + keep):
            if self.rowArray(rid, what[k]) == a.ctypes.data:
# ... 286 lines not shown
```

### include/gsplat_hip.h

```cpp
#ifndef GSPLAT_HIP_H
#define GSPLAT_HIP_H

#include <stdint.h>

#ifdef __cplusplus
extern "C" {
#endif

#define GSR_OK                0
#define GSR_E_INVALID        -1
#define GSR_E_HIP            -2
#define GSR_E_NO_DEVICE      -3
#define GSR_E_NO_GEOMETRY    -4
#define GSR_E_TOO_MANY_PAIRS -5
#define GSR_E_OOM            -6
#define GSR_E_COMM           -7

#define GSR_TILE              16
#define GSR_MAX_DIM           16384
#define GSR_MAX_PAIRS         0x7fffff00ll

typedef struct gsr_context gsr_context;

typedef struct gsr_camera {
    float obj_view[16];
    float object[16];
    float inv_object[16];
    float view[16];
    float proj[16];
    float cam_pos[3];
    int32_t width;
    int32_t height;
    int32_t sh_order;
} gsr_camera;

typedef struct gsr_stats {
    int64_t n_splats;
    int64_t n_visible;
    int64_t pairs_total;
    int64_t pairs_consumed;
    int32_t tiles_x, tiles_y;
    int32_t record_bytes;
    int32_t pair_bytes;
    float ms_preprocess, ms_depth_sort, ms_emit, ms_tile_sort, ms_blend, ms_total;
    double blend_ms_total;
    int64_t blend_launches;
    int64_t blend_pairs_consumed_total;
    double frame_ms_total;
    int64_t frames;
    int64_t entries_scanned;
    int64_t blend_entries_scanned_total;
    int32_t super_tile;
    int32_t stiles_x, stiles_y;
    int32_t reserved_;
    int64_t blend_wave_evals_total;
    double stage_ms_total[5];
    int64_t stage_frames;
    int64_t sorts_skipped;
    int64_t frames_requeued;
    int64_t lazy_redo_tiles;
    int64_t lazy_colours_total;
    int64_t frames_truncated;
    int64_t frames_culled;
    int64_t frames_repaired;
    int64_t clusters_total;
    int64_t clusters_kept;
    int32_t policy_bits;
    int32_t cull_dilate;
    int32_t cull_holdoff;
    int32_t reserved2_;
    int64_t frames_resorted;
    int64_t frames_slab;
    int64_t frames_jumped;
    int64_t frames_lazy;
    int64_t uploads;
    double upload_ms[6];
    int64_t moves;
    double move_ms[4];
} gsr_stats;

int  gsr_device_count(void);
int  gsr_create(int device, gsr_context** out);
void gsr_destroy(gsr_context* ctx);
const char* gsr_last_error(void);
const char* gsr_version(void);

int  gsr_set_stream(gsr_context* ctx, void* hip_stream);

#define GSR_TARGET_RGBA32F    0
#define GSR_TARGET_RGBA16F    1
#define GSR_TARGET_RGBA8      2
int  gsr_target_pixel_bytes(int format);
int  gsr_set_target_format(gsr_context* ctx, int format);
int  gsr_get_target_format(gsr_context* ctx);
int  gsr_convert_pixels(const float* rgba32f, int64_t n_pixels, int format, void* out);

int  gsr_upload_begin(gsr_context* ctx, int64_t total_splats, int has_sh, const float origin[3]);
int  gsr_upload_append(gsr_context* ctx, int64_t n,
                       const float* P, const uint16_t* Cd, const float* alpha,
                       const uint16_t* scale, const uint16_t* orient,
                       const uint16_t* shx, const uint16_t* shy, const uint16_t* shz);
typedef struct gsr_raw_attrs {
    const float* P;
    const float* Cd;
    const float* alpha;
    const float* scale;
    const float* orient;
    int32_t sh_scheme;
    int32_t sh_vec3_per_point;
    const float* sh_array;
    const float* const* sh_ptr;
} gsr_raw_attrs;
int  gsr_upload_append_raw(gsr_context* ctx, int64_t n, const gsr_raw_attrs* attrs);
int  gsr_upload_end(gsr_context* ctx);
int  gsr_upload_abort(gsr_context* ctx);
int  gsr_upload(gsr_context* ctx, int64_t n,
                const float* P, const uint16_t* Cd, const float* alpha,
                const uint16_t* scale, const uint16_t* orient,
                const uint16_t* shx, const uint16_t* shy, const uint16_t* shz,
                const float origin[3]);

typedef struct gsr_attr_update {
    const uint16_t* Cd;
    const float*    alpha;
    const uint16_t* scale;
    const uint16_t* orient;
    const uint16_t *shx, *shy, *shz;
} gsr_attr_update;
int  gsr_update(gsr_context* ctx, int64_t first, int64_t n, const gsr_attr_update* u);

int  gsr_move(gsr_context* ctx, int64_t first, int64_t n, const float* P, const float origin[3], const gsr_attr_update* u);

typedef struct gsr_device_attrs {
    const float* P;
    const float* Cd;
    const float* alpha;
    const float* scale;
    const float* orient;
    const float* sh;
    int32_t sh_vec3_per_point;
    int32_t reserved_;
} gsr_device_attrs;
int  gsr_upload_append_device(gsr_context* ctx, int64_t n, const gsr_device_attrs* a);
int  gsr_update_device(gsr_context* ctx, int64_t first, int64_t n, const gsr_device_attrs* a);
int  gsr_move_device(gsr_context* ctx, int64_t first, int64_t n, const float origin[3], const gsr_device_attrs* a);
int  gsr_debug_check_device_source(gsr_context* ctx, const void* p, int64_t bytes);

#define GSR_VIS_MAX_VOLUMES 4
#define GSR_VOL_BOX         1
#define GSR_VOL_ELLIPSOID   2
typedef struct gsr_crop_volume {
    int32_t kind;
    int32_t invert;
// ... 64 lines not shown
int  gsr_multi_render_depth(gsr_multi* m, const gsr_camera* cam, const float* depth, int depth_is_device,
                            float* rgba_out, int out_is_device);
int  gsr_multi_synchronize(gsr_multi* m);
int  gsr_multi_get_stats(gsr_multi* m, int rank, gsr_stats* out);
#define GSR_MULTI_BALANCE_PERIOD 24
#define GSR_MULTI_BALANCE_GAIN   150
int  gsr_multi_get_bands(gsr_multi* m, int32_t* first, int64_t* rebalances);

#define GSR_COMM_ID_BYTES 128
int  gsr_comm_available(void);
int  gsr_comm_get_unique_id(void* id);
int  gsr_comm_init(gsr_context* ctx, const void* id, int rank, int world);
int  gsr_comm_info(gsr_context* ctx, int* rank, int* nranks);
int  gsr_comm_destroy(gsr_context* ctx);
int  gsr_comm_render(gsr_context* ctx, const gsr_camera* cam, const float* depth, int depth_is_device,
                     float* rgba_out_device);

int  gsr_render(gsr_context* ctx, const gsr_camera* cam, float* rgba_out, int out_is_device);

int  gsr_render_depth(gsr_context* ctx, const gsr_camera* cam, const float* depth, int depth_is_device,
                      float* rgba_out, int out_is_device);

#define GSR_AOV_DEPTH 1
int  gsr_render_aov(gsr_context* ctx, const gsr_camera* cam, const float* depth, int depth_is_device,
                    float* rgba_out, int out_is_device, int aov, float* aov_out);
int  gsr_resolve_depth(const float* aov, int64_t n_pixels, float cov_min, float* depth_out);
int  gsr_resolve_depth_device(gsr_context* ctx, const float* aov, int64_t n_pixels, float cov_min, float* depth_out);

#define GSR_BG_COLOUR 1
#define GSR_BG_IMAGE  2
typedef struct gsr_background {
    int32_t kind;
    int32_t format;
    float   rgba[4];
    const void* image;
    int32_t image_is_device;
    int32_t reserved_;
} gsr_background;
int  gsr_render_over(gsr_context* ctx, const gsr_camera* cam, const float* depth, int depth_is_device,
                     const gsr_background* bg, float* rgba_out, int out_is_device);
int  gsr_composite_over(const float* rgba32f, int64_t n_pixels, const gsr_background* bg,
                        int out_format, void* out);

int  gsr_render_wire(gsr_context* ctx, const gsr_camera* cam, float* rgba_out, int out_is_device);
int  gsr_render_wire_over(gsr_context* ctx, const gsr_camera* cam, float* rgba_inout, int is_device);

int  gsr_synchronize(gsr_context* ctx);
int  gsr_get_stats(gsr_context* ctx, gsr_stats* out);
int  gsr_stats_reset(gsr_context* ctx);

#define GSR_OPT_XCD_SWIZZLE     1
#define GSR_OPT_STAGE_TIMING    2
#define GSR_OPT_SORT_CACHE      3
#define GSR_OPT_SUPER_TILE      4
#define GSR_OPT_FRAMES_IN_FLIGHT 6
#define GSR_OPT_DEBUG_FLAGS     5
#define GSR_OPT_DEFERRED_CHECK   7
#define GSR_OPT_ROW_WORK        17
#define GSR_OPT_SHARD_LAYOUT     9
#define GSR_OPT_TIMING_EVERY    11
#define GSR_OPT_OCCLUSION_CULL  10
#define GSR_OPT_LAZY_COLOUR      8
#define GSR_OPT_CLUSTER_CULL    12
#define GSR_OPT_STORAGE_ORDER   13
#define GSR_OPT_CULL_DILATE     14
#define GSR_OPT_LOCAL_SORT      15
#define GSR_OPT_FRONT_SLAB      16
int  gsr_set_option(gsr_context* ctx, int option, int value);

typedef struct gsr_debug_record {
    float cx, cy, a1x, a1y, b1x, b1y, hx, hy, r, g, b, la;
    float key;
    int32_t visible;
} gsr_debug_record;
int  gsr_debug_read_records(gsr_context* ctx, gsr_debug_record* out, int64_t n);
int  gsr_debug_read_cull(gsr_context* ctx, uint32_t* rect, int64_t n, uint32_t* clusters, int64_t cap, int64_t* n_clusters);
int  gsr_debug_read_depth_order(gsr_context* ctx, int32_t* perm, int64_t cap, int64_t* n_sorted);
int  gsr_debug_read_storage_order(gsr_context* ctx, int32_t* perm, int64_t n);
int  gsr_debug_read_resident(gsr_context* ctx, int which, void* out, int64_t bytes);
int  gsr_debug_read_tile_lists(gsr_context* ctx, int32_t* list_start, int32_t* list_end, int64_t n_lists,
                               int32_t* pair_splat, int64_t n_pairs);

int  gsr_debug_read_tile_work(gsr_context* ctx, uint32_t* work4, int64_t n_tiles);
int  gsr_debug_read_horizons(gsr_context* ctx, float* out4, int64_t n_tiles);

int  gsr_debug_sort_pairs(gsr_context* ctx, uint32_t* keys, uint32_t* vals, int64_t n, int key_bits);
int  gsr_debug_sort_pairs_local(gsr_context* ctx, uint32_t* keys, uint32_t* vals, int64_t n, int key_bits,
                                uint32_t bucket_lo, int bucket_shift);
int  gsr_debug_policy(int32_t* state16, int event, long long a, long long b);
int  gsr_debug_policy_state(gsr_context* ctx, int32_t* state16);
int  gsr_debug_frame_plan(int which, const int32_t* in, int32_t* policy16, int32_t* out);

#ifdef __cplusplus
}
#endif
#endif
```

Before: 4564.

## Publish culling verdict per tile block early and record last-blended splat per tile

The horizon-violation verdict used to be written once by the summary kernel after every tile block finished. Now each 8x8 tile block writes its own ticketed word to mapped host memory as soon as it computes its result, and the host scans those words incrementally. This lets the CPU act on the verdict earlier instead of waiting for the whole reduction. The blend kernel also keeps a small shared ring of recent splat indices and writes a per-tile last-contributing splat record. That adds extra shared memory, per-step work and a global store in the hot blend loop.

```diff
diff --git a/houdini-gsplat-renderer_amd/csrc/gsr_api.hip b/houdini-gsplat-renderer_amd/csrc/gsr_api.hip
--- a/houdini-gsplat-renderer_amd/csrc/gsr_api.hip
+++ b/houdini-gsplat-renderer_amd/csrc/gsr_api.hip
@@ -127,6 +127,7 @@
     size_t pair_cap = 0;
     int32_t *sstart = nullptr, *send = nullptr;
     uint4* tile_work = nullptr;
+    uint2* tile_last = nullptr;
     size_t tile_cap = 0;
     uint4* tile_work_a = nullptr;
     float* tbuf = nullptr;
@@ -160,6 +161,8 @@
     GsrSlotHints hints;
     GsrLocalSortPolicy local_pol;
     unsigned long long* h_end = nullptr;
+    uint32_t verdict_ticket = 0;
+    bool verdict_broke = false;
     unsigned long long* h_rows = nullptr;
     unsigned long long* h_rows_dev = nullptr;
     uint32_t rows_ticket = 0;
@@ -394,8 +397,9 @@
     ok = ok && hipMemset(sl.bkt_cnt, 0, (size_t)BK_BUCKETS * BK_STRIDE * sizeof(uint32_t)) == hipSuccess;
     ok = ok && hipMalloc(reinterpret_cast<void**>(&sl.d_counts), 4 * sizeof(uint32_t)) == hipSuccess;
     ok = ok && hipMemset(sl.d_counts, 0, 4 * sizeof(uint32_t)) == hipSuccess;
-    ok = ok && hipHostMalloc(reinterpret_cast<void**>(&sl.h_end), sizeof(unsigned long long), hipHostMallocMapped | hipHostMallocCoherent) == hipSuccess;
-    if (ok) sl.h_end[0] = 0ull;
+    static_assert(GSR_VERDICT_WORDS_MAX == (GSR_MAX_TILES_SIDE / 8) * (GSR_MAX_TILES_SIDE / 8), "one verdict word per 8x8 block of the largest frame");
+    ok = ok && hipHostMalloc(reinterpret_cast<void**>(&sl.h_end), (size_t)GSR_VERDICT_WORDS_MAX * sizeof(unsigned long long), hipHostMallocMapped | hipHostMallocCoherent) == hipSuccess;
+    if (ok) std::memset(sl.h_end, 0, (size_t)GSR_VERDICT_WORDS_MAX * sizeof(unsigned long long));
     ok = ok && hipHostGetDevicePointer(reinterpret_cast<void**>(&sl.h_end_dev), sl.h_end, 0) == hipSuccess;
     ok = ok && hipMalloc(reinterpret_cast<void**>(&sl.st_scan), 512 * sizeof(uint32_t)) == hipSuccess;
     ok = ok && hipMemset(sl.st_scan, 0, 512 * sizeof(uint32_t)) == hipSuccess;
@@ -454,7 +458,7 @@
     slot_free_splat_arrays(sl);
     dev_free(sl.hist); dev_free(sl.totals);
     dev_free(sl.pvA);
-    dev_free(sl.sstart); dev_free(sl.send); dev_free(sl.tile_work); dev_free(sl.order); dev_free(sl.sup_work); sl.fb.release(); dev_free(sl.fb32); sl.aovb.release(); sl.bgb.release();
+    dev_free(sl.sstart); dev_free(sl.send); dev_free(sl.tile_work); dev_free(sl.tile_last); dev_free(sl.order); dev_free(sl.sup_work); sl.fb.release(); dev_free(sl.fb32); sl.aovb.release(); sl.bgb.release();
     dev_free(sl.hpyr); dev_free(sl.hpyr_next); dev_free(sl.hraw); dev_free(sl.hstat); dev_free(sl.hpyr2); dev_free(sl.slab); dev_free(sl.tile_work_a); dev_free(sl.tbuf); dev_free(sl.ccnt); dev_free(sl.bkt_key); dev_free(sl.bkt_val); dev_free(sl.bkt_cnt); dev_free(sl.d_counts); dev_free(sl.st_scan); dev_free(sl.partial);
     if (sl.h_end) (void)hipHostFree(sl.h_end); if (sl.h_rows) (void)hipHostFree(sl.h_rows); sl.depth_stage.release(); dev_free(sl.dpyr); dev_free(sl.dactive);
     dev_free(sl.redo); dev_free(sl.lazy_ctr); dev_free(sl.colour_evals);
@@ -1877,7 +1881,7 @@
     a.out_format = j.format; a.out_packed = (j.format != GSR_TARGET_RGBA32F || over) ? (void*)j.target : nullptr;
     float4* tgt = reinterpret_cast<float4*>((j.format != GSR_TARGET_RGBA32F || over) ? sl.fb32 : j.target);
     auto launch = [&](auto kernel, unsigned g, const int32_t* map, uint4* work, auto... tail) {
-        hipLaunchKernelGGL(kernel, dim3(g), dim3(256), 0, s, a, map, sl.pvA, sl.sstart, sl.send, sl.rec, tgt, work, sl.zwin, j.d_depth, lz, tail...);
+        hipLaunchKernelGGL(kernel, dim3(g), dim3(256), 0, s, a, map, sl.pvA, sl.sstart, sl.send, sl.rec, tgt, work, sl.zwin, j.d_depth, lz, tail..., sl.tile_last);
     };
     auto launch_verb = [&](auto plain, auto aov, auto bg, unsigned g, const int32_t* map, uint4* work) {
         if (j.aov_target) launch(aov, g, map, work, j.aov_target);
@@ -1962,7 +1966,7 @@
     }
     if (j.phase == 2) { hz.slab = 2; hz.tile_work_a = sl.tile_work_a; }
     const int nblocks8 = ((j.f.tiles_x + 7) >> 3) * ((j.f.tiles_y + 7) >> 3);
-    hipLaunchKernelGGL(k_tile_pass, dim3((unsigned)nblocks8), dim3(64), 0, s, sl.tile_work, g, sl.sstart, sl.send, hz, sl.partial, sl.st_scan);
+    hipLaunchKernelGGL(k_tile_pass, dim3((unsigned)nblocks8), dim3(64), 0, s, sl.tile_work, sl.tile_last, g, sl.sstart, sl.send, hz, sl.partial, sl.st_scan);
     uint32_t* const prefix_arg = (j.f.sh_order > 0 && c->opt_lazy) ? c->prefix : (uint32_t*)nullptr;
     const uint32_t* const redo_arg = j.lazy ? reinterpret_cast<const uint32_t*>(sl.lazy_ctr) : (const uint32_t*)nullptr;
     uint32_t* const work_next = sl.sup_work ? sl.sup_work + 256 * (sl.sup_par ^ 1) : (uint32_t*)nullptr;
@@ -2236,11 +2240,24 @@
 {
     (void)c;
     const FrameJob& j = sl.job;
+    const int nwords = ((j.f.tiles_x + 7) >> 3) * ((j.f.tiles_y + 7) >> 3);
+    if (nwords > GSR_VERDICT_WORDS_MAX) return set_err(GSR_E_INVALID, "gsr_render: the frame has more tile blocks than verdict words");
     volatile unsigned long long* box = sl.h_end;
-    unsigned long long v = 0;
-    const int wrc = wait_mailbox(sl, box, j.ticket, "culling verdict", &v);
-    if (wrc) return wrc;
-    *broke = (v & GSR_END_HORIZON_BROKE) != 0ull;
+    GsrVerdictScan vs;
+    if (!vs.advance(box, nwords, j.ticket)) {
+        const auto t0 = std::chrono::steady_clock::now();
+        for (unsigned long spins = 1; !vs.advance(box, nwords, j.ticket); ++spins) {
+            if ((spins & 0xffu) == 0 && std::chrono::steady_clock::now() - t0 > std::chrono::microseconds(GSR_SPIN_US)) {
+                const hipError_t q = hipStreamSynchronize(sl.stream);
+                if (q != hipSuccess) return set_err(GSR_E_HIP, "gsr_render: waiting for the %s: %s", "culling verdict", hipGetErrorString(q));
+                if (!vs.advance(box, nwords, j.ticket)) return set_err(GSR_E_HIP, "gsr_render: the frame finished without delivering its %s", "culling verdict");
+                break;
+            }
+            __builtin_ia32_pause();
+        }
+    }
+    *broke = vs.broke;
+    sl.verdict_ticket = j.ticket; sl.verdict_broke = vs.broke;
     return GSR_OK;
 }
 
@@ -2378,10 +2395,11 @@
 
     if ((size_t)j.local_tiles + 1 > sl.tile_cap || !sl.sstart) {
         HIP_TRY(hipStreamSynchronize(s));
-        dev_free(sl.tile_work); dev_free(sl.tile_work_a); dev_free(sl.sstart); dev_free(sl.send); dev_free(sl.redo);
+        dev_free(sl.tile_work); dev_free(sl.tile_last); dev_free(sl.tile_work_a); dev_free(sl.sstart); dev_free(sl.send); dev_free(sl.redo);
         sl.tile_cap = 0;
-        if ((rc = dev_alloc(&sl.tile_work, (size_t)j.local_tiles + 1)) || (rc = dev_alloc(&sl.tile_work_a, (size_t)j.local_tiles + 1)) || (rc = dev_alloc(&sl.sstart, (size_t)65536 + 1)) ||
+        if ((rc = dev_alloc(&sl.tile_work, (size_t)j.local_tiles + 1)) || (rc = dev_alloc(&sl.tile_last, (size_t)j.local_tiles + 1)) || (rc = dev_alloc(&sl.tile_work_a, (size_t)j.local_tiles + 1)) || (rc = dev_alloc(&sl.sstart, (size_t)65536 + 1)) ||
             (rc = dev_alloc(&sl.send, (size_t)65536 + 1)) || (rc = dev_alloc(&sl.redo, (size_t)j.local_tiles + 1))) return rc;
+        HIP_TRY(hipMemset(sl.tile_last, 0xff, ((size_t)j.local_tiles + 1) * sizeof(uint2)));
         sl.tile_cap = (size_t)j.local_tiles + 1;
     }
     if (j.phase == 1 && j.out_px > sl.tbuf_cap && (rc = regrow(s, sl.tbuf, sl.tbuf_cap, j.out_px, j.out_px))) return rc;
@@ -2980,6 +2998,12 @@
     int rc = sync_all(c);
     if (rc) return rc;
     fetch_counters(c);
+    for (int k = 0; k < GSR_MAX_SLOTS; ++k) {
+        FrameSlot& vsl = c->slot[k];
+        if (!vsl.verdict_ticket || !vsl.h_counters || (uint32_t)(vsl.h_counters[0] >> 32) != vsl.verdict_ticket) continue;
+        if (((vsl.h_counters[0] & (unsigned long long)GSR_END_HORIZON_BROKE) != 0ull) != vsl.verdict_broke) c->st.verdict_mismatch += 1;
+        vsl.verdict_ticket = 0;
+    }
     FrameSlot* last = latest_slot(c);
     for (int k = 0; k < GSR_MAX_SLOTS; ++k)
         if (&c->slot[k] != last) harvest_slot(c, c->slot[k]);
@@ -3243,6 +3267,29 @@
     return GSR_OK;
 }
 
+extern "C" int gsr_debug_read_tile_last(gsr_context* c, uint32_t* last2, int64_t n_tiles)
+{
+    if (!c || !last2) return set_err(GSR_E_INVALID, "gsr_debug_read_tile_last: bad argument");
+    HIP_TRY(hipSetDevice(c->device));
+    int rc = sync_all(c);
+    if (rc) return rc;
+    FrameSlot* sl = latest_slot(c);
+    if (!sl || n_tiles != (int64_t)sl->last_tiles_x * sl->last_local_ty)
+        return set_err(GSR_E_INVALID, "gsr_debug_read_tile_last: expected %d tiles", sl ? sl->last_tiles_x * sl->last_local_ty : 0);
+    if (n_tiles) HIP_TRY(hipMemcpy(last2, sl->tile_last, (size_t)n_tiles * 8, hipMemcpyDeviceToHost));
+    return GSR_OK;
+}
+
+extern "C" int gsr_debug_verdict_words(const uint64_t* words, int32_t count, uint32_t ticket, int32_t polls, int32_t* out3)
+{
+    if (!out3 || (count > 0 && !words) || count > GSR_VERDICT_WORDS_MAX) return set_err(GSR_E_INVALID, "gsr_debug_verdict_words: bad argument");
+    GsrVerdictScan vs;
+    bool done = false;
+    for (int32_t p = 0; p < (polls > 0 ? polls : 1); ++p) done = vs.advance(reinterpret_cast<const volatile unsigned long long*>(words), count, ticket);
+    out3[0] = done ? 1 : 0; out3[1] = vs.broke ? 1 : 0; out3[2] = vs.next;
+    return GSR_OK;
+}
+
 extern "C" int gsr_debug_read_tile_work(gsr_context* c, uint32_t* work4, int64_t n_tiles)
 {
     if (!c || !work4) return set_err(GSR_E_INVALID, "gsr_debug_read_tile_work: bad argument");
diff --git a/houdini-gsplat-renderer_amd/csrc/gsr_mailbox.h b/houdini-gsplat-renderer_amd/csrc/gsr_mailbox.h
--- a/houdini-gsplat-renderer_amd/csrc/gsr_mailbox.h
+++ b/houdini-gsplat-renderer_amd/csrc/gsr_mailbox.h
@@ -25,3 +25,19 @@
     }
     bool has(uint32_t hint) const { return (hints & hint) != 0u; }
 };
+
+static constexpr int GSR_VERDICT_WORDS_MAX = 16384;
+struct GsrVerdictScan {
+    int next = 0;
+    bool broke = false;
+    bool advance(const volatile unsigned long long* words, int count, uint32_t ticket)
+    {
+        while (next < count) {
+            const unsigned long long v = words[next];
+            if ((uint32_t)(v >> 32) != ticket) return false;
+            if (v & (unsigned long long)GSR_END_HORIZON_BROKE) broke = true;
+            ++next;
+        }
+        return true;
+    }
+};
diff --git a/houdini-gsplat-renderer_amd/csrc/k_blend.h b/houdini-gsplat-renderer_amd/csrc/k_blend.h
--- a/houdini-gsplat-renderer_amd/csrc/k_blend.h
+++ b/houdini-gsplat-renderer_amd/csrc/k_blend.h
@@ -86,8 +86,8 @@
 gsr_blend_tile(const GsrBlendArgs& a, const int32_t* __restrict__ tile_map, const uint2* __restrict__ svals,
                const int32_t* __restrict__ sstart, const int32_t* __restrict__ send,
                const GsrRecord* __restrict__ recs, float4* __restrict__ out, uint4* __restrict__ tile_work,
-               const float* __restrict__ zwin, const float* __restrict__ depth, const GsrLazyArgs& lz, float2* __restrict__ aov = nullptr,
-               const GsrBgArgs* __restrict__ bg = nullptr)
+               const float* __restrict__ zwin, const float* __restrict__ depth, const GsrLazyArgs& lz, uint2* __restrict__ tile_last,
+               float2* __restrict__ aov = nullptr, const GsrBgArgs* __restrict__ bg = nullptr)
 {
     constexpr bool ZSTAGE = HAS_DEPTH || AOV;
     constexpr int PF4 = 5;
@@ -101,6 +101,7 @@
     __shared__ uint32_t slastu[4];
     __shared__ uint32_t stail[32];
     __shared__ uint32_t slast[4];
+    __shared__ uint32_t sring[32];
 
     int tile;
     if (LAZY) {
@@ -159,7 +160,7 @@
     if (a.slab == 2) {
         const uint4 wa = a.tile_work_a[tile];
         if (wa.w & 1u) {
-            if (tid == 0) tile_work[tile] = make_uint4(0u, 0u, 0u, 1u | 0x8000u | (0xffffu << 16));
+            if (tid == 0) { tile_work[tile] = make_uint4(0u, 0u, 0u, 1u | 0x8000u | (0xffffu << 16)); tile_last[tile] = make_uint2(0xffffffffu, 0xffffffffu); }
             return;
         }
         if (pix_ok) {
@@ -253,6 +254,15 @@
             if (h3) { q[pos & (BL_QCAP - 1)] = preB.z; }
             q_tail += wt.x + wt.y + wt.z + wt.w;
             if (tid == 0) stail[(scan_pos >> 10) & 31] = q_tail;
+            {
+                int rem2 = rem;
+                if constexpr (AOV) {
+                    int n2 = n;
+                    asm volatile("" : "+s"(n2));
+                    rem2 = n2 - (scan_pos + 4 * tid);
+                }
+                if (tid == 255 ? rem2 > 0 : (rem2 > 0 && rem2 <= 4)) sring[(scan_pos >> 10) & 31] = rem2 == 1 ? preA.x : (rem2 == 2 ? preA.z : (rem2 == 3 ? preB.x : preB.z));
+            }
             if (first_hit_step < 0 && q_tail != 0u) first_hit_step = scan_pos >> 10;
             scan_pos += 1024;
             spar ^= 1;
@@ -517,6 +527,11 @@
         const uint32_t fs = (uint32_t)(first_hit_step < 0 ? 0 : (first_hit_step > 0x1fff ? 0x1fff : first_hit_step)) | (sdmet ? 0x2000u : 0u);
         const uint4 tw = make_uint4((uint32_t)(rd < n ? rd : n), fetched, sevals, (saturated ? 1u : 0u) | (fs << 1) | (u_all ? 0x8000u : 0u) | (es_c << 16) | (es_u << 24));
         tile_work[tile] = tw;
+        const int last_step = (scan_pos >> 10) - 1;
+        auto last_of = [&](uint32_t es) __attribute__((always_inline)) -> uint32_t {
+            return (es != 0u && es != 0xffu && last_step - (int)(es - 1u) < 32) ? (sring[(es - 1u) & 31] & a.idx_mask) : 0xffffffffu;
+        };
+        tile_last[tile] = make_uint2(last_of(es_c), last_of(es_u));
         if (a.sup_work && gsr_tile_weight(tw)) atomicAdd(&a.sup_work[st], gsr_tile_weight(tw));
     }
 }
@@ -526,18 +541,18 @@
 k_blend(GsrBlendArgs a, const int32_t* __restrict__ tile_map, const uint2* __restrict__ svals,
         const int32_t* __restrict__ sstart, const int32_t* __restrict__ send,
         const GsrRecord* __restrict__ recs, float4* __restrict__ out, uint4* __restrict__ tile_work,
-        const float* __restrict__ zwin, const float* __restrict__ depth, GsrLazyArgs lz)
-{
-    gsr_blend_tile<HAS_DEPTH, false>(a, tile_map, svals, sstart, send, recs, out, tile_work, zwin, depth, lz);
+        const float* __restrict__ zwin, const float* __restrict__ depth, GsrLazyArgs lz, uint2* __restrict__ tile_last)
+{
+    gsr_blend_tile<HAS_DEPTH, false>(a, tile_map, svals, sstart, send, recs, out, tile_work, zwin, depth, lz, tile_last);
 }
 template <bool HAS_DEPTH>
 __global__ void __launch_bounds__(256)
 k_blend_lazy(GsrBlendArgs a, const int32_t* __restrict__ tile_map, const uint2* __restrict__ svals,
              const int32_t* __restrict__ sstart, const int32_t* __restrict__ send,
              const GsrRecord* __restrict__ recs, float4* __restrict__ out, uint4* __restrict__ tile_work,
-             const float* __restrict__ zwin, const float* __restrict__ depth, GsrLazyArgs lz)
-{
-    gsr_blend_tile<HAS_DEPTH, true>(a, tile_map, svals, sstart, send, recs, out, tile_work, zwin, depth, lz);
+             const float* __restrict__ zwin, const float* __restrict__ depth, GsrLazyArgs lz, uint2* __restrict__ tile_last)
+{
+    gsr_blend_tile<HAS_DEPTH, true>(a, tile_map, svals, sstart, send, recs, out, tile_work, zwin, depth, lz, tile_last);
 }
 
 template <bool HAS_DEPTH>
@@ -545,18 +560,18 @@
 k_blend_aov(GsrBlendArgs a, const int32_t* __restrict__ tile_map, const uint2* __restrict__ svals,
             const int32_t* __restrict__ sstart, const int32_t* __restrict__ send,
             const GsrRecord* __restrict__ recs, float4* __restrict__ out, uint4* __restrict__ tile_work,
-            const float* __restrict__ zwin, const float* __restrict__ depth, GsrLazyArgs lz, float2* __restrict__ aov)
-{
-    gsr_blend_tile<HAS_DEPTH, false, true>(a, tile_map, svals, sstart, send, recs, out, tile_work, zwin, depth, lz, aov);
+            const float* __restrict__ zwin, const float* __restrict__ depth, GsrLazyArgs lz, float2* __restrict__ aov, uint2* __restrict__ tile_last)
+{
+    gsr_blend_tile<HAS_DEPTH, false, true>(a, tile_map, svals, sstart, send, recs, out, tile_work, zwin, depth, lz, tile_last, aov);
 }
 template <bool HAS_DEPTH>
 __global__ void __launch_bounds__(256)
 k_blend_aov_lazy(GsrBlendArgs a, const int32_t* __restrict__ tile_map, const uint2* __restrict__ svals,
                  const int32_t* __restrict__ sstart, const int32_t* __restrict__ send,
                  const GsrRecord* __restrict__ recs, float4* __restrict__ out, uint4* __restrict__ tile_work,
-                 const float* __restrict__ zwin, const float* __restrict__ depth, GsrLazyArgs lz, float2* __restrict__ aov)
-{
-    gsr_blend_tile<HAS_DEPTH, true, true>(a, tile_map, svals, sstart, send, recs, out, tile_work, zwin, depth, lz, aov);
+                 const float* __restrict__ zwin, const float* __restrict__ depth, GsrLazyArgs lz, float2* __restrict__ aov, uint2* __restrict__ tile_last)
+{
+    gsr_blend_tile<HAS_DEPTH, true, true>(a, tile_map, svals, sstart, send, recs, out, tile_work, zwin, depth, lz, tile_last, aov);
 }
 
 template <bool HAS_DEPTH>
@@ -564,18 +579,18 @@
 k_blend_over(GsrBlendArgs a, const int32_t* __restrict__ tile_map, const uint2* __restrict__ svals,
              const int32_t* __restrict__ sstart, const int32_t* __restrict__ send,
              const GsrRecord* __restrict__ recs, float4* __restrict__ out, uint4* __restrict__ tile_work,
-             const float* __restrict__ zwin, const float* __restrict__ depth, GsrLazyArgs lz, GsrBgArgs bg)
-{
-    gsr_blend_tile<HAS_DEPTH, false, false, true>(a, tile_map, svals, sstart, send, recs, out, tile_work, zwin, depth, lz, nullptr, &bg);
+             const float* __restrict__ zwin, const float* __restrict__ depth, GsrLazyArgs lz, GsrBgArgs bg, uint2* __restrict__ tile_last)
+{
+    gsr_blend_tile<HAS_DEPTH, false, false, true>(a, tile_map, svals, sstart, send, recs, out, tile_work, zwin, depth, lz, tile_last, nullptr, &bg);
 }
 template <bool HAS_DEPTH>
 __global__ void __launch_bounds__(256)
 k_blend_over_lazy(GsrBlendArgs a, const int32_t* __restrict__ tile_map, const uint2* __restrict__ svals,
                   const int32_t* __restrict__ sstart, const int32_t* __restrict__ send,
                   const GsrRecord* __restrict__ recs, float4* __restrict__ out, uint4* __restrict__ tile_work,
-                  const float* __restrict__ zwin, const float* __restrict__ depth, GsrLazyArgs lz, GsrBgArgs bg)
-{
-    gsr_blend_tile<HAS_DEPTH, true, false, true>(a, tile_map, svals, sstart, send, recs, out, tile_work, zwin, depth, lz, nullptr, &bg);
+                  const float* __restrict__ zwin, const float* __restrict__ depth, GsrLazyArgs lz, GsrBgArgs bg, uint2* __restrict__ tile_last)
+{
+    gsr_blend_tile<HAS_DEPTH, true, false, true>(a, tile_map, svals, sstart, send, recs, out, tile_work, zwin, depth, lz, tile_last, nullptr, &bg);
 }
 
 #ifdef SW_PROFILE
@@ -590,6 +605,9 @@
 #endif
 #ifndef SW_HEADROOM_ADD
 #define SW_HEADROOM_ADD 1024u
+#endif
+#ifndef TP_POST_FENCE
+#define TP_POST_FENCE 0
 #endif
 struct GsrSumArgs {
     int32_t n_tiles, tiles_x, tiles_y , super_shift, stiles_x, n_super;
@@ -621,7 +639,7 @@
     uint32_t wmax, unsat, nused, nfin, viol, pad_;
 };
 __global__ void __launch_bounds__(64)
-k_tile_pass(const uint4* __restrict__ tile_work, GsrSumArgs g, const int32_t* __restrict__ sstart, const int32_t* __restrict__ send,
+k_tile_pass(const uint4* __restrict__ tile_work, const uint2* __restrict__ tile_last, GsrSumArgs g, const int32_t* __restrict__ sstart, const int32_t* __restrict__ send,
             GsrHorizonArgs hz, GsrTilePartial* __restrict__ partial ,
             uint32_t* __restrict__ st_scan )
 {
@@ -631,10 +649,6 @@
     const int b = (int)blockIdx.x, by = b / nbx, bx = b - by * nbx;
     const int tx = bx * 8 + lx, gty = by * 8 + ly;
     const bool inside = tx < g.tiles_x && gty < g.tiles_y;
-    if (hz.raw && b == 0) {
-        const int n45 = gsr_pyr_dim(g.tiles_x, 4) * gsr_pyr_dim(g.tiles_y, 4) + gsr_pyr_dim(g.tiles_x, 5) * gsr_pyr_dim(g.tiles_y, 5);
-        for (int i = lane; i < n45; i += 64) hz.pyr_out[hz.pyr_off[4] + i] = 0.0f;
-    }
     bool own = false;
     int ti = 0, st = 0;
     if (inside && gsr_shard_owns(g.shard, gty)) {
@@ -643,6 +657,7 @@
         if (i < g.n_tiles) { own = true; ti = i; st = (gty >> g.super_shift) * g.stiles_x + (tx >> g.super_shift); }
     }
     uint4 w = tile_work[ti];
+    const uint2 tl = tile_last[ti];
     uint4 wa = make_uint4(0u, 0u, 0u, 0u);
     if (hz.slab == 2 && own) wa = hz.tile_work_a[ti];
     const bool a_done = (wa.w & 1u) != 0u;
@@ -669,6 +684,40 @@
     const bool opaque = own && (classic_now || (w.w & 0x8000u) != 0u);
     const uint32_t first = ((w.w >> 1) & 0x1fffu) << 10;
     const uint32_t want = rd + ((rd > first ? rd - first : 0u) >> 2) + 1024u;
+    uint32_t viol = 0u, nused = 0u, nfin = 0u;
+    const bool ok = opaque && rd > 0u && rd <= len;
+    const bool c1 = opaque_c && rdc > 0u && rdc <= len && hold < 3.0e38f, c2 = ok && want < len;
+    bool c3 = false;
+    uint32_t i2 = 0u;
+    float klast = 0.0f;
+    if (hz.raw) {
+        uint32_t i1 = pred_classic ? tl.x : tl.y;
+        if (__ballot(c1 && i1 == 0xffffffffu) != 0ull) {
+            const bool need = c1 && i1 == 0xffffffffu;
+            const uint32_t l1 = hz.lists[need ? (uint32_t)s0 + rdc - 1u : 0u].x & hz.idx_mask;
+            if (need) i1 = l1;
+        }
+        c3 = ok && !c2 && !(hold < 3.0e38f) && hz.depth_culled != 0;
+        i2 = hz.lists[c2 ? (uint32_t)s0 + want : (c3 ? (uint32_t)s0 + len - 1u : 0u)].x & hz.idx_mask;
+        const float4 P1 = hz.geoA[c1 ? i1 : 0u];
+        { const float dx = P1.x - hz.cam[0], dy = P1.y - hz.cam[1], dz = P1.z - hz.cam[2]; klast = gsr_fma(dz, dz, gsr_fma(dy, dy, dx * dx)); }
+        const bool none_c = opaque_c && !pred_classic && rdc == 0u;
+        if (own && hold < 3.0e38f && !none_c && (!opaque_c || !c1 || !(klast <= hold))) viol = 1u;
+    }
+    const bool any_viol = __ballot(viol != 0u) != 0ull;
+    if (hz.host_end && lane == 0) {
+        const unsigned long long word = ((unsigned long long)hz.ticket << 32) | (unsigned long long)(any_viol ? GSR_END_HORIZON_BROKE : 0u);
+#if TP_POST_FENCE
+        hz.host_end[b] = word;
+        __threadfence_system();
+#else
+        __hip_atomic_store(hz.host_end + b, word, __ATOMIC_RELAXED, __HIP_MEMORY_SCOPE_SYSTEM);
+#endif
+    }
+    if (hz.raw && b == 0) {
+        const int n45 = gsr_pyr_dim(g.tiles_x, 4) * gsr_pyr_dim(g.tiles_y, 4) + gsr_pyr_dim(g.tiles_x, 5) * gsr_pyr_dim(g.tiles_y, 5);
+        for (int i = lane; i < n45; i += 64) hz.pyr_out[hz.pyr_off[4] + i] = 0.0f;
+    }
     {
         const int gs = g.super_shift < 3 ? g.super_shift : 3;
         uint32_t m = opaque_all ? rd_all : 0u, open = (own && !opaque_all && !a_done) ? 1u : 0u, any = own ? 1u : 0u;
@@ -682,22 +731,13 @@
             if (open) st_scan[256 + gst] = 1u;
         }
     }
-    uint32_t viol = 0u, nused = 0u, nfin = 0u;
     if (hz.raw) {
-        const bool ok = opaque && rd > 0u && rd <= len;
-        const bool c1 = opaque_c && rdc > 0u && rdc <= len && hold < 3.0e38f, c2 = ok && want < len;
-        const uint32_t i1 = hz.lists[c1 ? (uint32_t)s0 + rdc - 1u : 0u].x & hz.idx_mask;
-        const bool c3 = ok && !c2 && !(hold < 3.0e38f) && hz.depth_culled != 0;
-        const uint32_t i2 = hz.lists[c2 ? (uint32_t)s0 + want : (c3 ? (uint32_t)s0 + len - 1u : 0u)].x & hz.idx_mask;
-        const float4 P1 = hz.geoA[c1 ? i1 : 0u], P2 = hz.geoA[c2 ? i2 : 0u];
-        float klast, hnew;
-        { const float dx = P1.x - hz.cam[0], dy = P1.y - hz.cam[1], dz = P1.z - hz.cam[2]; klast = gsr_fma(dz, dz, gsr_fma(dy, dy, dx * dx)); }
+        const float4 P2 = hz.geoA[c2 ? i2 : 0u];
+        float hnew;
         { const float dx = P2.x - hz.cam[0], dy = P2.y - hz.cam[1], dz = P2.z - hz.cam[2]; hnew = gsr_fma(dz, dz, gsr_fma(dy, dy, dx * dx)); }
         float h = 0.0f;
         if (own) {
-            const bool none_c = opaque_c && !pred_classic && rdc == 0u;
             const bool none = opaque && !classic_now && rd == 0u;
-            if (hold < 3.0e38f && !none_c && (!opaque_c || !c1 || !(klast <= hold))) viol = 1u;
             if (viol && hz.dbg) {
                 const uint32_t k = atomicAdd(hz.dbg, 1u);
                 if (k < 8u) {
@@ -727,7 +767,6 @@
         nused += __shfl_down(nused, d, 64); nfin += __shfl_down(nfin, d, 64);
         { const uint32_t o = __shfl_down(wmax, d, 64); wmax = o > wmax ? o : wmax; }
     }
-    const bool any_viol = __ballot(viol != 0u) != 0ull;
     if (lane == 0) {
         GsrTilePartial p;
         p.scanned = sc; p.fetched = fe; p.evals = ev; p.wmax = wmax; p.unsat = unsat; p.nused = nused; p.nfin = nfin;
@@ -842,11 +881,6 @@
     }
     __syncthreads();
     SWP(2)
-    if (hz.host_end && threadIdx.x == 0) {
-        uint32_t v = s_viol;
-        *hz.host_end = ((unsigned long long)hz.ticket << 32) | (unsigned long long)(v ? GSR_END_HORIZON_BROKE : 0u);
-        __threadfence_system();
-    }
     if (sup_work_next) sup_work_next[threadIdx.x] = 0u;
     {
         const int st = (int)threadIdx.x;
@@ -876,7 +910,8 @@
         const unsigned long long t2 = old2 + s_sum[1], t4 = old4 + s_sum[0], t5 = old5 + s_sum[2];
         counters[1] = s_sum[1]; counters[2] = t2; counters[3] = s_sum[0]; counters[4] = t4; counters[5] = t5;
         if (colour_evals) *colour_total = old_ct + s_cev;
-        summary[0] = 0ull; summary[1] = s_sum[1]; summary[2] = t2; summary[3] = s_sum[0]; summary[4] = t4; summary[5] = t5;
+        summary[0] = hz.host_end ? (((unsigned long long)hz.ticket << 32) | (unsigned long long)(s_viol ? GSR_END_HORIZON_BROKE : 0u)) : 0ull;
+        summary[1] = s_sum[1]; summary[2] = t2; summary[3] = s_sum[0]; summary[4] = t4; summary[5] = t5;
         summary[6] = (unsigned long long)nvis;
         summary[7] = (unsigned long long)nredo;
     }
diff --git a/houdini-gsplat-renderer_amd/engine.py b/houdini-gsplat-renderer_amd/engine.py
--- a/houdini-gsplat-renderer_amd/engine.py
+++ b/houdini-gsplat-renderer_amd/engine.py
@@ -37,7 +37,7 @@
                 ("lazy_redo_tiles", C.c_int64), ("lazy_colours_total", C.c_int64), ("frames_truncated", C.c_int64),
                 ("frames_culled", C.c_int64), ("frames_repaired", C.c_int64),
                 ("clusters_total", C.c_int64), ("clusters_kept", C.c_int64),
-                ("policy_bits", C.c_int32), ("cull_dilate", C.c_int32), ("cull_holdoff", C.c_int32), ("reserved2_", C.c_int32),
+                ("policy_bits", C.c_int32), ("cull_dilate", C.c_int32), ("cull_holdoff", C.c_int32), ("verdict_mismatch", C.c_int32),
                 ("frames_resorted", C.c_int64), ("frames_slab", C.c_int64), ("frames_jumped", C.c_int64), ("frames_lazy", C.c_int64),
                 ("uploads", C.c_int64), ("upload_ms", C.c_double * 6),
                 ("moves", C.c_int64), ("move_ms", C.c_double * 4)]
@@ -136,7 +136,7 @@
     "gsr_upload_begin", "gsr_upload_append", "gsr_upload_append_raw", "gsr_upload_end", "gsr_upload_abort", "gsr_upload", "gsr_set_row_shard", "gsr_band_rows",
     "gsr_stitch_bands", "gsr_render", "gsr_render_depth", "gsr_render_wire", "gsr_render_wire_over", "gsr_synchronize", "gsr_get_stats", "gsr_stats_reset", "gsr_set_option",
     "gsr_debug_read_records", "gsr_debug_read_depth_order", "gsr_debug_read_storage_order", "gsr_debug_read_tile_lists", "gsr_debug_sort_pairs", "gsr_debug_sort_pairs_local", "gsr_debug_policy", "gsr_debug_policy_state", "gsr_debug_frame_plan",
-    "gsr_debug_read_tile_work", "gsr_debug_read_horizons", "gsr_debug_read_cull",
+    "gsr_debug_read_tile_work", "gsr_debug_read_tile_last", "gsr_debug_verdict_words", "gsr_debug_read_horizons", "gsr_debug_read_cull",
     "gsr_multi_create", "gsr_multi_destroy", "gsr_multi_count", "gsr_multi_transport", "gsr_multi_context",
     "gsr_multi_set_stream", "gsr_multi_set_option", "gsr_multi_upload_begin", "gsr_multi_upload_append",
     "gsr_multi_upload_end", "gsr_multi_upload_abort", "gsr_multi_upload", "gsr_multi_render", "gsr_multi_render_depth",
@@ -266,6 +266,8 @@
     L.gsr_debug_policy_state.argtypes = [vp, vp]
     L.gsr_debug_frame_plan.argtypes = [i32, vp, vp, vp]
     L.gsr_debug_read_tile_work.argtypes = [vp, vp, i64]
+    L.gsr_debug_read_tile_last.argtypes = [vp, vp, i64]
+    L.gsr_debug_verdict_words.argtypes = [vp, C.c_int32, C.c_uint32, C.c_int32, vp]
     L.gsr_debug_read_horizons.argtypes = [vp, vp, i64]
     L.gsr_target_pixel_bytes.argtypes = [i32]
     L.gsr_set_target_format.argtypes = [vp, i32]
@@ -1019,6 +1021,13 @@
         _check(self.L.gsr_debug_read_tile_work(self.h, out.ctypes.data, nt))
         return out.reshape(st["tiles_y"], st["tiles_x"], 4)
 
+    def debug_tile_last(self) -> np.ndarray:
+        st = self.stats()
+        nt = st["tiles_x"] * st["tiles_y"]
+        out = np.zeros((nt, 2), np.uint32)
+        _check(self.L.gsr_debug_read_tile_last(self.h, out.ctypes.data, nt))
+        return out.reshape(st["tiles_y"], st["tiles_x"], 2)
+
     def debug_horizons(self, tiles_x: int, tiles_y: int) -> np.ndarray:
         out = np.zeros((4, tiles_y, tiles_x), np.float32)
         _check(self.L.gsr_debug_read_horizons(self.h, out.ctypes.data, tiles_x * tiles_y))
diff --git a/include/gsplat_hip.h b/include/gsplat_hip.h
--- a/include/gsplat_hip.h
+++ b/include/gsplat_hip.h
@@ -68,7 +68,7 @@
     int32_t policy_bits;
     int32_t cull_dilate;
     int32_t cull_holdoff;
-    int32_t reserved2_;
+    int32_t verdict_mismatch;
     int64_t frames_resorted;
     int64_t frames_slab;
     int64_t frames_jumped;
@@ -299,6 +299,8 @@
                                int32_t* pair_splat, int64_t n_pairs);
 
 int  gsr_debug_read_tile_work(gsr_context* ctx, uint32_t* work4, int64_t n_tiles);
+int  gsr_debug_read_tile_last(gsr_context* ctx, uint32_t* last2, int64_t n_tiles);
+int  gsr_debug_verdict_words(const uint64_t* words, int32_t count, uint32_t ticket, int32_t polls, int32_t* out3);
 int  gsr_debug_read_horizons(gsr_context* ctx, float* out4, int64_t n_tiles);
 
 int  gsr_debug_sort_pairs(gsr_context* ctx, uint32_t* keys, uint32_t* vals, int64_t n, int key_bits);
```

New measurement: 4533. No clear change (-0.7%).
